# Ryan21wy/HSIMAE

Hardware: AMD Instinct MI355X
Metric: HSI patches/sec (9x9x96, mask 75%) pretrain fwd+bwd (higher is better)
Workload: dtype bf16; 1 GPU; HSIMAE-Base pretrain fwd+bwd, 9x9x96 cubes, per-GPU batch 4096, mask 0.75, bf16 MFMA operands / fp32 accumulate + residual; per_gpu_batch=4096, global_batch=4096, parallelism=dp1

## Files before the change

hsimae_amd/_lib.py:

```python
from __future__ import annotations

import ctypes as C
import os

HERE = os.path.dirname(os.path.abspath(__file__))
LIB_PATH = os.environ.get("HSIMAE_LIB") or os.path.join(HERE, "libhsimae_hip.so")

i32, i64, f32, vp = C.c_int32, C.c_int64, C.c_float, C.c_void_p


class Config(C.Structure):
    _fields_ = [("bands", i32), ("embed_dim", i32), ("depth", i32), ("s_depth", i32), ("num_heads", i32),
                ("dec_dim", i32), ("dec_depth", i32), ("dec_heads", i32), ("hidden", i32), ("dec_hidden", i32),
                ("norm_pix_loss", i32), ("precision", i32)]


class IO(C.Structure):
    _fields_ = [("x", vp), ("sn", i64), ("sb", i64), ("sh", i64), ("sw", i64),
                ("N", i32), ("len_t", i32), ("len_l", i32),
                ("noise1", vp), ("noise2", vp), ("params", vp), ("wpk", vp),
                ("workspace", vp), ("workspace_bytes", i64),
                ("grad_scale", f32), ("want_recons", i32),
                ("loss", vp), ("pred_img", vp), ("mask_img", vp), ("mask", vp),
                ("ids_keep", vp), ("ids_restore", vp), ("latent", vp), ("pred", vp), ("drop_scale", vp),
                ("bucket_stream", vp), ("det_acc", vp)]


class MaskParams(C.Structure):
    _fields_ = [("noise1", vp), ("noise2", vp), ("N", i32), ("T", i32), ("L", i32), ("len_t", i32), ("len_l", i32),
                ("ids_keep", vp), ("ids_restore", vp), ("mask", vp)]


class PatchParams(C.Structure):
    _fields_ = [("x", vp), ("sn", i64), ("sb", i64), ("sh", i64), ("sw", i64), ("N", i32), ("T", i32), ("K", i32),
                ("ids_keep", vp), ("out", vp), ("pos_ids", vp)]


class GemmParams(C.Structure):
    _fields_ = [("A", vp), ("lda", i32), ("M", i32), ("N", i32), ("K", i32), ("n_valid", i32),
                ("W", vp), ("W2", vp), ("bias", vp), ("bias2", vp), ("gamma", vp), ("beta", vp),
                ("stats", vp), ("u_out", vp), ("ldu", i32), ("out", vp), ("ldo", i32),
                ("res", vp), ("res2", vp), ("ldr", i32), ("pos", vp), ("ids", vp), ("ldpos", i32),
                ("h13", vp), ("ldh", i32), ("hoff", i32),
                ("lnx", vp), ("dgamma", vp), ("dbeta", vp), ("accumulate", i32),
                ("a_rowscale", vp), ("out_rowscale", vp),
                ("prec", i32), ("W8", vp), ("S8", vp), ("W8b", vp), ("S8b", vp), ("ln_width", i32),
                ("det_base", vp), ("det_acc", vp)]


class PackDesc(C.Structure):
    _fields_ = [("src", vp), ("rows", i32), ("cols", i32), ("transpose", i32), ("n_off", i32), ("k_off", i32),
                ("KS", i32), ("dst", vp), ("fp8", i32), ("scales", vp)]


class AttnParams(C.Structure):
    _fields_ = [("qkv", vp), ("ld", i32), ("d", i32), ("heads", i32), ("hd", i32), ("Ts", i32), ("nsamples", i32),
                ("mode", i32), ("len_l", i32), ("o", vp), ("ldo", i32), ("lse", vp), ("dout", vp), ("lddo", i32),
                ("dqkv", vp), ("kv_off", i32)]


class AttnBlockWeights(C.Structure):
    _fields_ = [(n, vp) for n in ("n1w", "n1b", "bqkv", "pb", "qkv", "p", "qkvT", "pT")]


class MlpWeights(C.Structure):
    _fields_ = [("n2w", vp), ("n2b", vp), ("w1b", vp), ("w3b", vp), ("w2b", vp),
                ("w1", vp), ("w3", vp), ("w2", vp), ("w2T", vp), ("w13T", vp), ("hidden", i32)]


class DecBlockWeights(C.Structure):
    _fields_ = [(n, vp) for n in ("n1w", "n1b", "bqkv", "pb", "n2w", "n2b", "w1b", "w3b", "w2b", "qkv", "p", "w1", "w3", "w2", "w2T",
                                  "qf", "kf", "vf", "pf", "w1f", "w3f")] + [("hidden", i32)]


class DecBlockGrads(C.Structure):
    _fields_ = [(n, vp) for n in ("n1w", "n1b", "qw", "qb", "kw", "kb", "vw", "vb", "pw", "pb", "n2w", "n2b", "w1w", "w1b", "w2w",
                                  "w2b", "w3w", "w3b")]


class WgradTask(C.Structure):
    _fields_ = [("dO", vp), ("dO_f32", i32), ("ldo", i32), ("A", vp), ("lda", i32), ("N", i32), ("K", i32),
                ("dW", vp), ("ldw", i32), ("db", vp), ("dO_rowscale", vp), ("dO_plane_rows", i32), ("A_plane_rows", i32)]


class WgradParams(C.Structure):
    _fields_ = [("t", WgradTask * 16), ("ntasks", i32), ("M", i32), ("msplit", i32), ("det_base", vp), ("det_acc", vp), ("slab", vp)]


class LnBwdParams(C.Structure):
    _fields_ = [("du", vp), ("x", vp), ("stats", vp), ("gamma", vp), ("dres", vp), ("dx", vp), ("accumulate", i32),
                ("dgamma", vp), ("dbeta", vp), ("M", i32), ("d", i32), ("ld", i32),
                ("det_base", vp), ("det_acc", vp)]


class AssembleParams(C.Structure):
    _fields_ = [("y", vp), ("N", i32), ("K", i32), ("TL", i32), ("Dd", i32), ("ids_restore", vp), ("pos", vp),
                ("yfull", vp), ("dyfull", vp), ("dy", vp), ("ld", i32)]


class LossParams(C.Structure):
    _fields_ = [("x", vp), ("sn", i64), ("sb", i64), ("sh", i64), ("sw", i64), ("N", i32), ("T", i32),
                ("pred", vp), ("mask", vp), ("norm_pix", i32), ("inv_scale", f32), ("partial", vp), ("loss", vp),
                ("sum_mask", f32), ("dpred", vp), ("pred_img", vp), ("mask_img", vp)]


class CubeParams(C.Structure):
    _fields_ = [("scenes", vp), ("scene_f64", i32), ("scene_off", vp), ("scene_w", vp), ("bands", i32),
                ("cut", vp), ("index", vp), ("flips", vp), ("N", i32),
                ("out", vp), ("sn", i64), ("sb", i64), ("sh", i64), ("sw", i64)]


class SceneParams(C.Structure):
    _fields_ = [("scene", vp), ("scene_f64", i32), ("H", i32), ("W", i32), ("C", i32),
                ("p0", i64), ("pixels", vp), ("N", i32),
                ("out", vp), ("sn", i64), ("sb", i64), ("sh", i64), ("sw", i64)]


class GwpcaParams(C.Structure):
    _fields_ = [("scene", vp), ("scene_f64", i32), ("H", i32), ("W", i32), ("C", i32), ("nc", i32), ("group", i32), ("whiten", i32),
                ("minmax", vp), ("mean", vp), ("lambda_", vp), ("proj", vp), ("group_off", vp)]


class BuildInfo(C.Structure):
    _fields_ = [("abi_version", i32), ("variant_bits", C.c_uint32), ("kernel_source_hash", C.c_uint64), ("flags_hash", C.c_uint64),
                ("default_flags", i32), ("reserved", i32)]


BUCKET_CB = C.CFUNCTYPE(None, i32, i64, i64, vp)

SYMBOLS = {
    "hsimae_version": (C.c_int, []),
    "hsimae_build_info": (C.c_int, [C.POINTER(BuildInfo)]),
    "hsimae_variant_name": (C.c_char_p, [C.c_int]),
    "hsimae_strerror": (C.c_char_p, [C.c_int]),
    "hsimae_two_streams_active": (C.c_int, []),
    "hsimae_effective_precision": (C.c_int, [C.POINTER(Config)]),
    "hsimae_dec_block_slab_floats": (i64, []),
    "hsimae_wgrad_slab_bytes": (i64, [C.POINTER(Config), i32]),
    "hsimae_param_layout": (C.c_int, [C.POINTER(Config), C.POINTER(i64), C.POINTER(i64), C.c_int]),
    "hsimae_wpk_elems": (i64, [C.POINTER(Config)]),
    "hsimae_pack_table_bytes": (i64, [C.POINTER(Config)]),
    "hsimae_build_pack_table": (C.c_int, [C.POINTER(Config), vp, vp, vp]),
    "hsimae_pack_params": (C.c_int, [C.POINTER(Config), vp, vp]),
    "hsimae_workspace_bytes": (i64, [C.POINTER(Config), i32, i32, i32]),
    "hsimae_forward": (C.c_int, [C.POINTER(Config), C.POINTER(IO), vp]),
    "hsimae_backward": (C.c_int, [C.POINTER(Config), C.POINTER(IO), vp, BUCKET_CB, vp, vp]),
    "hsimae_mask_from_noise": (C.c_int, [C.POINTER(MaskParams), vp]),
    "hsimae_patch_gather": (C.c_int, [C.POINTER(PatchParams), vp]),
    "hsimae_gemm": (C.c_int, [C.POINTER(GemmParams), i32, i32, vp]),
    "hsimae_gemm_tiled": (C.c_int, [C.POINTER(GemmParams), i32, i32, i32, i32, vp]),
    "hsimae_pack_matrix": (C.c_int, [vp, i32, i32, vp]),
    "hsimae_enc_mlp_fwd": (C.c_int, [vp, vp, vp, i32, i32, C.POINTER(MlpWeights), vp, vp]),
    "hsimae_enc_mlp_bwd": (C.c_int, [vp, vp, vp, vp, vp, vp, vp, vp, i32, i32, C.POINTER(MlpWeights), vp, vp, vp, vp, i32, vp]),
    "hsimae_dec_block_fwd": (C.c_int, [C.POINTER(DecBlockWeights), vp, vp, vp, vp, vp, i32, i32, i32, vp]),
    "hsimae_dec_block_bwd": (C.c_int, [C.POINTER(DecBlockWeights), C.POINTER(DecBlockGrads), vp, vp, vp, vp, vp, vp, vp, i32, i32, vp, vp]),
    "hsimae_attn_fwd": (C.c_int, [C.POINTER(AttnParams), vp]),
    "hsimae_attn_bwd": (C.c_int, [C.POINTER(AttnParams), vp]),
    "hsimae_attn_block_fwd": (C.c_int, [C.POINTER(AttnBlockWeights), vp, vp, vp, vp, vp, vp, vp, i32, i32, i32, i32, i32, i32, vp]),
    "hsimae_attn_block_bwd": (C.c_int, [C.POINTER(AttnBlockWeights), vp, vp, vp, vp, vp, vp, vp, vp, vp, vp, vp, vp, i32, i32, i32,
                                        i32, i32, i32, i32, vp]),
    "hsimae_wgrad": (C.c_int, [C.POINTER(WgradParams), vp]),
    "hsimae_wgrad_msplit": (i32, [i32, i64]),
    "hsimae_ln_bwd": (C.c_int, [C.POINTER(LnBwdParams), vp]),
    "hsimae_ln_fwd": (C.c_int, [vp, vp, vp, vp, i32, i32, vp]),
    "hsimae_assemble_fwd": (C.c_int, [C.POINTER(AssembleParams), vp]),
    "hsimae_assemble_bwd": (C.c_int, [C.POINTER(AssembleParams), vp]),
    "hsimae_loss_partials": (C.c_int, [i32, i32]),
    "hsimae_loss": (C.c_int, [C.POINTER(LossParams), vp]),
    "hsimae_adamw_step": (C.c_int, [vp, vp, vp, vp, vp, i64, f32, f32, f32, f32, f32, i32, vp]),
    "hsimae_cube_gather": (C.c_int, [C.POINTER(CubeParams), vp]),
    "hsimae_scene_windows": (C.c_int, [C.POINTER(SceneParams), vp]),
    "hsimae_class_argmax": (C.c_int, [C.POINTER(SceneParams), vp, i32, i32, i32, vp, vp]),
    "hsimae_gwpca_workspace_bytes": (i64, [C.POINTER(GwpcaParams)]),
    "hsimae_gwpca_fit": (C.c_int, [C.POINTER(GwpcaParams), vp, vp]),
    "hsimae_gwpca_apply": (C.c_int, [C.POINTER(GwpcaParams), vp, i32, vp]),
    "hsimae_encode": (C.c_int, [C.POINTER(Config), C.POINTER(IO), vp]),
    "hsimae_encode_backward": (C.c_int, [C.POINTER(Config), C.POINTER(IO), vp, vp, BUCKET_CB, vp, vp]),
    "hsimae_agg_pool": (C.c_int, [vp, vp, i32, i32, i32, i32, vp]),
    "hsimae_head_bwd": (C.c_int, [vp, vp, vp, vp, vp, vp, i32, i32, i32, i32, i32, vp]),
    "hsimae_decode": (C.c_int, [C.POINTER(Config), C.POINTER(IO), vp, vp, vp]),
    "hsimae_decode_backward": (C.c_int, [C.POINTER(Config), C.POINTER(IO), vp, vp, vp, BUCKET_CB, vp, vp]),
}

ABI_VERSION = 108
PREC_BF16, PREC_FP8 = 0, 1
A_BF16, A_F32, A_F32_LN = 0, 1, 2
E_BF16, E_F32, E_RES_F32, E_POS_F32, E_SWIGLU, E_SWIGLU_BWD, E_LN_BWD = 0, 1, 2, 3, 4, 5, 6

_lib = None


def load() -> C.CDLL:
    global _lib
    if _lib is None:
        if not os.path.exists(LIB_PATH):
            raise RuntimeError(
                f"{LIB_PATH} not found: build it with `python -m hsimae_amd.build` (hipcc --offload-arch=gfx950). "
                "hsimae_amd has no CPU fallback.")
        lib = C.CDLL(LIB_PATH)
        for name, (res, args) in SYMBOLS.items():
            fn = getattr(lib, name)
            fn.restype, fn.argtypes = res, args
        got = lib.hsimae_version()
        if got != ABI_VERSION:
            raise RuntimeError(f"{LIB_PATH} answers ABI version {got}, these bindings were written for {ABI_VERSION}: "
                               "rebuild it with `python -m hsimae_amd.build --force`")
        info = _query_build_info(lib)
        if info["variant"] and os.environ.get("HSIMAE_ALLOW_VARIANT") != "1":
            raise RuntimeError(f"{LIB_PATH} is a variant build ({', '.join(info['variant'])}): its kernels are instrumented or compute "
                               "wrong results on purpose (timing ablations).  Set HSIMAE_ALLOW_VARIANT=1 to load it for an experiment.")
        _lib = lib
    return _lib


def _query_build_info(lib) -> dict:
    bi = BuildInfo()
    rc = lib.hsimae_build_info(C.byref(bi))
    if rc != 0:
        raise RuntimeError(f"hsimae_build_info failed with code {rc}")
    names = []
    for b in range(32):
        if bi.variant_bits >> b & 1:
            n = lib.hsimae_variant_name(b)
            names.append(n.decode() if n else f"bit{b}")
    return {"path": LIB_PATH, "abi_version": bi.abi_version, "variant_bits": bi.variant_bits, "variant": names,
            "kernel_source_hash": f"{bi.kernel_source_hash:016x}", "flags_hash": f"{bi.flags_hash:016x}",
            "default_flags": bool(bi.default_flags)}


def build_info() -> dict:
    return _query_build_info(load())


def check(code: int, what: str = "hsimae") -> None:
    if code != 0:
        msg = load().hsimae_strerror(code)
        raise RuntimeError(f"{what} failed with code {code}: {msg.decode() if msg else '?'}")


def ptr(t) -> int | None:
    return None if t is None else t.data_ptr()
```

hsimae_amd/csrc/api.hip:

```cpp
#include "common.h"
#include "kernels.h"
#include "plan.h"
#include <vector>
#include <algorithm>
#include <cstring>
#include <cstdlib>
#include <mutex>
#include <unordered_map>
#include <initializer_list>

using namespace hsplan;

namespace {

#define CK(expr) do { int _e = (expr); if (_e) return _e; } while (0)
#define CK0(expr) do { int _e0 = (expr); if (_e0) return _e0; } while (0)

inline hipStream_t S(void* s) { return reinterpret_cast<hipStream_t>(s); }
struct BlkP {
    const float *n1w, *n1b, *bqkv, *pb, *n2w, *n2b, *w1b, *w3b, *w2b;
    const hs_bf16 *qkv, *p, *w1, *w3, *w2, *qkvT, *pT, *w13T, *w2T;
    const float *qf, *kf, *vf, *pf, *w1f, *w3f;
    int prec;
    struct I8 { const uint8_t* w; const uint8_t* s; } qkv8, p8, w1_8, w3_8, w2_8, qkvT8, pT8, w13T8, w2T8;
};

BlkP resolve(const BlkOff& o, const BlkW& w, const float* P, const hs_bf16* wpk, const WLayout& WL) {
    const float* fbase = reinterpret_cast<const float*>(wpk + WL.bf16_elems);
    BlkP b;
    b.n1w = P + o.n1w; b.n1b = P + o.n1b; b.bqkv = fbase + w.bqkv; b.pb = P + o.pb; b.n2w = P + o.n2w; b.n2b = P + o.n2b;
    b.w1b = P + o.w1b; b.w3b = P + o.w3b; b.w2b = P + o.w2b;
    b.qkv = wpk + w.qkv; b.p = wpk + w.p; b.w1 = wpk + w.w1; b.w3 = wpk + w.w3; b.w2 = wpk + w.w2;
    b.qkvT = wpk + w.qkvT; b.pT = wpk + w.pT; b.w13T = wpk + w.w13T; b.w2T = wpk + w.w2T;
    b.qf = P + o.qw; b.kf = P + o.kw; b.vf = P + o.vw; b.pf = P + o.pw; b.w1f = P + o.w1w; b.w3f = P + o.w3w;
    const uint8_t* base8 = reinterpret_cast<const uint8_t*>(fbase + WL.f32_elems);
    auto i8 = [&](const Img8& im) { BlkP::I8 r; r.w = base8 + im.w; r.s = base8 + im.s; return r; };
    b.prec = HSIMAE_PREC_BF16;
    b.qkv8 = i8(w.qkv8); b.p8 = i8(w.p8); b.w1_8 = i8(w.w1_8); b.w3_8 = i8(w.w3_8); b.w2_8 = i8(w.w2_8);
    b.qkvT8 = i8(w.qkvT8); b.pT8 = i8(w.pT8); b.w13T8 = i8(w.w13T8); b.w2T8 = i8(w.w2T8);
    return b;
}
enum : uint32_t {
    SC_FUSED_DEC = 1u << 0,
    SC_DEC_SPLIT = 1u << 1,
    SC_FP8_UNFUSED = 1u << 2,
    SC_FUSED_MLP = 1u << 3,
    SC_ATTN_BLOCK = 1u << 4,
    SC_ATTN_BLOCK256 = 1u << 5,
    SC_ATTN_BLOCK_BWD = 1u << 6,
    SC_PROJ_BWD = 1u << 7,
    SC_LNBWD = 1u << 8,
    SC_LNBWD_512 = 1u << 9,
    SC_RECOMPUTE = 1u << 10,
    SC_WGRAD_SLAB = 1u << 11,
    SC_DEC_SLAB = 1u << 12,
    SC_PLANAR = 1u << 13,
    SC_ATTN_BLOCK256_BWD = 1u << 14,
};
uint32_t sched_from_env() {
    auto off = [](const char* name) { const char* e = getenv(name); return e && e[0] == '0'; };
    auto one = [](const char* name) { const char* e = getenv(name); return e && e[0] == '1'; };
    uint32_t b = 0;
    if (!off("HSIMAE_FUSED_DEC")) b |= SC_FUSED_DEC;
    if (!off("HSIMAE_DEC_SPLIT")) b |= SC_DEC_SPLIT;
    if (one("HSIMAE_FP8_UNFUSED")) b |= SC_FP8_UNFUSED;
    if (!off("HSIMAE_FUSED_MLP")) b |= SC_FUSED_MLP;
    if (!off("HSIMAE_FUSED_ATTN_BLOCK")) b |= SC_ATTN_BLOCK;
    if (!off("HSIMAE_FUSED_ATTN_BLOCK256")) b |= SC_ATTN_BLOCK256;
    if (!off("HSIMAE_FUSED_ATTN_BLOCK_BWD")) b |= SC_ATTN_BLOCK_BWD;
    if (!off("HSIMAE_FUSED_PROJ_BWD")) b |= SC_PROJ_BWD;
    if (!off("HSIMAE_FUSED_LNBWD")) b |= SC_LNBWD;
    if (!off("HSIMAE_FUSED_LNBWD_512")) b |= SC_LNBWD_512;
    if (!off("HSIMAE_ATTN_BWD_RECOMPUTE")) b |= SC_RECOMPUTE;
    if (!off("HSIMAE_WGRAD_SLAB")) b |= SC_WGRAD_SLAB;
    if (!off("HSIMAE_DEC_SLAB")) b |= SC_DEC_SLAB;
    if (!off("HSIMAE_WGRAD_PLANAR")) b |= SC_PLANAR;
    if (!off("HSIMAE_FUSED_ATTN_BLOCK256_BWD")) b |= SC_ATTN_BLOCK256_BWD;
    return b;
}
struct SchedRec { uint32_t enc = 0, dec = 0; bool has_enc = false, has_dec = false; uint64_t gen = 0; };
std::mutex g_sched_mu;
std::unordered_map<const void*, SchedRec> g_sched;
uint64_t g_sched_gen = 0;
void record_sched(const void* ws, bool enc, bool dec, uint32_t bits) {
    std::lock_guard<std::mutex> lk(g_sched_mu);
    if (g_sched.size() > 4096 && g_sched.find(ws) == g_sched.end()) {
        std::vector<uint64_t> gens;
        gens.reserve(g_sched.size());
        for (auto& kv : g_sched) gens.push_back(kv.second.gen);
        std::nth_element(gens.begin(), gens.begin() + gens.size() / 2, gens.end());
        const uint64_t cut = gens[gens.size() / 2];
        for (auto it = g_sched.begin(); it != g_sched.end();) it = it->second.gen < cut ? g_sched.erase(it) : std::next(it);
    }
    SchedRec& r = g_sched[ws];
    r.gen = ++g_sched_gen;
    if (enc) {
        r.enc = bits; r.has_enc = true;
        if (!dec) r.has_dec = false;
    }
    if (dec) { r.dec = bits; r.has_dec = true; }
}
int lookup_sched(const void* ws, bool need_enc, bool need_dec, uint32_t& enc, uint32_t& dec) {
    std::lock_guard<std::mutex> lk(g_sched_mu);
    auto it = g_sched.find(ws);
    if (it == g_sched.end() || (need_enc && !it->second.has_enc) || (need_dec && !it->second.has_dec)) return HSIMAE_ENOFORWARD;
    enc = it->second.enc; dec = it->second.dec;
    return HSIMAE_OK;
}

BlkP resolve_enc(const Geo& g, uint32_t sc, const BlkOff& o, const BlkW& w, const float* P, const hs_bf16* wpk, const WLayout& WL) {
    BlkP b = resolve(o, w, P, wpk, WL);
    b.prec = (g.prec == HSIMAE_PREC_FP8 && (g.D >= 512 || (sc & SC_FP8_UNFUSED))) ? HSIMAE_PREC_FP8 : HSIMAE_PREC_BF16;
    return b;
}


struct Side {
    hipStream_t s = nullptr; hipEvent_t fork = nullptr, join = nullptr; bool ok = false, init = false;
    std::vector<hipEvent_t> pool; size_t next = 0;
};
Side& side() {
    static Side sides[32];
    static Side none;
    static std::mutex mu;
    int dev = -1;
    if (hipGetDevice(&dev) != hipSuccess || dev < 0 || dev >= 32) return none;
    std::lock_guard<std::mutex> lk(mu);
    Side& x = sides[dev];
    if (!x.init) {
        x.init = true;
        const char* e = getenv("HSIMAE_TWO_STREAMS");
        if (!(e && e[0] == '0'))
            x.ok = hipStreamCreateWithFlags(&x.s, hipStreamNonBlocking) == hipSuccess &&
                   hipEventCreateWithFlags(&x.fork, hipEventDisableTiming) == hipSuccess &&
                   hipEventCreateWithFlags(&x.join, hipEventDisableTiming) == hipSuccess;
    }
    return x;
}
hipEvent_t pool_event(Side& sd) {
    if (sd.pool.size() < 96) {
        hipEvent_t e = nullptr;
        if (hipEventCreateWithFlags(&e, hipEventDisableTiming) == hipSuccess) { sd.pool.push_back(e); return e; }
    }
    if (sd.pool.empty()) return nullptr;
    return sd.pool[sd.next++ % sd.pool.size()];
}

struct Emitter {
    hsimae_bucket_cb cb; void* user; hipStream_t bucket; int stage;
    float* grads; const int64_t* det_acc;
    int operator()(int64_t off, int64_t end, hipStream_t done_on) {
        if (det_acc) CK0(hs_det_convert(det_acc + off, grads + off, end - off, done_on));
        if (cb) {
            if (bucket) {
                hipEvent_t e = pool_event(side());
                if (!e) return (int)hipErrorOutOfMemory;
                CK0((int)hipEventRecord(e, done_on));
                CK0((int)hipStreamWaitEvent(bucket, e, 0));
            }
            cb(stage, off, end - off, user);
        }
        ++stage;
        return HSIMAE_OK;
    }
};

bool fused_dec_enabled(const Geo& g, uint32_t sc) {
    return (sc & SC_FUSED_DEC) && hs_dec_fused_supported(g.Dd, g.Hd, g.hdec, g.TL);
}



bool fused_mlp_enabled(int d, int h, uint32_t sc) {
    return (sc & SC_FUSED_MLP) && hs_enc_mlp_fused_supported(d, h);
}

EncMlpPtrs mlp_ptrs(const BlkP& b, int h) {
    EncMlpPtrs m;
    m.n2w = b.n2w; m.n2b = b.n2b; m.w1b = b.w1b; m.w3b = b.w3b; m.w2b = b.w2b;
    m.w1 = b.w1; m.w3 = b.w3; m.w2 = b.w2; m.w2T = b.w2T; m.w13T = b.w13T; m.h = h;
    return m;
}

DecBlockPtrs dec_ptrs(const BlkP& b, int h) {
    DecBlockPtrs d;
    d.n1w = b.n1w; d.n1b = b.n1b; d.bqkv = b.bqkv; d.pb = b.pb; d.n2w = b.n2w; d.n2b = b.n2b;
    d.w1b = b.w1b; d.w3b = b.w3b; d.w2b = b.w2b;
    d.qkv = b.qkv; d.p = b.p; d.w1 = b.w1; d.w3 = b.w3; d.w2 = b.w2;
    d.qkvT = b.qkvT; d.pT = b.pT; d.w13T = b.w13T; d.w2T = b.w2T; d.h = h;
    d.qf = b.qf; d.kf = b.kf; d.vf = b.vf; d.pf = b.pf; d.w1f = b.w1f; d.w3f = b.w3f;
    return d;
}

GemmParams gp() { GemmParams p; std::memset(&p, 0, sizeof(p)); return p; }

int dec_block_fwd_fused(const BlkP& bp, const float* z, const BlkBuf& b, int N, int64_t Md, int TL, int Dd, int hdec, uint32_t sc, hipStream_t s) {
    if ((sc & SC_DEC_SPLIT) && hs_enc_mlp_fused_supported(Dd, hdec)) {
        CK(hs_dec_attn_fwd(z, b.x1, b.o, b.lse, N, TL, dec_ptrs(bp, hdec), s));
        return hs_enc_mlp_fwd(b.x1, nullptr, b.x2, (int)Md, Dd, mlp_ptrs(bp, hdec), s);
    }
    return hs_dec_block_fwd(z, b.x1, b.x2, b.o, b.lse, N, TL, dec_ptrs(bp, hdec), s);
}

static bool attn_bwd_recompute(int d, int dp, int heads, int h, int Ts, bool f8u, uint32_t sc) {
    if (!(sc & SC_PROJ_BWD) || !(sc & SC_LNBWD) || !(sc & SC_RECOMPUTE)) return false;
    return !f8u && d == 128 && dp == d && fused_mlp_enabled(d, h, sc) && (sc & SC_ATTN_BLOCK) && (sc & SC_ATTN_BLOCK_BWD) &&
           hs_attn_block_bwd_fusable(d, heads, Ts);
}

int block_fwd(const BlkP& P, uint32_t sc, const float* x_in, const BlkBuf& b, int64_t M, int d, int heads, int h, int hp, int Ts,
              int nsamples, int mode, int len_l, const float* res2, hipStream_t s, const float* rs_a = nullptr,
              const float* rs_m = nullptr) {
    GemmParams p = gp();
    const int dp = rup(d, 32);
    const bool f8 = P.prec == HSIMAE_PREC_FP8;
    const bool f8u = f8 && (sc & SC_FP8_UNFUSED);
    auto w8 = [&](GemmParams& q, const BlkP::I8& a) { if (f8) { q.prec = HSIMAE_PREC_FP8; q.W8 = a.w; q.S8 = a.s; } };
    if (!f8u && (sc & SC_ATTN_BLOCK) && hs_attn_block_fusable(d, heads, Ts)) {
        CK(hs_attn_block_fwd(x_in, P.n1w, P.n1b, P.qkv, P.bqkv, P.p, P.pb, b.u, attn_bwd_recompute(d, dp, heads, h, Ts, f8u, sc) ? nullptr : b.qkv,
                             b.o, b.lse, b.x1, rs_a, Ts, nsamples, mode, len_l, s));
        if (fused_mlp_enabled(d, h, sc)) return hs_enc_mlp_fwd(b.x1, res2, b.x2, (int)M, d, mlp_ptrs(P, h), s, rs_m);
    } else if (!f8 && dp == d && (sc & SC_ATTN_BLOCK256) && hs_attn_block256_fusable(d, heads, Ts, nsamples)) {
        CK(hs_attn_block256_fwd(x_in, P.n1w, P.n1b, P.qkv, P.bqkv, P.p, P.pb, b.u, b.qkv, b.o, b.lse, b.x1, rs_a, Ts, nsamples, mode,
                                len_l, s));
    } else {
    p.A = x_in; p.lda = dp; p.M = (int)M; p.N = 3 * dp; p.K = dp; p.n_valid = 3 * dp; p.W = P.qkv; p.bias = P.bqkv;
    p.gamma = P.n1w; p.beta = P.n1b; p.u_out = b.u; p.ldu = dp; p.out = b.qkv; p.ldo = 3 * dp; p.ln_width = d;
    w8(p, P.qkv8);
    CK(hs_gemm(p, A_F32_LN, E_BF16, s));
    AttnParams a; std::memset(&a, 0, sizeof(a));
    a.qkv = b.qkv; a.ld = 3 * dp; a.d = d; a.heads = heads; a.hd = d / heads; a.Ts = Ts; a.nsamples = nsamples;
    a.mode = mode; a.len_l = len_l; a.o = b.o; a.ldo = dp; a.lse = b.lse; a.kv_off = dp;
    CK(hs_attn_fwd(a, s));
    p = gp();
    p.A = b.o; p.lda = dp; p.M = (int)M; p.N = dp; p.K = dp; p.n_valid = d; p.W = P.p; p.bias = P.pb;
    p.res = x_in; p.ldr = dp; p.out = b.x1; p.ldo = dp; p.out_rowscale = rs_a;
    w8(p, P.p8);
    CK(hs_gemm(p, A_BF16, E_RES_F32, s));
    }
    if (!f8u && fused_mlp_enabled(d, h, sc)) return hs_enc_mlp_fwd(b.x1, res2, b.x2, (int)M, d, mlp_ptrs(P, h), s, rs_m);
    p = gp();
    p.A = b.x1; p.lda = dp; p.M = (int)M; p.N = hp; p.K = dp; p.n_valid = h; p.W = P.w1; p.W2 = P.w3; p.bias = P.w1b;
    p.bias2 = P.w3b; p.gamma = P.n2w; p.beta = P.n2b; p.u_out = b.u2; p.ldu = dp; p.out = b.g; p.ldo = hp;
    p.h13 = b.h13; p.ldh = 2 * hp; p.hoff = hp; p.ln_width = d;
    if (f8) { w8(p, P.w1_8); p.W8b = P.w3_8.w; p.S8b = P.w3_8.s; }
    CK(hs_gemm(p, A_F32_LN, E_SWIGLU, s));
    p = gp();
    p.A = b.g; p.lda = hp; p.M = (int)M; p.N = dp; p.K = hp; p.n_valid = d; p.W = P.w2; p.bias = P.w2b;
    p.res = b.x1; p.res2 = res2; p.ldr = dp; p.out = b.x2; p.ldo = dp; p.out_rowscale = rs_m;
    w8(p, P.w2_8);
    CK(hs_gemm(p, A_BF16, E_RES_F32, s));
    return HSIMAE_OK;
}


static bool wide_ln_fused(int d, int dp, bool f8, uint32_t sc) {
    return (sc & SC_LNBWD) && dp == d && (d == 256 || (d == 512 && f8 && (sc & SC_LNBWD_512)));
}

int block_bwd(const BlkP& P, uint32_t sc, const BlkOff& o, float* grads, const float* x_in, const BlkBuf& b, int64_t M, int d,
              int heads, int h, int hp, int Ts, int nsamples, int mode, int len_l, float* G0, const Scr& w,
              float* dx_out, int accumulate, hipStream_t s, int concurrent = 1, const float* rs_a = nullptr,
              const float* rs_m = nullptr, int64_t* det_acc = nullptr) {
    float* G1 = w.G1;
    GemmParams p = gp();
    const int dp = rup(d, 32);
    LnBwdParams l; std::memset(&l, 0, sizeof(l));
    l.M = (int)M; l.d = d; l.ld = dp; l.det_base = grads; l.det_acc = det_acc;
    const bool f8 = P.prec == HSIMAE_PREC_FP8;
    const bool f8u = f8 && (sc & SC_FP8_UNFUSED);
    auto w8 = [&](GemmParams& q, const BlkP::I8& a) { if (f8) { q.prec = HSIMAE_PREC_FP8; q.W8 = a.w; q.S8 = a.s; } };
    const bool fmlp = !f8u && fused_mlp_enabled(d, h, sc);
    bool g1b_done = false;
    const int hp64 = rup(hp, 64);
    const bool planar = fmlp && (sc & SC_PLANAR) && M % 32 == 0 && (M + kPlanePadRows) * 2 * (int64_t)(hp64 + 256) * 2 < (1ll << 32);
    const int prow = planar ? (int)M + HS_PLANE_PAD_ROWS : 0;
    if (fmlp) {
        CK(hs_enc_mlp_bwd(b.x1, G0, G1, b.u2, w.dh13, b.g, w.g0b, w.g1b, (int)M, d, mlp_ptrs(P, h), grads + o.n2w,
                          grads + o.n2b, s, rs_m, rs_a, HsDet{grads, reinterpret_cast<long long*>(det_acc)}, prow));
    } else {
        p.A = G0; p.lda = dp; p.M = (int)M; p.N = hp; p.K = dp; p.n_valid = hp; p.W = P.w2T; p.out = w.dh13; p.ldo = 2 * hp;
        p.h13 = b.h13; p.ldh = 2 * hp; p.hoff = hp; p.a_rowscale = rs_m;
        w8(p, P.w2T8);
        CK(hs_gemm(p, A_F32, E_SWIGLU_BWD, s));
        p = gp();
        p.A = w.dh13; p.lda = 2 * hp; p.M = (int)M; p.N = dp; p.K = 2 * hp; p.n_valid = d; p.W = P.w13T;
        w8(p, P.w13T8);
        if (wide_ln_fused(d, dp, f8, sc)) {
            p.out = G1; p.ldo = dp; p.res = G0; p.ldr = dp; p.lnx = b.x1; p.gamma = P.n2w; p.accumulate = 0;
            p.dgamma = grads + o.n2w; p.dbeta = grads + o.n2b; p.det_base = grads; p.det_acc = det_acc;
            if (!rs_a) { p.u_out = w.g1b; p.ldu = dp; g1b_done = true; }
            CK(hs_gemm(p, A_BF16, E_LN_BWD, s));
        } else {
            p.out = w.du; p.ldo = dp;
            CK(hs_gemm(p, A_BF16, E_F32, s));
            l.du = w.du; l.x = b.x1; l.gamma = P.n2w; l.dres = G0; l.dx = G1; l.accumulate = 0;
            l.dgamma = grads + o.n2w; l.dbeta = grads + o.n2b;
            CK(hs_ln_bwd(l, s));
        }
        CK(hs_rows_to_bf16(G0, w.g0b, M, dp, rs_m, s));
        if (!g1b_done) CK(hs_rows_to_bf16(G1, w.g1b, M, dp, rs_a, s));
    }
    auto run_wgrad = [&]() -> int {
        WgradParams g; std::memset(&g, 0, sizeof(g));
        auto task = [&](int, const void* dO, int ldo, const hs_bf16* A, int lda, int N, int K, int64_t dW, int64_t db) {
            WgradTask& t = g.t[g.ntasks++];
            t.dO = dO; t.dO_f32 = 0; t.ldo = ldo; t.A = A; t.lda = lda; t.N = N; t.K = K; t.dW = grads + dW; t.ldw = K;
            t.db = grads + db; t.dO_rowscale = nullptr;
        };
        task(0, w.dqkv, 3 * dp, b.u, dp, d, d, o.qw, o.qb);
        task(1, w.dqkv + dp, 3 * dp, b.u, dp, d, d, o.kw, o.kb);
        task(2, w.dqkv + 2 * dp, 3 * dp, b.u, dp, d, d, o.vw, o.vb);
        task(3, w.g1b, dp, b.o, dp, d, d, o.pw, o.pb);
        if (planar) {
            task(4, w.dh13, hp64, b.u2, dp, h, d, o.w1w, o.w1b); g.t[g.ntasks - 1].dO_plane_rows = prow;
            task(5, w.dh13 + (int64_t)hp64 * prow, hp64, b.u2, dp, h, d, o.w3w, o.w3b); g.t[g.ntasks - 1].dO_plane_rows = prow;
        } else {
            task(4, w.dh13, 2 * hp, b.u2, dp, h, d, o.w1w, o.w1b);
            task(5, w.dh13 + hp, 2 * hp, b.u2, dp, h, d, o.w3w, o.w3b);
        }
#ifdef HS_ABL_DW2
        if (!fmlp)
#endif
        { task(6, w.g0b, dp, b.g, planar ? hp64 : hp, d, h, o.w2w, o.w2b); g.t[g.ntasks - 1].A_plane_rows = prow; }
        g.M = (int)M; g.det_base = grads; g.det_acc = det_acc;
        g.slab = (sc & SC_WGRAD_SLAB) ? w.slab : nullptr;
        int tiles = 0;
        for (int i = 0; i < g.ntasks; ++i) tiles += ((g.t[i].N + 127) / 128) * ((g.t[i].K + 127) / 128);
        g.msplit = wgrad_msplit(tiles, M, concurrent);
        return hs_wgrad(g, s);
    };
    AttnParams a; std::memset(&a, 0, sizeof(a));
    a.qkv = b.qkv; a.ld = 3 * dp; a.d = d; a.heads = heads; a.hd = d / heads; a.Ts = Ts; a.nsamples = nsamples;
    a.mode = mode; a.len_l = len_l; a.o = b.o; a.ldo = dp; a.lse = b.lse; a.dout = w.dob; a.lddo = dp; a.dqkv = w.dqkv; a.kv_off = dp;
    const bool fuse_pb = (sc & SC_PROJ_BWD) != 0;
    const bool fuse_ln = (sc & SC_LNBWD) != 0;
    const bool rc = attn_bwd_recompute(d, dp, heads, h, Ts, f8u, sc);
    const bool blk_bwd = rc || (fuse_pb && fuse_ln && fmlp && !f8u && d == 128 && dp == d && hs_attn_proj_fusable(a) &&
                                (sc & SC_ATTN_BLOCK_BWD) && hs_attn_block_bwd_fusable(d, heads, Ts));
    const bool blk256_bwd = !blk_bwd && !f8 && dp == d && (sc & SC_ATTN_BLOCK256_BWD) && (sc & SC_LNBWD) && (sc & SC_PROJ_BWD) &&
                            hs_attn_block256_bwd_fusable(d, heads, Ts, nsamples);
    if (blk256_bwd) {
        CK(hs_attn_block256_bwd(b.qkv, b.lse, w.g1b, G1, x_in, P.n1w, P.pT, P.qkvT, w.dqkv, dx_out, grads + o.n1w, grads + o.n1b, grads,
                                reinterpret_cast<long long*>(det_acc), Ts, nsamples, mode, len_l, accumulate, s));
        CK(run_wgrad());
        return HSIMAE_OK;
    }
    if (blk_bwd) {
        CK(hs_attn_block_bwd(rc ? nullptr : b.qkv, b.u, P.qkv, P.bqkv, b.o, b.lse, w.g1b, G1, x_in, P.n1w, P.pT, P.qkvT, w.dqkv, dx_out,
                             grads + o.n1w, grads + o.n1b, grads, reinterpret_cast<long long*>(det_acc), Ts, nsamples, mode, len_l,
                             accumulate, s));
    } else {
        p = gp();
        p.A = w.g1b; p.lda = dp; p.M = (int)M; p.N = dp; p.K = dp; p.n_valid = dp;
        p.W = P.pT; p.out = w.dob; p.ldo = dp;
        w8(p, P.pT8);
        CK(hs_gemm(p, A_BF16, E_BF16, s));
    }
    if (!blk_bwd) CK(hs_attn_bwd(a, s));
    CK(run_wgrad());

    if (blk_bwd) return HSIMAE_OK;
    const bool ln_fused = fuse_ln && ((d == 128 && !f8u) || wide_ln_fused(d, dp, f8, sc));
    p = gp();
    p.A = w.dqkv; p.lda = 3 * dp; p.M = (int)M; p.N = dp; p.K = 3 * dp; p.n_valid = d; p.W = P.qkvT;
    if (ln_fused) {
        p.out = dx_out; p.ldo = d; p.res = G1; p.ldr = d; p.lnx = x_in; p.gamma = P.n1w; p.accumulate = accumulate;
        p.dgamma = grads + o.n1w; p.dbeta = grads + o.n1b; p.det_base = grads; p.det_acc = det_acc;
        if (d != 128) w8(p, P.qkvT8);
        CK(hs_gemm(p, A_BF16, E_LN_BWD, s));
    } else {
        p.out = w.du; p.ldo = dp;
        w8(p, P.qkvT8);
        CK(hs_gemm(p, A_BF16, E_F32, s));
    }

    if (!ln_fused) {
        l.du = w.du; l.x = x_in; l.gamma = P.n1w; l.dres = G1; l.dx = dx_out; l.accumulate = accumulate;
        l.dgamma = grads + o.n1w; l.dbeta = grads + o.n1b;
        CK(hs_ln_bwd(l, s));
    }
    return HSIMAE_OK;
}

struct Ctx {
    Geo g; PLayout L; WLayout W; Ws w;
    int N, K, len_t, len_l;
    int64_t Me, Md;
};

int make_ctx(const hsimae_config* cfg, const hsimae_io* io, Ctx& c, bool need_ws) {
    CK(make_geo(cfg, c.g));
    if (!io) return HSIMAE_ENULL;
    c.N = io->N; c.len_t = io->len_t; c.len_l = io->len_l;
    if (c.N <= 0 || c.len_t < 1 || c.len_t > c.g.T || c.len_l < 1 || c.len_l > 9) return HSIMAE_EDIMS;
    c.K = c.len_t * c.len_l;
    c.Me = (int64_t)c.N * c.K; c.Md = (int64_t)c.N * c.g.TL;
    if (c.Md * 96 >= (1ll << 31) || c.Me * 3 * c.g.Dp >= (1ll << 31)) return HSIMAE_EUNSUPPORTED;
    make_playout(c.g, c.L);
    make_wlayout(c.g, c.W);
    if (need_ws) {
        if (!io->workspace || !io->params || !io->wpk) return HSIMAE_ENULL;
        if (reinterpret_cast<uintptr_t>(io->workspace) % 256) return HSIMAE_EALIGN;
        carve(c.g, c.N, c.K, reinterpret_cast<char*>(io->workspace), c.w);
        if (c.w.bytes > io->workspace_bytes) return HSIMAE_EDIMS;
    }
    return HSIMAE_OK;
}

}

extern "C" unsigned hs_variant_bits_gemm();
extern "C" unsigned hs_variant_bits_attn();
extern "C" unsigned hs_variant_bits_attn_wide();
extern "C" unsigned hs_variant_bits_wgrad();
extern "C" unsigned hs_variant_bits_elem();
extern "C" unsigned hs_variant_bits_pack();
extern "C" unsigned hs_variant_bits_fused_dec();
extern "C" unsigned hs_variant_bits_fused_enc();
extern "C" unsigned hs_variant_bits_loader();
extern "C" unsigned hs_variant_bits_scene();
extern "C" unsigned hs_variant_bits_gwpca();
#ifndef HS_KERNEL_SOURCE_HASH
#define HS_KERNEL_SOURCE_HASH 0ULL
#endif
#ifndef HS_BUILD_FLAGS_HASH
#define HS_BUILD_FLAGS_HASH 0ULL
#endif
#ifndef HS_BUILD_DEFAULT_FLAGS
#define HS_BUILD_DEFAULT_FLAGS 0
#endif

extern "C" {

int hsimae_version(void) { return HSIMAE_VERSION; }

int hsimae_build_info(hsimae_build_info_t* out) {
    if (!out) return HSIMAE_ENULL;
    out->abi_version = HSIMAE_VERSION;
    out->variant_bits = hs_variant_bits() | hs_variant_bits_gemm() | hs_variant_bits_attn() | hs_variant_bits_attn_wide() | hs_variant_bits_wgrad() | hs_variant_bits_elem() | hs_variant_bits_pack() | hs_variant_bits_fused_dec() | hs_variant_bits_fused_enc() | hs_variant_bits_loader() | hs_variant_bits_scene() | hs_variant_bits_gwpca();
    out->kernel_source_hash = HS_KERNEL_SOURCE_HASH;
    out->flags_hash = HS_BUILD_FLAGS_HASH;
    out->default_flags = HS_BUILD_DEFAULT_FLAGS;
    out->reserved = 0;
    return HSIMAE_OK;
}
const char* hsimae_variant_name(int bit) {
    switch (bit) {
#define HS_X(b, name) case b: return #name;
        HS_VARIANT_TABLE(HS_X)
#undef HS_X
        default: return nullptr;
    }
}

int hsimae_two_streams_active(void) { return side().ok ? 1 : 0; }
int hsimae_effective_precision(const hsimae_config* cfg) {
    if (!cfg) return HSIMAE_ENULL;
    Geo g; CK(make_geo(cfg, g));
    return (g.prec == HSIMAE_PREC_FP8 && (g.D >= 512 || (sched_from_env() & SC_FP8_UNFUSED))) ? HSIMAE_PREC_FP8 : HSIMAE_PREC_BF16;
}

const char* hsimae_strerror(int code) {
    switch (code) {
        case HSIMAE_OK: return "ok";
        case HSIMAE_EDIMS: return "bad dimensions or strides";
        case HSIMAE_EUNSUPPORTED: return "configuration not supported by the gfx950 kernels";
        case HSIMAE_EALIGN: return "misaligned pointer";
        case HSIMAE_ENULL: return "required pointer is NULL";
        case HSIMAE_ENOFORWARD: return "no forward pass of this process has filled this workspace (the backward follows the forward's recorded schedule)";
        default: return code > 0 ? hipGetErrorString((hipError_t)code) : "unknown error";
    }
}

int hsimae_param_layout(const hsimae_config* cfg, int64_t* offsets, int64_t* sizes, int max_entries) {
    return param_layout(cfg, offsets, sizes, max_entries);
}

int64_t hsimae_wpk_elems(const hsimae_config* cfg) { return wpk_elems(cfg); }

int64_t hsimae_pack_table_bytes(const hsimae_config* cfg) { return pack_table_bytes(cfg); }

int hsimae_build_pack_table(const hsimae_config* cfg, const float* params_dev, hs_bf16* wpk_dev, void* table_host) {
    return build_pack_table(cfg, params_dev, wpk_dev, table_host);
}

int hsimae_pack_params(const hsimae_config* cfg, const void* table_dev, void* stream) {
    Geo g; CK(make_geo(cfg, g));
    if (!table_dev) return HSIMAE_ENULL;
    const int n = (int)(hsimae_pack_table_bytes(cfg) / (int64_t)sizeof(PackDesc));
    const int maxe = std::max({g.D * g.D, g.h * g.D, g.Dd * g.Dd, g.hdec * g.Dd, g.D * g.Dd, g.D * 72});
    return hs_pack(reinterpret_cast<const PackDesc*>(table_dev), n, maxe, S(stream));
}

int64_t hsimae_workspace_bytes(const hsimae_config* cfg, int32_t N, int32_t len_t, int32_t len_l) {
    return workspace_bytes(cfg, N, len_t, len_l);
}

struct DropRs { const float* a; const float* m; };
static DropRs drop_rs(const hsimae_io* io, int e, int64_t Me) {
    if (!io->drop_scale) return DropRs{nullptr, nullptr};
    const float* base = io->drop_scale + (int64_t)e * 2 * Me;
    return DropRs{base, base + Me};
}

static int forward_impl(const hsimae_config* cfg, const hsimae_io* io, void* stream, bool encoder_only) {
    Ctx c; CK(make_ctx(cfg, io, c, true));
    if (!io->x || !io->noise1 || !io->noise2 || !io->mask || !io->ids_keep || !io->ids_restore) return HSIMAE_ENULL;
    if (encoder_only ? !io->latent : !io->loss) return HSIMAE_ENULL;
    if (!encoder_only && io->want_recons && (!io->pred_img || !io->mask_img)) return HSIMAE_ENULL;
    hipStream_t s = S(stream);
    const Geo& g = c.g; const float* P = io->params; const Ws& w = c.w;
    const uint32_t sc = sched_from_env();
    record_sched(io->workspace, true, !encoder_only, sc);

    MaskParams m; m.noise1 = io->noise1; m.noise2 = io->noise2; m.N = c.N; m.T = g.T; m.L = 9; m.len_t = c.len_t;
    m.len_l = c.len_l; m.ids_keep = io->ids_keep; m.ids_restore = io->ids_restore; m.mask = io->mask;
    CK(hs_mask(m, s));
    PatchParams pp; pp.x = io->x; pp.sn = io->sn; pp.sb = io->sb; pp.sh = io->sh; pp.sw = io->sw; pp.N = c.N; pp.T = g.T;
    pp.K = c.K; pp.ids_keep = io->ids_keep; pp.out = w.a_pe; pp.pos_ids = nullptr;
    CK(hs_patch_gather(pp, s));
    GemmParams p = gp();
    p.A = w.a_pe; p.lda = 96; p.M = (int)c.Me; p.N = g.Dp; p.K = 96; p.n_valid = g.D; p.W = io->wpk + c.W.pe; p.bias = P + c.L.peb;
    p.pos = P + c.L.pos; p.ids = io->ids_keep; p.ldpos = g.D; p.out = w.x0; p.ldo = g.Dp;
    CK(hs_gemm(p, A_BF16, E_POS_F32, s));

    const float* x = w.x0;
    if (g.has_axis) {
        Side& sd = side();
        const bool forked = sd.ok && g.sdepth > 1;
        if (forked) {
            CK((int)hipEventRecord(sd.fork, s));
            CK((int)hipStreamWaitEvent(sd.s, sd.fork, 0));
        }
        const float* xa = w.x0;
        const float* xb = w.x0;
        for (int i = 0; i < g.sdepth; ++i) {
            BlkP b1 = resolve_enc(g, sc, c.L.b1[i], c.W.b1[i], P, io->wpk, c.W);
            const DropRs r1 = drop_rs(io, i, c.Me), r2d = drop_rs(io, g.sdepth + i, c.Me);
            CK(block_fwd(b1, sc, xa, w.b1[i], c.Me, g.D, g.H, g.h, g.hp, c.K, c.N, 1, c.len_l, nullptr, s, r1.a, r1.m));
            xa = w.b1[i].x2;
            BlkP b2 = resolve_enc(g, sc, c.L.b2[i], c.W.b2[i], P, io->wpk, c.W);
            const bool last = (i == g.sdepth - 1);
            const float* r2 = last ? xa : nullptr;
            if (last && forked) {
                CK((int)hipEventRecord(sd.join, sd.s));
                CK((int)hipStreamWaitEvent(s, sd.join, 0));
            }
            CK(block_fwd(b2, sc, xb, w.b2[i], c.Me, g.D, g.H, g.h, g.hp, c.K, c.N, 2, c.len_l, r2, (forked && !last) ? sd.s : s,
                         r2d.a, r2d.m));
            xb = w.b2[i].x2;
        }
        x = xb;
    }
    for (int i = 0; i < g.nfus; ++i) {
        BlkP bp = resolve_enc(g, sc, c.L.bf[i], c.W.bf[i], P, io->wpk, c.W);
        const DropRs rf = drop_rs(io, (g.has_axis ? 2 * g.sdepth : 0) + i, c.Me);
        CK(block_fwd(bp, sc, x, w.bf[i], c.Me, g.D, g.H, g.h, g.hp, c.K, c.N, 0, c.len_l, nullptr, s, rf.a, rf.m));
        x = w.bf[i].x2;
    }
    if (encoder_only) {
        CK(hs_ln_fwd(x, P + c.L.nw, P + c.L.nb, io->latent, (int)c.Me, g.D, s, g.Dp, g.D));
        return HSIMAE_OK;
    }
    p = gp();
    p.A = x; p.lda = g.Dp; p.M = (int)c.Me; p.N = g.Ddp; p.K = g.Dp; p.n_valid = g.Dd; p.W = io->wpk + c.W.de; p.bias = P + c.L.deb;
    p.gamma = P + c.L.nw; p.beta = P + c.L.nb; p.u_out = w.lat; p.ldu = g.Dp; p.out = w.y; p.ldo = g.Ddp; p.ln_width = g.D;
    CK(hs_gemm(p, A_F32_LN, E_F32, s));
    AssembleParams as; std::memset(&as, 0, sizeof(as));
    as.y = w.y; as.N = c.N; as.K = c.K; as.TL = g.TL; as.Dd = g.Dd; as.ld = g.Ddp; as.ids_restore = io->ids_restore; as.pos = P + c.L.dpos;
    as.yfull = w.yfull;
    CK(hs_assemble_fwd(as, s));
    const float* z = w.yfull;
    const bool fdec = fused_dec_enabled(g, sc);
    for (int i = 0; i < g.ddepth; ++i) {
        BlkP bp = resolve(c.L.bd[i], c.W.bd[i], P, io->wpk, c.W);
        if (fdec) CK(dec_block_fwd_fused(bp, z, w.bd[i], c.N, c.Md, g.TL, g.Dd, g.hdec, sc, s));
        else CK(block_fwd(bp, sc, z, w.bd[i], c.Md, g.Dd, g.Hd, g.hdec, g.hpd, g.TL, c.N, 0, 9, nullptr, s));
        z = w.bd[i].x2;
    }
    p = gp();
    p.A = z; p.lda = g.Ddp; p.M = (int)c.Md; p.N = 80; p.K = g.Ddp; p.n_valid = 72; p.W = io->wpk + c.W.dp; p.bias = P + c.L.dpb;
    p.gamma = P + c.L.dnw; p.beta = P + c.L.dnb; p.u_out = w.zn; p.ldu = g.Ddp; p.out = w.pred; p.ldo = 72; p.ln_width = g.Dd;
    CK(hs_gemm(p, A_F32_LN, E_F32, s));
    LossParams lp; std::memset(&lp, 0, sizeof(lp));
    const float sum_mask = (float)((int64_t)c.N * (g.TL - c.K));
    lp.x = io->x; lp.sn = io->sn; lp.sb = io->sb; lp.sh = io->sh; lp.sw = io->sw; lp.N = c.N; lp.T = g.T; lp.pred = w.pred;
    lp.mask = io->mask; lp.norm_pix = g.norm_pix; lp.inv_scale = io->grad_scale / (72.f * sum_mask); lp.partial = w.partial;
    lp.loss = io->loss; lp.sum_mask = sum_mask; lp.dpred = w.dpred;
    lp.pred_img = io->want_recons ? io->pred_img : nullptr; lp.mask_img = io->want_recons ? io->mask_img : nullptr;
    CK(hs_loss(lp, s));
    if (io->pred) CK((int)hipMemcpyAsync(io->pred, w.pred, c.Md * 72 * 4, hipMemcpyDeviceToDevice, s));
    if (io->latent) CK(hs_ln_fwd(x, P + c.L.nw, P + c.L.nb, io->latent, (int)c.Me, g.D, s, g.Dp, g.D));
    return HSIMAE_OK;
}

int hsimae_forward(const hsimae_config* cfg, const hsimae_io* io, void* stream) { return forward_impl(cfg, io, stream, false); }
int hsimae_encode(const hsimae_config* cfg, const hsimae_io* io, void* stream) { return forward_impl(cfg, io, stream, true); }

int hsimae_decode(const hsimae_config* cfg, const hsimae_io* io, const float* latent, float* pred, void* stream) {
    Ctx c; CK(make_ctx(cfg, io, c, true));
    if (!latent || !pred || !io->ids_restore) return HSIMAE_ENULL;
    hipStream_t s = S(stream);
    const Geo& g = c.g; const float* P = io->params; const Ws& w = c.w;
    const uint32_t sc = sched_from_env();
    record_sched(io->workspace, false, true, sc);
    GemmParams p = gp();
    const float* lat_in = latent;
    if (g.Dp != g.D) {
        CK((int)hipMemcpy2DAsync(w.G2, (size_t)g.Dp * 4, latent, (size_t)g.D * 4, (size_t)g.D * 4, (size_t)c.Me, hipMemcpyDeviceToDevice, s));
        lat_in = w.G2;
    }
    p.A = lat_in; p.lda = g.Dp; p.M = (int)c.Me; p.N = g.Ddp; p.K = g.Dp; p.n_valid = g.Dd; p.W = io->wpk + c.W.de; p.bias = P + c.L.deb;
    p.out = w.y; p.ldo = g.Ddp;
    CK(hs_gemm(p, A_F32, E_F32, s));
    CK(hs_rows_to_bf16(lat_in, w.lat, c.Me, g.Dp, nullptr, s));
    AssembleParams as; std::memset(&as, 0, sizeof(as));
    as.y = w.y; as.N = c.N; as.K = c.K; as.TL = g.TL; as.Dd = g.Dd; as.ld = g.Ddp; as.ids_restore = io->ids_restore; as.pos = P + c.L.dpos;
    as.yfull = w.yfull;
    CK(hs_assemble_fwd(as, s));
    const float* z = w.yfull;
    const bool fdec = fused_dec_enabled(g, sc);
    for (int i = 0; i < g.ddepth; ++i) {
        BlkP bp = resolve(c.L.bd[i], c.W.bd[i], P, io->wpk, c.W);
        if (fdec) CK(dec_block_fwd_fused(bp, z, w.bd[i], c.N, c.Md, g.TL, g.Dd, g.hdec, sc, s));
        else CK(block_fwd(bp, sc, z, w.bd[i], c.Md, g.Dd, g.Hd, g.hdec, g.hpd, g.TL, c.N, 0, 9, nullptr, s));
        z = w.bd[i].x2;
    }
    p = gp();
    p.A = z; p.lda = g.Ddp; p.M = (int)c.Md; p.N = 80; p.K = g.Ddp; p.n_valid = 72; p.W = io->wpk + c.W.dp; p.bias = P + c.L.dpb;
    p.gamma = P + c.L.dnw; p.beta = P + c.L.dnb; p.u_out = w.zn; p.ldu = g.Ddp; p.out = pred; p.ldo = 72; p.ln_width = g.Dd;
    return hs_gemm(p, A_F32_LN, E_F32, s);
}

static int encoder_backward(const Ctx& c, const hsimae_io* io, float* grads, hipStream_t s, Emitter& emit, uint32_t sc) {
    const Geo& g = c.g; const float* P = io->params; const Ws& w = c.w; const PLayout& L = c.L;
    for (int i = g.nfus - 1; i >= 0; --i) {
        BlkP bp = resolve_enc(g, sc, L.bf[i], c.W.bf[i], P, io->wpk, c.W);
        const float* xin = (i > 0) ? w.bf[i - 1].x2 : (g.has_axis ? w.b2[g.sdepth - 1].x2 : w.x0);
        const DropRs rf = drop_rs(io, (g.has_axis ? 2 * g.sdepth : 0) + i, c.Me);
        CK(block_bwd(bp, sc, L.bf[i], grads, xin, w.bf[i], c.Me, g.D, g.H, g.h, g.hp, c.K, c.N, 0, c.len_l, w.G0, w.sc, w.G0, 0, s, 1,
                     rf.a, rf.m, io->det_acc));
        CK(emit(L.bf[i].n1w, L.bf[i].end, s));
    }
    if (g.has_axis) {
        Side& sd = side();
        const bool forked = sd.ok && g.sdepth > 1;
        CK((int)hipMemcpyAsync(w.G2, w.G0, c.Me * g.Dp * 4, hipMemcpyDeviceToDevice, s));
        if (forked) {
            CK((int)hipEventRecord(sd.fork, s));
            CK((int)hipStreamWaitEvent(sd.s, sd.fork, 0));
        }
        hipStream_t s2 = forked ? sd.s : s;
        const Scr& scr2 = forked ? w.sc2 : w.sc;
        const bool per_block = emit.bucket != nullptr || !forked;
        for (int i = g.sdepth - 1; i >= 0; --i) {
            BlkP b2 = resolve_enc(g, sc, L.b2[i], c.W.b2[i], P, io->wpk, c.W);
            const DropRs r1 = drop_rs(io, i, c.Me), r2d = drop_rs(io, g.sdepth + i, c.Me);
            const float* xin2 = (i > 0) ? w.b2[i - 1].x2 : w.x0;
            CK(block_bwd(b2, sc, L.b2[i], grads, xin2, w.b2[i], c.Me, g.D, g.H, g.h, g.hp, c.K, c.N, 2, c.len_l, w.G0, scr2, w.G0, 0, s2, forked ? 2 : 1,
                         r2d.a, r2d.m, io->det_acc));
            if (per_block) CK(emit(L.b2[i].n1w, L.b2[i].end, s2));
            if (i == 0 && forked) {
                CK((int)hipEventRecord(sd.join, sd.s));
                CK((int)hipStreamWaitEvent(s, sd.join, 0));
            }
            BlkP b1 = resolve_enc(g, sc, L.b1[i], c.W.b1[i], P, io->wpk, c.W);
            const float* xin1 = (i > 0) ? w.b1[i - 1].x2 : w.x0;
            float* out = (i == 0) ? w.G0 : w.G2;
            CK(block_bwd(b1, sc, L.b1[i], grads, xin1, w.b1[i], c.Me, g.D, g.H, g.h, g.hp, c.K, c.N, 1, c.len_l, w.G2, w.sc, out, i == 0, s, forked ? 2 : 1,
                         r1.a, r1.m, io->det_acc));
            if (per_block) CK(emit(L.b1[i].n1w, L.b1[i].end, s));
        }
        if (!per_block) {
            for (int i = g.sdepth - 1; i >= 0; --i) CK(emit(L.b2[i].n1w, L.b2[i].end, s));
            for (int i = g.sdepth - 1; i >= 0; --i) CK(emit(L.b1[i].n1w, L.b1[i].end, s));
        }
    }
    {
        WgradParams wg; std::memset(&wg, 0, sizeof(wg));
        WgradTask& t = wg.t[0]; t.dO = w.G0; t.dO_f32 = 1; t.ldo = g.Dp; t.A = w.a_pe; t.lda = 96; t.N = g.D; t.K = 72;
        t.dW = grads + L.pew; t.ldw = 72; t.db = grads + L.peb;
        wg.det_base = grads; wg.det_acc = io->det_acc;
        wg.ntasks = 1; wg.M = (int)c.Me; wg.msplit = wgrad_msplit((g.D + 127) / 128, c.Me);
        CK(hs_wgrad(wg, s));
    }
    CK(emit(0, L.peb + g.D, s));
    return HSIMAE_OK;
}

static int decoder_backward(const Ctx& c, const hsimae_io* io, float* grads, hipStream_t s, Emitter& emit, uint32_t sc) {
    const Geo& g = c.g; const float* P = io->params; const Ws& w = c.w; const PLayout& L = c.L;
    const float* zlast = w.bd[g.ddepth - 1].x2;
    GemmParams p = gp();
    p.A = w.dpred; p.lda = 96; p.M = (int)c.Md; p.N = g.Ddp; p.K = 96; p.n_valid = g.Dd; p.W = io->wpk + c.W.dpT; p.out = w.du; p.ldo = g.Ddp;
    CK(hs_gemm(p, A_BF16, E_F32, s));
    {
        WgradParams wg; std::memset(&wg, 0, sizeof(wg));
        WgradTask& t = wg.t[0]; t.dO = w.dpred; t.dO_f32 = 0; t.ldo = 96; t.A = w.zn; t.lda = g.Ddp; t.N = 72; t.K = g.Dd;
        t.dW = grads + L.dpw; t.ldw = g.Dd; t.db = grads + L.dpb;
        wg.det_base = grads; wg.det_acc = io->det_acc;
        wg.ntasks = 1; wg.M = (int)c.Md; wg.msplit = wgrad_msplit(1, c.Md);
        CK(hs_wgrad(wg, s));
    }
    LnBwdParams l; std::memset(&l, 0, sizeof(l));
    l.du = w.du; l.x = zlast; l.gamma = P + L.dnw; l.dres = nullptr; l.dx = w.G0; l.dgamma = grads + L.dnw; l.dbeta = grads + L.dnb;
    l.M = (int)c.Md; l.d = g.Dd; l.ld = g.Ddp; l.det_base = grads; l.det_acc = io->det_acc;
    CK(hs_ln_bwd(l, s));
    CK(emit(L.dnw, L.total, s));

    const bool fdec = fused_dec_enabled(g, sc);
    for (int i = g.ddepth - 1; i >= 0; --i) {
        BlkP bp = resolve(L.bd[i], c.W.bd[i], P, io->wpk, c.W);
        const float* xin = (i == 0) ? w.yfull : w.bd[i - 1].x2;
        if (fdec) {
            const BlkOff& o = L.bd[i];
            DecBlockGrads dg;
            dg.n1w = grads + o.n1w; dg.n1b = grads + o.n1b; dg.qw = grads + o.qw; dg.qb = grads + o.qb;
            dg.kw = grads + o.kw; dg.kb = grads + o.kb; dg.vw = grads + o.vw; dg.vb = grads + o.vb;
            dg.pw = grads + o.pw; dg.pb = grads + o.pb; dg.n2w = grads + o.n2w; dg.n2b = grads + o.n2b;
            dg.w1w = grads + o.w1w; dg.w1b = grads + o.w1b; dg.w2w = grads + o.w2w; dg.w2b = grads + o.w2b;
            dg.w3w = grads + o.w3w; dg.w3b = grads + o.w3b;
            dg.det = HsDet{grads, reinterpret_cast<long long*>(io->det_acc)};
            CK(hs_dec_block_bwd(xin, w.bd[i].x1, w.G0, w.G1, w.G0, w.bd[i].o, w.bd[i].lse, c.N, g.TL, dec_ptrs(bp, g.hdec), dg, s,
                                (sc & SC_DEC_SLAB) ? w.slab : nullptr));
        } else {
            CK(block_bwd(bp, sc, L.bd[i], grads, xin, w.bd[i], c.Md, g.Dd, g.Hd, g.hdec, g.hpd, g.TL, c.N, 0, 9, w.G0, w.sc, w.G0, 0, s, 1, nullptr, nullptr,
                         io->det_acc));
        }
        CK(emit(L.bd[i].n1w, L.bd[i].end, s));
    }
    AssembleParams as; std::memset(&as, 0, sizeof(as));
    as.N = c.N; as.K = c.K; as.TL = g.TL; as.Dd = g.Dd; as.ld = g.Ddp; as.ids_restore = io->ids_restore; as.dyfull = w.G0; as.dy = w.dyb;
    CK(hs_assemble_bwd(as, s));
    p = gp();
    p.A = w.dyb; p.lda = g.Ddp; p.M = (int)c.Me; p.N = g.Dp; p.K = g.Ddp; p.n_valid = g.D; p.W = io->wpk + c.W.deT; p.out = w.du; p.ldo = g.Dp;
    CK(hs_gemm(p, A_BF16, E_F32, s));
    {
        WgradParams wg; std::memset(&wg, 0, sizeof(wg));
        WgradTask& t = wg.t[0]; t.dO = w.dyb; t.dO_f32 = 0; t.ldo = g.Ddp; t.A = w.lat; t.lda = g.Dp; t.N = g.Dd; t.K = g.D;
        t.dW = grads + L.dew; t.ldw = g.D; t.db = grads + L.deb;
        wg.det_base = grads; wg.det_acc = io->det_acc;
        wg.ntasks = 1; wg.M = (int)c.Me; wg.msplit = wgrad_msplit(((g.Dd + 127) / 128) * ((g.D + 127) / 128), c.Me);
        CK(hs_wgrad(wg, s));
    }
    return HSIMAE_OK;
}

int hsimae_backward(const hsimae_config* cfg, const hsimae_io* io, float* grads, hsimae_bucket_cb cb, void* user,
                    void* stream) {
    Ctx c; CK(make_ctx(cfg, io, c, true));
    if (!grads || !io->ids_restore) return HSIMAE_ENULL;
    uint32_t sc_enc = 0, sc_dec = 0;
    CK(lookup_sched(io->workspace, true, true, sc_enc, sc_dec));
    hipStream_t s = S(stream);
    if (io->det_acc) CK((int)hipMemsetAsync(io->det_acc, 0, (size_t)c.L.total * 8, s));
    const Geo& g = c.g; const float* P = io->params; const Ws& w = c.w; const PLayout& L = c.L;
    Emitter emit{cb, user, cb ? S(io->bucket_stream) : nullptr, 0, grads, io->det_acc};
    CK(decoder_backward(c, io, grads, s, emit, sc_dec));
    const float* xf = g.nfus ? w.bf[g.nfus - 1].x2 : (g.has_axis ? w.b2[g.sdepth - 1].x2 : w.x0);
    LnBwdParams l; std::memset(&l, 0, sizeof(l));
    l.du = w.du; l.x = xf; l.gamma = P + L.nw; l.dres = nullptr; l.dx = w.G0; l.dgamma = grads + L.nw; l.dbeta = grads + L.nb;
    l.M = (int)c.Me; l.d = g.D; l.ld = g.Dp; l.det_base = grads; l.det_acc = io->det_acc;
    CK(hs_ln_bwd(l, s));
    CK(emit(L.nw, L.deb + g.Dd, s));
    return encoder_backward(c, io, grads, s, emit, sc_enc);
}

int hsimae_decode_backward(const hsimae_config* cfg, const hsimae_io* io, const float* dpred, float* dlatent, float* grads,
                           hsimae_bucket_cb cb, void* user, void* stream) {
    Ctx c; CK(make_ctx(cfg, io, c, true));
    if (!grads || !dpred || !dlatent || !io->ids_restore) return HSIMAE_ENULL;
    uint32_t sc_enc = 0, sc_dec = 0;
    CK(lookup_sched(io->workspace, false, true, sc_enc, sc_dec));
    hipStream_t s = S(stream);
    if (io->det_acc) CK((int)hipMemsetAsync(io->det_acc, 0, (size_t)c.L.total * 8, s));
    const Geo& g = c.g; const Ws& w = c.w; const PLayout& L = c.L;
    CK(hs_rows_pad_bf16(dpred, w.dpred, c.Md, 72, 96, s));
    Emitter emit{cb, user, cb ? S(io->bucket_stream) : nullptr, 0, grads, io->det_acc};
    CK(decoder_backward(c, io, grads, s, emit, sc_dec));
    CK(emit(L.dew, L.deb + g.Dd, s));
    return (int)hipMemcpy2DAsync(dlatent, (size_t)g.D * 4, w.du, (size_t)g.Dp * 4, (size_t)g.D * 4, (size_t)c.Me, hipMemcpyDeviceToDevice, s);
}

int hsimae_encode_backward(const hsimae_config* cfg, const hsimae_io* io, const float* dlatent, float* grads,
                           hsimae_bucket_cb cb, void* user, void* stream) {
    Ctx c; CK(make_ctx(cfg, io, c, true));
    if (!grads || !dlatent) return HSIMAE_ENULL;
    uint32_t sc_enc = 0, sc_dec = 0;
    CK(lookup_sched(io->workspace, true, false, sc_enc, sc_dec));
    hipStream_t s = S(stream);
    if (io->det_acc) CK((int)hipMemsetAsync(io->det_acc, 0, (size_t)c.L.total * 8, s));
    const Geo& g = c.g; const float* P = io->params; const Ws& w = c.w; const PLayout& L = c.L;
    const float* xf = g.nfus ? w.bf[g.nfus - 1].x2 : (g.has_axis ? w.b2[g.sdepth - 1].x2 : w.x0);
    LnBwdParams l; std::memset(&l, 0, sizeof(l));
    const float* dlat = dlatent;
    if (g.Dp != g.D) {
        CK((int)hipMemcpy2DAsync(w.du, (size_t)g.Dp * 4, dlatent, (size_t)g.D * 4, (size_t)g.D * 4, (size_t)c.Me, hipMemcpyDeviceToDevice, s));
        dlat = w.du;
    }
    l.du = dlat; l.x = xf; l.gamma = P + L.nw; l.dres = nullptr; l.dx = w.G0; l.dgamma = grads + L.nw; l.dbeta = grads + L.nb;
    l.M = (int)c.Me; l.d = g.D; l.ld = g.Dp; l.det_base = grads; l.det_acc = io->det_acc;
    CK(hs_ln_bwd(l, s));
    Emitter emit{cb, user, cb ? S(io->bucket_stream) : nullptr, 0, grads, io->det_acc};
    CK(emit(L.nw, L.nb + g.D, s));
    return encoder_backward(c, io, grads, s, emit, sc_enc);
}

int hsimae_mask_from_noise(const hsimae_mask_params* p, void* stream) { return p ? hs_mask(*p, S(stream)) : HSIMAE_ENULL; }
int hsimae_patch_gather(const hsimae_patch_params* p, void* stream) { return p ? hs_patch_gather(*p, S(stream)) : HSIMAE_ENULL; }
int hsimae_gemm(const hsimae_gemm_params* p, int32_t a_kind, int32_t epilogue, void* stream) {
    return p ? hs_gemm(*p, a_kind, epilogue, S(stream)) : HSIMAE_ENULL;
}
int hsimae_gemm_tiled(const hsimae_gemm_params* p, int32_t a_kind, int32_t epilogue, int32_t bm, int32_t kc, void* stream) {
    return p ? hs_gemm_tiled(*p, a_kind, epilogue, bm, kc, S(stream)) : HSIMAE_ENULL;
}
int hsimae_pack_matrix(const hsimae_pack_desc* d, int32_t n, int32_t max_elems, void* stream) {
    return d ? hs_pack(d, n, max_elems, S(stream)) : HSIMAE_ENULL;
}
static EncMlpPtrs mlp_from_abi(const hsimae_mlp_weights* w) {
    EncMlpPtrs m;
    m.n2w = w->n2w; m.n2b = w->n2b; m.w1b = w->w1b; m.w3b = w->w3b; m.w2b = w->w2b;
    m.w1 = w->w1; m.w3 = w->w3; m.w2 = w->w2; m.w2T = w->w2T; m.w13T = w->w13T; m.h = w->hidden;
    return m;
}
int hsimae_enc_mlp_fwd(const float* x1, const float* res2, float* x2, int32_t M, int32_t d, const hsimae_mlp_weights* w,
                       const float* rowscale, void* stream) {
    if (M <= 0) return HSIMAE_OK;
    if (!x1 || !x2 || !w) return HSIMAE_ENULL;
    if (!hs_enc_mlp_fused_supported(d, w->hidden)) return HSIMAE_EUNSUPPORTED;
    return hs_enc_mlp_fwd(x1, res2, x2, M, d, mlp_from_abi(w), S(stream), rowscale);
}
int hsimae_enc_mlp_bwd(const float* x1, const float* dy, float* dx1, hs_bf16* u2, hs_bf16* dh13, hs_bf16* g, hs_bf16* dyb,
                       hs_bf16* dx1b, int32_t M, int32_t d, const hsimae_mlp_weights* w, float* g_n2w, float* g_n2b,
                       const float* rs_mlp, const float* rs_attn, int32_t plane_rows, void* stream) {
    if (plane_rows && plane_rows < M) return HSIMAE_EDIMS;
    if (M <= 0) return HSIMAE_OK;
    if (!x1 || !dy || !dx1 || !w || !g_n2w || !g_n2b) return HSIMAE_ENULL;
    if ((!u2) != (!dyb) || (!dh13) != (!g)) return HSIMAE_ENULL;
    if (!hs_enc_mlp_fused_supported(d, w->hidden)) return HSIMAE_EUNSUPPORTED;
    return hs_enc_mlp_bwd(x1, dy, dx1, u2, dh13, g, dyb, dx1b, M, d, mlp_from_abi(w), g_n2w, g_n2b, S(stream), rs_mlp, rs_attn,
                          HsDet{nullptr, nullptr}, plane_rows);
}
static DecBlockPtrs dec_from_abi(const hsimae_dec_block_weights* w) {
    DecBlockPtrs d; std::memset(&d, 0, sizeof(d));
    d.n1w = w->n1w; d.n1b = w->n1b; d.bqkv = w->bqkv; d.pb = w->pb; d.n2w = w->n2w; d.n2b = w->n2b;
    d.w1b = w->w1b; d.w3b = w->w3b; d.w2b = w->w2b;
    d.qkv = w->qkv; d.p = w->p; d.w1 = w->w1; d.w3 = w->w3; d.w2 = w->w2; d.w2T = w->w2T;
    d.qf = w->qf; d.kf = w->kf; d.vf = w->vf; d.pf = w->pf; d.w1f = w->w1f; d.w3f = w->w3f; d.h = w->hidden;
    return d;
}
int hsimae_dec_block_fwd(const hsimae_dec_block_weights* w, const float* x, float* x1, float* x2, hs_bf16* o, float* lse,
                         int32_t nsamples, int32_t Ts, int32_t split, void* stream) {
    if (nsamples <= 0) return HSIMAE_OK;
    if (!w || !x || !x1 || !x2 || !o || !lse) return HSIMAE_ENULL;
    if (!hs_dec_fused_supported(64, 8, w->hidden, Ts)) return HSIMAE_EUNSUPPORTED;
    const DecBlockPtrs d = dec_from_abi(w);
    if (split) {
        CK(hs_dec_attn_fwd(x, x1, o, lse, nsamples, Ts, d, S(stream)));
        EncMlpPtrs m;
        m.n2w = d.n2w; m.n2b = d.n2b; m.w1b = d.w1b; m.w3b = d.w3b; m.w2b = d.w2b;
        m.w1 = d.w1; m.w3 = d.w3; m.w2 = d.w2; m.w2T = d.w2T; m.w13T = nullptr; m.h = d.h;
        return hs_enc_mlp_fwd(x1, nullptr, x2, nsamples * Ts, 64, m, S(stream));
    }
    return hs_dec_block_fwd(x, x1, x2, o, lse, nsamples, Ts, d, S(stream));
}
int64_t hsimae_dec_block_slab_floats(void) { return kDecSlabFloats; }
int64_t hsimae_wgrad_slab_bytes(const hsimae_config* cfg, int32_t side_stream) { return wgrad_slab_bytes(cfg, side_stream); }
int hsimae_dec_block_bwd(const hsimae_dec_block_weights* w, const hsimae_dec_block_grads* g, const float* x, const float* x1,
                         const float* dy, float* dx1_tmp, float* dx, const hs_bf16* o, const float* lse, int32_t nsamples,
                         int32_t Ts, float* slab, void* stream) {
    if (nsamples <= 0) return HSIMAE_OK;
    if (!w || !g || !x || !x1 || !dy || !dx1_tmp || !dx || !o || !lse) return HSIMAE_ENULL;
    if (!hs_dec_fused_supported(64, 8, w->hidden, Ts)) return HSIMAE_EUNSUPPORTED;
    DecBlockGrads dg;
    dg.n1w = g->n1w; dg.n1b = g->n1b; dg.qw = g->qw; dg.qb = g->qb; dg.kw = g->kw; dg.kb = g->kb; dg.vw = g->vw; dg.vb = g->vb;
    dg.pw = g->pw; dg.pb = g->pb; dg.n2w = g->n2w; dg.n2b = g->n2b; dg.w1w = g->w1w; dg.w1b = g->w1b; dg.w2w = g->w2w;
    dg.w2b = g->w2b; dg.w3w = g->w3w; dg.w3b = g->w3b; dg.det = HsDet{nullptr, nullptr};
    return hs_dec_block_bwd(x, x1, dy, dx1_tmp, dx, o, lse, nsamples, Ts, dec_from_abi(w), dg, S(stream), slab);
}
int hsimae_attn_fwd(const hsimae_attn_params* p, void* stream) { return p ? hs_attn_fwd(*p, S(stream)) : HSIMAE_ENULL; }
int hsimae_attn_bwd(const hsimae_attn_params* p, void* stream) { return p ? hs_attn_bwd(*p, S(stream)) : HSIMAE_ENULL; }
static int attn_block_check(const hsimae_attn_block_weights* w, int d, int heads, int Ts, int nsamples, int mode, int len_l,
                            std::initializer_list<const void*> rows) {
    if (!w || !w->n1w || !w->n1b || !w->bqkv || !w->pb || !w->qkv || !w->p || !w->qkvT || !w->pT) return HSIMAE_ENULL;
    if (!((d == 128 && heads == 8) || (d == 256 && heads == 16))) return HSIMAE_EUNSUPPORTED;
    if (mode < 0 || mode > 2) return HSIMAE_EUNSUPPORTED;
    if (Ts < 1 || (mode != 0 && len_l < 1)) return HSIMAE_EDIMS;
    if (Ts > 32) return HSIMAE_EUNSUPPORTED;
    if (d == 256 && !hs_attn_block256_fusable(d, heads, Ts, nsamples)) return HSIMAE_EUNSUPPORTED;
    for (const void* r : rows) {
        if (!r) return HSIMAE_ENULL;
        if (reinterpret_cast<uintptr_t>(r) & 15) return HSIMAE_EALIGN;
    }
    return HSIMAE_OK;
}
int hsimae_attn_block_fwd(const hsimae_attn_block_weights* w, const float* x, hs_bf16* u, hs_bf16* qkv, hs_bf16* o, float* lse,
                          float* x1, const float* rowscale, int32_t d, int32_t heads, int32_t Ts, int32_t nsamples, int32_t mode,
                          int32_t len_l, void* stream) {
    if (nsamples < 0) return HSIMAE_EDIMS;
    if (nsamples == 0) return HSIMAE_OK;
    CK(attn_block_check(w, d, heads, Ts, nsamples, mode, len_l, {x, u, o, lse, x1}));
    if (qkv && (reinterpret_cast<uintptr_t>(qkv) & 15)) return HSIMAE_EALIGN;
    if (d == 128)
        return hs_attn_block_fwd(x, w->n1w, w->n1b, w->qkv, w->bqkv, w->p, w->pb, u, qkv, o, lse, x1, rowscale, Ts, nsamples, mode, len_l,
                                 S(stream));
    if (!qkv) return HSIMAE_EUNSUPPORTED;
    return hs_attn_block256_fwd(x, w->n1w, w->n1b, w->qkv, w->bqkv, w->p, w->pb, u, qkv, o, lse, x1, rowscale, Ts, nsamples, mode, len_l,
                                S(stream));
}
int hsimae_attn_block_bwd(const hsimae_attn_block_weights* w, const hs_bf16* qkv, const hs_bf16* u, const hs_bf16* o, const float* lse,
                          const hs_bf16* dx1b, const float* dx1, const float* x, hs_bf16* dqkv, float* dx, float* dgamma, float* dbeta,
                          int64_t* det_acc, int32_t accumulate, int32_t d, int32_t heads, int32_t Ts, int32_t nsamples, int32_t mode,
                          int32_t len_l, void* stream) {
    if (nsamples < 0) return HSIMAE_EDIMS;
    if (nsamples == 0) return HSIMAE_OK;
    CK(attn_block_check(w, d, heads, Ts, nsamples, mode, len_l, {u, o, lse, dx1b, dx1, x, dqkv, dx}));
    if (!dgamma || !dbeta) return HSIMAE_ENULL;
    if (qkv && (reinterpret_cast<uintptr_t>(qkv) & 15)) return HSIMAE_EALIGN;
    if (!qkv && d != 128) return HSIMAE_EUNSUPPORTED;
    if (det_acc && dbeta != dgamma + d) return HSIMAE_EDIMS;
    hipStream_t s = S(stream);
    if (det_acc) CK((int)hipMemsetAsync(det_acc, 0, sizeof(int64_t) * 2 * d, s));
    long long* acc = reinterpret_cast<long long*>(det_acc);
    if (d == 128)
        CK(hs_attn_block_bwd(qkv, u, w->qkv, w->bqkv, o, lse, dx1b, dx1, x, w->n1w, w->pT, w->qkvT, dqkv, dx, dgamma, dbeta, dgamma, acc,
                             Ts, nsamples, mode, len_l, accumulate, s));
    else
        CK(hs_attn_block256_bwd(qkv, lse, dx1b, dx1, x, w->n1w, w->pT, w->qkvT, dqkv, dx, dgamma, dbeta, dgamma, acc, Ts, nsamples, mode,
                                len_l, accumulate, s));
    return det_acc ? hs_det_convert(det_acc, dgamma, 2 * d, s) : HSIMAE_OK;
}
int hsimae_wgrad(const hsimae_wgrad_params* p, void* stream) { return p ? hs_wgrad(*p, S(stream)) : HSIMAE_ENULL; }
int32_t hsimae_wgrad_msplit(int32_t tiles, int64_t M) { return wgrad_msplit(tiles, M); }
int hsimae_agg_pool(const float* latent, float* pooled, int32_t N, int32_t T, int32_t L, int32_t D, void* stream) {
    if (N <= 0) return HSIMAE_OK;
    if (!latent || !pooled) return HSIMAE_ENULL;
    return hs_agg_pool(latent, pooled, N, T, L, D, S(stream));
}
int hsimae_head_bwd(const float* g, const float* pooled, const float* w, float* gw, float* gb, float* dlatent, int32_t N, int32_t C,
                    int32_t T, int32_t L, int32_t D, void* stream) {
    if (N <= 0) return HSIMAE_OK;
    if (!g || !pooled || !w || !gw || !gb || !dlatent) return HSIMAE_ENULL;
    return hs_head_bwd(g, pooled, w, gw, gb, dlatent, N, C, T, L, D, S(stream));
}
int hsimae_cube_gather(const hsimae_cube_params* p, void* stream) {
    if (!p) return HSIMAE_ENULL;
    if (p->N <= 0) return HSIMAE_OK;
    if (!p->scenes || !p->scene_off || !p->scene_w || !p->cut || !p->index || !p->out) return HSIMAE_ENULL;
    return hs_cube_gather(*p, S(stream));
}
int hsimae_scene_windows(const hsimae_scene_params* p, void* stream) {
    if (!p) return HSIMAE_ENULL;
    if (p->N < 0 || p->H <= 0 || p->W <= 0 || p->C <= 0) return HSIMAE_EDIMS;
    if (p->N == 0) return HSIMAE_OK;
    if (!p->scene || !p->out) return HSIMAE_ENULL;
    if (!p->pixels && (p->p0 < 0 || p->p0 + p->N > (int64_t)p->H * p->W)) return HSIMAE_EDIMS;
    return hs_scene_windows(*p, S(stream));
}
int hsimae_class_argmax(const hsimae_scene_params* p, const float* logits, int32_t ld, int32_t num_class, int32_t first, int64_t* map,
                        void* stream) {
    if (!p) return HSIMAE_ENULL;
    if (p->N < 0 || p->H <= 0 || p->W <= 0 || first < 0 || first >= num_class || num_class > 256 || ld < num_class) return HSIMAE_EDIMS;
    if (p->N == 0) return HSIMAE_OK;
    if (!logits || !map) return HSIMAE_ENULL;
    if (!p->pixels && (p->p0 < 0 || p->p0 + p->N > (int64_t)p->H * p->W)) return HSIMAE_EDIMS;
    return hs_class_argmax(*p, logits, ld, num_class, first, map, S(stream));
}
int64_t hsimae_gwpca_workspace_bytes(const hsimae_gwpca_params* p) { return p ? hs_gwpca_workspace_bytes(*p) : (int64_t)HSIMAE_ENULL; }
int hsimae_gwpca_fit(const hsimae_gwpca_params* p, void* workspace, void* stream) {
    return p ? hs_gwpca_fit(*p, workspace, S(stream)) : HSIMAE_ENULL;
}
int hsimae_gwpca_apply(const hsimae_gwpca_params* p, void* out, int32_t out_f64, void* stream) {
    return p ? hs_gwpca_apply(*p, out, out_f64, S(stream)) : HSIMAE_ENULL;
}
int hsimae_ln_bwd(const hsimae_lnbwd_params* p, void* stream) { return p ? hs_ln_bwd(*p, S(stream)) : HSIMAE_ENULL; }
int hsimae_ln_fwd(const float* x, const float* gamma, const float* beta, float* out, int32_t M, int32_t d, void* stream) {
    return (x && gamma && beta && out) ? hs_ln_fwd(x, gamma, beta, out, M, d, S(stream)) : HSIMAE_ENULL;
}
int hsimae_assemble_fwd(const hsimae_assemble_params* p, void* stream) { return p ? hs_assemble_fwd(*p, S(stream)) : HSIMAE_ENULL; }
int hsimae_assemble_bwd(const hsimae_assemble_params* p, void* stream) { return p ? hs_assemble_bwd(*p, S(stream)) : HSIMAE_ENULL; }
int hsimae_adamw_step(float* params, const float* grads, float* exp_avg, float* exp_avg_sq, const uint8_t* group, int64_t n,
                      float lr, float beta1, float beta2, float eps, float weight_decay, int32_t step, void* stream) {
    if (!params || !grads || !exp_avg || !exp_avg_sq || !group) return HSIMAE_ENULL;
    return hs_adamw(params, grads, exp_avg, exp_avg_sq, group, n, lr, beta1, beta2, eps, weight_decay, step, S(stream));
}
int hsimae_loss_partials(int32_t N, int32_t T) { return hs_loss_partials(N, T); }
int hsimae_loss(const hsimae_loss_params* p, void* stream) { return p ? hs_loss(*p, S(stream)) : HSIMAE_ENULL; }

}
```

hsimae_amd/csrc/gemm.hip:

```cpp
#include "common.h"
#include "kernels.h"
#include <algorithm>
#include <cstdlib>
#include <type_traits>

#ifdef HS_PHASE_TIMING
__device__ unsigned long long hs_phase_cycles_gemm[64];
extern "C" __attribute__((visibility("default"))) int hsimae_debug_phases_gemm(unsigned long long* out, int reset) {
    int rc = (int)hipMemcpyFromSymbol(out, HIP_SYMBOL(hs_phase_cycles_gemm), sizeof(unsigned long long) * 64);
    if (reset) { unsigned long long z[64] = {0}; rc |= (int)hipMemcpyToSymbol(HIP_SYMBOL(hs_phase_cycles_gemm), z, sizeof(z)); }
    return rc;
}
#define PH_DECL unsigned long long ph_t0 = __builtin_readcyclecounter(), ph_acc[4] = {0, 0, 0, 0};
#define PH(i) { const unsigned long long ph_t = __builtin_readcyclecounter(); ph_acc[i] += ph_t - ph_t0; ph_t0 = ph_t; }
#define PH_FLUSH(base) if (threadIdx.x == 0) { for (int i = 0; i < 4; ++i) atomicAdd(&hs_phase_cycles_gemm[(base) + i], ph_acc[i]); }
#else
#define PH_DECL
#define PH(i)
#define PH_FLUSH(base)
#endif

namespace {

typedef __attribute__((ext_vector_type(8))) int i32x8;

#ifndef HS_EPI_ROWS_F8
#define HS_EPI_ROWS_F8 16
#endif
template <int KC, int F8 = 0, int BM = 128> struct EpiRows {
    static constexpr int f8rows = HS_EPI_ROWS_F8 > BM ? BM : HS_EPI_ROWS_F8;
    static constexpr int v = F8 ? f8rows : (KC >= 512 ? 16 : 32);
};
constexpr int TS = 132;

template <int AK, int EPI, int KC, int BM, int F8, int NCH>
__global__ __launch_bounds__(256, (EPI == E_LN_BWD || BM <= 64) ? 2 : 1) void gemm_kernel(GemmParams p) {
    extern __shared__ __attribute__((aligned(16))) char smem[];
    static_assert(!F8 || KC == 512, "the fp8 path stages 512-deep chunks (one scale dword per row and lane group)");
    static_assert(NCH == 1 || (AK != A_F32_LN && EPI != E_SWIGLU), "k-outer: no LayerNorm prologue, no gate pair");
    constexpr int MT = BM / 16;
    constexpr int LDA = F8 ? KC + 16 : KC + 8;
    constexpr int ABYTES = F8 ? BM * LDA : BM * LDA * 2;
    constexpr int SCBYTES = F8 ? BM * 16 : 0;
    constexpr bool DUAL = (EPI == E_SWIGLU);
    constexpr int PR = EpiRows<KC, F8, BM>::v;
    bf16_t* As = reinterpret_cast<bf16_t*>(smem);
    unsigned char* As8 = reinterpret_cast<unsigned char*>(smem);
    unsigned char* Sc = reinterpret_cast<unsigned char*>(smem + ABYTES);
    float* rstat = reinterpret_cast<float*>(smem + ABYTES + SCBYTES);
    float* T1 = rstat + 2 * BM;
    float* T2 = T1 + PR * TS;

    const int tid = threadIdx.x, lane = tid & 63, wave = __builtin_amdgcn_readfirstlane(tid >> 6);
    const int row0 = blockIdx.x * BM;
    const int KS_total = F8 ? (p.K + 127) / 128 : p.K / 32;
    const int NT_total = p.N / 16;
    const int n_chunks = (NT_total + 7) / 8;
    const int k_chunks = (p.K + KC - 1) / KC;

    auto put_a8 = [&](int r, int c8, const float (&f)[8]) {
        float am = 0.f;
#pragma unroll
        for (int e = 0; e < 8; ++e) am = fmaxf(am, fabsf(f[e]));
        am = lanes_max<4>(am);
        int eb = (int)((__float_as_uint(am) >> 23) & 0xffu) - 8;
        eb = min(max(eb, 1), 254);
        const float inv = __uint_as_float((unsigned)(254 - eb) << 23);
        float q[8];
#pragma unroll
        for (int e = 0; e < 8; ++e) q[e] = fminf(fmaxf(f[e] * inv, -448.f), 448.f);
        int lo = __builtin_amdgcn_cvt_pk_fp8_f32(q[0], q[1], 0, false);
        lo = __builtin_amdgcn_cvt_pk_fp8_f32(q[2], q[3], lo, true);
        int hi = __builtin_amdgcn_cvt_pk_fp8_f32(q[4], q[5], 0, false);
        hi = __builtin_amdgcn_cvt_pk_fp8_f32(q[6], q[7], hi, true);
        *reinterpret_cast<int2*>(As8 + r * LDA + c8) = make_int2(lo, hi);
        if ((c8 & 31) == 0) Sc[(r * 4 + ((c8 & 127) >> 5)) * 4 + (c8 >> 7)] = (unsigned char)eb;
    };

    auto stage_ln = [&]() {
#ifndef HS_LN_NB
#define HS_LN_NB 4
#endif
        constexpr int TPR = KC / 8, RPP = 256 / TPR, NPASS = BM / RPP, NB = NPASS < HS_LN_NB ? NPASS : HS_LN_NB;
        const float* A = reinterpret_cast<const float*>(p.A);
        const int c8 = (tid % TPR) * 8;
        const int lnw = p.ln_width ? p.ln_width : p.K;
        const bool cok = c8 < p.K, cv = c8 < lnw;
        float g[8], bt[8];
#pragma unroll
        for (int e = 0; e < 8; ++e) { g[e] = cv ? p.gamma[c8 + e] : 0.f; bt[e] = cv ? p.beta[c8 + e] : 0.f; }
        const float invk = 1.f / (float)lnw;
        for (int pb = 0; pb < NPASS; pb += NB) {
            float f[NB][8];
#pragma unroll
            for (int i = 0; i < NB; ++i) {
                const int r = tid / TPR + (pb + i) * RPP;
                const int row = min(row0 + r, p.M - 1);
                float4 x0 = make_float4(0.f, 0.f, 0.f, 0.f), x1 = x0;
                if (cv) {
                    x0 = *reinterpret_cast<const float4*>(A + (size_t)row * p.lda + c8);
                    x1 = *reinterpret_cast<const float4*>(A + (size_t)row * p.lda + c8 + 4);
                }
                f[i][0] = x0.x; f[i][1] = x0.y; f[i][2] = x0.z; f[i][3] = x0.w;
                f[i][4] = x1.x; f[i][5] = x1.y; f[i][6] = x1.z; f[i][7] = x1.w;
            }
#pragma unroll
            for (int i = 0; i < NB; ++i) {
                const int r = tid / TPR + (pb + i) * RPP;
                float sm = 0.f;
#pragma unroll
                for (int e = 0; e < 8; ++e) sm += f[i][e];
                sm = lanes_sum<TPR>(sm);
                const float mean = sm * invk;
                float q = 0.f;
#pragma unroll
                for (int e = 0; e < 8; ++e) { const float dl = cv ? f[i][e] - mean : 0.f; q += dl * dl; }
                q = lanes_sum<TPR>(q);
                const float rstd = rsqrtf(q * invk + 1e-5f);
#pragma unroll
                for (int e = 0; e < 8; ++e) f[i][e] = (f[i][e] - mean) * rstd * g[e] + bt[e];
                const bf16x8 val = cv ? cvt8(f[i]) : zero8();
                if (cok && p.u_out && row0 + r < p.M)
                    HS_NT(true, reinterpret_cast<bf16x8*>(p.u_out + (size_t)(row0 + r) * p.ldu + c8), val);
                if constexpr (F8) {
                    if (!cv) {
#pragma unroll
                        for (int e = 0; e < 8; ++e) f[i][e] = 0.f;
                    }
                    put_a8(r, c8, f[i]);
                } else {
                    *reinterpret_cast<bf16x8*>(As + r * LDA + c8) = val;
                }
            }
        }
    };

    auto stage = [&](int kc) {
        constexpr int TPR = KC / 8;
        constexpr int RPP = 256 / TPR;
        const int c8 = (tid % TPR) * 8;
        const int kcol = kc * KC + c8;
#pragma unroll 4
        for (int r = tid / TPR; r < BM; r += RPP) {
            const int row = min(row0 + r, p.M - 1);
            bf16x8 val = zero8();
            float f[8] = {0.f, 0.f, 0.f, 0.f, 0.f, 0.f, 0.f, 0.f};
            if (kcol < p.K) {
                if constexpr (AK == A_BF16) {
                    const bf16_t* A = reinterpret_cast<const bf16_t*>(p.A);
                    val = *reinterpret_cast<const bf16x8*>(A + (size_t)row * p.lda + kcol);
                    if constexpr (F8) {
#pragma unroll
                        for (int i = 0; i < 8; ++i) f[i] = bf2f(val[i]);
                    }
                } else {
                    const float* A = reinterpret_cast<const float*>(p.A);
                    const float4 x0 = *reinterpret_cast<const float4*>(A + (size_t)row * p.lda + kcol);
                    const float4 x1 = *reinterpret_cast<const float4*>(A + (size_t)row * p.lda + kcol + 4);
                    f[0] = x0.x; f[1] = x0.y; f[2] = x0.z; f[3] = x0.w; f[4] = x1.x; f[5] = x1.y; f[6] = x1.z; f[7] = x1.w;
                    if constexpr (AK == A_F32) {
                        if (p.a_rowscale) {
                            const float rs = p.a_rowscale[row];
#pragma unroll
                            for (int i = 0; i < 8; ++i) f[i] *= rs;
                        }
                    }
                    if constexpr (AK == A_F32_LN) {
                        const float mean = rstat[2 * r], rstd = rstat[2 * r + 1];
                        const float4 g0 = *reinterpret_cast<const float4*>(p.gamma + kcol);
                        const float4 g1 = *reinterpret_cast<const float4*>(p.gamma + kcol + 4);
                        const float4 b0 = *reinterpret_cast<const float4*>(p.beta + kcol);
                        const float4 b1 = *reinterpret_cast<const float4*>(p.beta + kcol + 4);
                        const float g[8] = {g0.x, g0.y, g0.z, g0.w, g1.x, g1.y, g1.z, g1.w};
                        const float b[8] = {b0.x, b0.y, b0.z, b0.w, b1.x, b1.y, b1.z, b1.w};
#pragma unroll
                        for (int i = 0; i < 8; ++i) f[i] = (f[i] - mean) * rstd * g[i] + b[i];
                    }
                    val = cvt8(f);
                    if constexpr (AK == A_F32_LN) {
                        if (p.u_out && row0 + r < p.M)
                            HS_NT(true, reinterpret_cast<bf16x8*>(p.u_out + (size_t)(row0 + r) * p.ldu + kcol), val);
                    }
                }
            }
            if constexpr (F8) put_a8(r, c8, f);
            else *reinterpret_cast<bf16x8*>(As + r * LDA + c8) = val;
        }
    };

    constexpr int NPF = (NCH > 1 && AK == A_BF16) ? BM * KC / 8 / 256 : 1;
    auto stage_load = [&](int kc, bf16x8 (&pre)[NPF]) {
        constexpr int TPR = KC / 8, RPP = 256 / TPR;
        const int kcol = kc * KC + (tid % TPR) * 8;
        const bf16_t* A = reinterpret_cast<const bf16_t*>(p.A);
#pragma unroll
        for (int i = 0; i < NPF; ++i) {
            const int row = min(row0 + tid / TPR + i * RPP, p.M - 1);
            pre[i] = zero8();
            if (kcol < p.K) pre[i] = *reinterpret_cast<const bf16x8*>(A + (size_t)row * p.lda + kcol);
        }
    };
    auto stage_store = [&](const bf16x8 (&pre)[NPF]) {
        constexpr int TPR = KC / 8, RPP = 256 / TPR;
        const int c8 = (tid % TPR) * 8;
#pragma unroll
        for (int i = 0; i < NPF; ++i) {
            const int r = tid / TPR + i * RPP;
            if constexpr (F8) {
                float f[8];
#pragma unroll
                for (int e = 0; e < 8; ++e) f[e] = bf2f(pre[i][e]);
                put_a8(r, c8, f);
            } else {
                *reinterpret_cast<bf16x8*>(As + r * LDA + c8) = pre[i];
            }
        }
    };

    const int arow = lane & 15, ag = lane >> 4;

#ifndef HS_G_F8_128
#define HS_G_F8_128 2
#endif
#ifndef HS_G_BF_128
#define HS_G_BF_128 4
#endif
#ifndef HS_G_F8_64
#define HS_G_F8_64 2
#endif
    constexpr int G = F8 ? (BM == 128 ? HS_G_F8_128 : HS_G_F8_64)
#ifndef HS_G_BF_LN
#define HS_G_BF_LN 4
#endif
                         : (DUAL ? 2 : (AK == A_F32_LN ? HS_G_BF_LN : (BM == 128 ? HS_G_BF_128 : 4)));
    constexpr int KSTEP = F8 ? 128 : 32;
    using Frag = typename std::conditional<F8 != 0, i32x8, bf16x8>::type;
    struct Grp { Frag b[G][2]; Frag b2[DUAL ? G : 1][2]; unsigned sb[2]; unsigned sb2[2]; };
    auto fetch = [&](int nc_, int kc_, int gb_, Grp& gr) {
        const int ks0_ = kc_ * (KC / KSTEP);
        const int nks_ = min(KC / KSTEP, KS_total - ks0_);
#pragma unroll
        for (int i = 0; i < G; ++i)
#pragma unroll
            for (int j = 0; j < 2; ++j) {
                const int nt = nc_ * 8 + wave * 2 + j, ks = gb_ + i;
                const bool live = nc_ < n_chunks && ks < nks_ && nt < NT_total;
                if constexpr (F8) {
                    i32x8 z = {0, 0, 0, 0, 0, 0, 0, 0};
                    gr.b[i][j] = z;
                    if constexpr (DUAL) gr.b2[i][j] = z;
                    if (live) {
                        const size_t off = (((size_t)nt * KS_total + ks0_ + ks) * 64 + lane) * 32;
                        const int4 lo = *reinterpret_cast<const int4*>(p.W8 + off), hi = *reinterpret_cast<const int4*>(p.W8 + off + 16);
                        gr.b[i][j] = i32x8{lo.x, lo.y, lo.z, lo.w, hi.x, hi.y, hi.z, hi.w};
                        if constexpr (DUAL) {
                            const int4 l2 = *reinterpret_cast<const int4*>(p.W8b + off), h2 = *reinterpret_cast<const int4*>(p.W8b + off + 16);
                            gr.b2[i][j] = i32x8{l2.x, l2.y, l2.z, l2.w, h2.x, h2.y, h2.z, h2.w};
                        }
                    }
                } else {
                    if (live) {
                        const size_t off = (((size_t)nt * KS_total + ks0_ + ks) * 64 + lane) * 8;
                        gr.b[i][j] = *reinterpret_cast<const bf16x8*>(p.W + off);
                        if constexpr (DUAL) gr.b2[i][j] = *reinterpret_cast<const bf16x8*>(p.W2 + off);
                    } else {
                        gr.b[i][j] = zero8();
                        if constexpr (DUAL) gr.b2[i][j] = zero8();
                    }
                }
            }
        if constexpr (F8) {
#pragma unroll
            for (int j = 0; j < 2; ++j) {
                const int nt = nc_ * 8 + wave * 2 + j;
                const bool live = nc_ < n_chunks && kc_ < k_chunks && nt < NT_total;
                const size_t so = (((size_t)nt * k_chunks + kc_) * 64 + lane) * 4;
                gr.sb[j] = live ? *reinterpret_cast<const unsigned*>(p.S8 + so) : 0u;
                gr.sb2[j] = 0u;
                if constexpr (DUAL) gr.sb2[j] = live ? *reinterpret_cast<const unsigned*>(p.S8b + so) : 0u;
            }
        }
    };
    Grp cur;
    fetch(0, 0, 0, cur);
    PH_DECL

    auto mma = [&](f32x4 (&acc)[MT][2], f32x4 (&acc2)[DUAL ? MT : 1][2], const Grp& cur, int gb, int nks, const unsigned (&sa)[F8 ? MT : 1]) {
#pragma unroll
                for (int i = 0; i < G; ++i) {
                    const int ks = gb + i;
                    if (ks < nks) {
                        if constexpr (F8) {
                            const int sh = 8 * ks;
                            const int sb0 = (int)(cur.sb[0] >> sh), sb1 = (int)(cur.sb[1] >> sh);
                            const int tb0 = (int)(cur.sb2[0] >> sh), tb1 = (int)(cur.sb2[1] >> sh);
#pragma unroll
                            for (int mt = 0; mt < MT; ++mt) {
                                const unsigned char* ap = As8 + (mt * 16 + arow) * LDA + ks * 128 + ag * 16;
                                const int4 lo = *reinterpret_cast<const int4*>(ap), hi = *reinterpret_cast<const int4*>(ap + 64);
                                const i32x8 a = {lo.x, lo.y, lo.z, lo.w, hi.x, hi.y, hi.z, hi.w};
                                const int sam = (int)(sa[mt] >> sh);
                                acc[mt][0] = __builtin_amdgcn_mfma_scale_f32_16x16x128_f8f6f4(a, cur.b[i][0], acc[mt][0], 0, 0, 0, sam, 0, sb0);
                                acc[mt][1] = __builtin_amdgcn_mfma_scale_f32_16x16x128_f8f6f4(a, cur.b[i][1], acc[mt][1], 0, 0, 0, sam, 0, sb1);
                                if constexpr (DUAL) {
                                    acc2[mt][0] = __builtin_amdgcn_mfma_scale_f32_16x16x128_f8f6f4(a, cur.b2[i][0], acc2[mt][0], 0, 0, 0, sam, 0, tb0);
                                    acc2[mt][1] = __builtin_amdgcn_mfma_scale_f32_16x16x128_f8f6f4(a, cur.b2[i][1], acc2[mt][1], 0, 0, 0, sam, 0, tb1);
                                }
                            }
                        } else {
#pragma unroll
                            for (int mt = 0; mt < MT; ++mt) {
                                const bf16x8 a = *reinterpret_cast<const bf16x8*>(As + (mt * 16 + arow) * LDA + ks * 32 + ag * 8);
#pragma unroll
                                for (int j = 0; j < 2; ++j) {
                                    acc[mt][j] = mfma16(a, cur.b[i][j], acc[mt][j]);
                                    if constexpr (DUAL) acc2[mt][j] = mfma16(a, cur.b2[i][j], acc2[mt][j]);
                                }
                            }
                        }
                    }
                }
    };

    auto epilogue = [&](int nc, f32x4 (&acc)[MT][2], f32x4 (&acc2)[DUAL ? MT : 1][2]) {
        const int ccols = min(128, p.N - nc * 128);
        if constexpr (EPI == E_LN_BWD) {
            const int c8 = (tid & 15) * 8;
            float gm[8], dgam[8], dbet[8];
#pragma unroll
            for (int e = 0; e < 8; ++e) { gm[e] = p.gamma[c8 + e]; dgam[e] = 0.f; dbet[e] = 0.f; }
#pragma unroll
            for (int ps = 0; ps < BM / PR; ++ps) {
                constexpr int NPC = PR * 16 / 256;
                __builtin_amdgcn_sched_barrier(0);
                float xr[NPC][8], rs[NPC][8];
#pragma unroll
                for (int i = 0; i < NPC; ++i) {
                    const int row = row0 + ps * PR + ((tid + 256 * i) >> 4);
#pragma unroll
                    for (int e = 0; e < 8; ++e) { xr[i][e] = 0.f; rs[i][e] = 0.f; }
                    if (row < p.M) {
                        const float* xp = p.lnx + (size_t)row * p.ldr + c8;
                        const float* rp = p.res + (size_t)row * p.ldr + c8;
                        const float4 a0 = *reinterpret_cast<const float4*>(xp), a1 = *reinterpret_cast<const float4*>(xp + 4);
                        const float4 r0 = *reinterpret_cast<const float4*>(rp), r1 = *reinterpret_cast<const float4*>(rp + 4);
                        xr[i][0] = a0.x; xr[i][1] = a0.y; xr[i][2] = a0.z; xr[i][3] = a0.w;
                        xr[i][4] = a1.x; xr[i][5] = a1.y; xr[i][6] = a1.z; xr[i][7] = a1.w;
                        rs[i][0] = r0.x; rs[i][1] = r0.y; rs[i][2] = r0.z; rs[i][3] = r0.w;
                        rs[i][4] = r1.x; rs[i][5] = r1.y; rs[i][6] = r1.z; rs[i][7] = r1.w;
                        if (p.accumulate) {
                            const float* op = reinterpret_cast<const float*>(p.out) + (size_t)row * p.ldo + c8;
                            const float4 o0 = *reinterpret_cast<const float4*>(op), o1 = *reinterpret_cast<const float4*>(op + 4);
                            rs[i][0] += o0.x; rs[i][1] += o0.y; rs[i][2] += o0.z; rs[i][3] += o0.w;
                            rs[i][4] += o1.x; rs[i][5] += o1.y; rs[i][6] += o1.z; rs[i][7] += o1.w;
                        }
                    }
                }
                lds_barrier();
#pragma unroll
                for (int mi = 0; mi < PR / 16; ++mi)
#pragma unroll
                    for (int j = 0; j < 2; ++j)
#pragma unroll
                        for (int r = 0; r < 4; ++r)
                            T1[(mi * 16 + ag * 4 + r) * TS + wave * 32 + j * 16 + arow] = acc[ps * (PR / 16) + mi][j][r];
                lds_barrier();
#pragma unroll
                for (int i = 0; i < NPC; ++i) {
                    const int rl = (tid + 256 * i) >> 4;
                    const int row = row0 + ps * PR + rl;
                    const float4 t0 = *reinterpret_cast<const float4*>(T1 + rl * TS + c8);
                    const float4 t1 = *reinterpret_cast<const float4*>(T1 + rl * TS + c8 + 4);
                    const float du[8] = {t0.x, t0.y, t0.z, t0.w, t1.x, t1.y, t1.z, t1.w};
                    float sm = 0.f;
#pragma unroll
                    for (int e = 0; e < 8; ++e) sm += xr[i][e];
                    sm = lanes_sum<16>(sm);
                    const float mean = sm * (1.f / 128.f);
                    float q = 0.f;
#pragma unroll
                    for (int e = 0; e < 8; ++e) { xr[i][e] -= mean; q += xr[i][e] * xr[i][e]; }
                    q = lanes_sum<16>(q);
                    const float rstd = rsqrtf(q * (1.f / 128.f) + 1e-5f);
                    float a = 0.f, b = 0.f, t[8];
#pragma unroll
                    for (int e = 0; e < 8; ++e) { xr[i][e] *= rstd; t[e] = du[e] * gm[e]; a += t[e]; b += t[e] * xr[i][e]; }
                    a = lanes_sum<16>(a); b = lanes_sum<16>(b);
                    a *= (1.f / 128.f); b *= (1.f / 128.f);
                    if (row < p.M) {
                        float v[8];
#pragma unroll
                        for (int e = 0; e < 8; ++e) {
                            v[e] = rs[i][e] + rstd * (t[e] - a - xr[i][e] * b);
                            dgam[e] += du[e] * xr[i][e];
                            dbet[e] += du[e];
                        }
                        float* op = reinterpret_cast<float*>(p.out) + (size_t)row * p.ldo + c8;
                        *reinterpret_cast<float4*>(op) = make_float4(v[0], v[1], v[2], v[3]);
                        *reinterpret_cast<float4*>(op + 4) = make_float4(v[4], v[5], v[6], v[7]);
                    }
                }
            }
            lds_barrier();
            float* red = T1;
#pragma unroll
            for (int e = 0; e < 8; ++e) { red[tid * 8 + e] = dgam[e]; red[2048 + tid * 8 + e] = dbet[e]; }
            lds_barrier();
            {
                const int which = tid >> 7, c = tid & 127, o8 = c >> 3, e = c & 7;
                float sacc = 0.f;
                for (int t2 = o8; t2 < 256; t2 += 16) sacc += red[which * 2048 + t2 * 8 + e];
                hs_gadd(HsDet{p.det_base, reinterpret_cast<long long*>(p.det_acc)}, (which ? p.dbeta : p.dgamma) + c, sacc);
            }
            PH(2)
            return;
        }
#pragma unroll
        for (int ps = 0; ps < BM / PR; ++ps) {
            lds_barrier();
#pragma unroll
            for (int mi = 0; mi < PR / 16; ++mi)
#pragma unroll
                for (int j = 0; j < 2; ++j)
#pragma unroll
                    for (int r = 0; r < 4; ++r) {
                        const int o = (mi * 16 + ag * 4 + r) * TS + wave * 32 + j * 16 + arow;
                        T1[o] = acc[ps * (PR / 16) + mi][j][r];
                        if constexpr (DUAL) T2[o] = acc2[ps * (PR / 16) + mi][j][r];
                    }
            lds_barrier();
#pragma unroll
            for (int i = 0; i < PR * 16 / 256; ++i) {
                const int piece = tid + 256 * i;
                const int rl = piece >> 4, c8 = (piece & 15) * 8;
                const int row = row0 + ps * PR + rl;
                const int col = nc * 128 + c8;
                if (row >= p.M || c8 >= ccols) continue;
                const float4 t0 = *reinterpret_cast<const float4*>(T1 + rl * TS + c8);
                const float4 t1 = *reinterpret_cast<const float4*>(T1 + rl * TS + c8 + 4);
                float v[8] = {t0.x, t0.y, t0.z, t0.w, t1.x, t1.y, t1.z, t1.w};
                const int nv = p.n_valid - col;
                const bool cvalid = nv > 0;
                if (p.bias && cvalid) {
                    if (nv >= 8) {
                        const float4 b0 = *reinterpret_cast<const float4*>(p.bias + col);
                        const float4 b1 = *reinterpret_cast<const float4*>(p.bias + col + 4);
                        v[0] += b0.x; v[1] += b0.y; v[2] += b0.z; v[3] += b0.w;
                        v[4] += b1.x; v[5] += b1.y; v[6] += b1.z; v[7] += b1.w;
                    } else {
#pragma unroll
                        for (int e = 0; e < 8; ++e) if (e < nv) v[e] += p.bias[col + e];
                    }
                }
                if constexpr (EPI == E_BF16) {
                    if (nv < 8) {
#pragma unroll
                        for (int e = 0; e < 8; ++e) if (e >= nv) v[e] = 0.f;
                    }
                    *reinterpret_cast<bf16x8*>(reinterpret_cast<bf16_t*>(p.out) + (size_t)row * p.ldo + col) = cvt8(v);
                } else if constexpr (EPI == E_F32 || EPI == E_RES_F32 || EPI == E_POS_F32) {
                    if (!cvalid) continue;
                    if constexpr (EPI == E_RES_F32) {
                        if (p.out_rowscale) {
                            const float rs = p.out_rowscale[row];
#pragma unroll
                            for (int e = 0; e < 8; ++e) v[e] *= rs;
                        }
                        const float* rp = p.res + (size_t)row * p.ldr + col;
                        const float4 r0 = *reinterpret_cast<const float4*>(rp), r1 = *reinterpret_cast<const float4*>(rp + 4);
                        v[0] += r0.x; v[1] += r0.y; v[2] += r0.z; v[3] += r0.w;
                        v[4] += r1.x; v[5] += r1.y; v[6] += r1.z; v[7] += r1.w;
                        if (p.res2) {
                            const float* qp = p.res2 + (size_t)row * p.ldr + col;
                            const float4 q0 = *reinterpret_cast<const float4*>(qp), q1 = *reinterpret_cast<const float4*>(qp + 4);
                            v[0] += q0.x; v[1] += q0.y; v[2] += q0.z; v[3] += q0.w;
                            v[4] += q1.x; v[5] += q1.y; v[6] += q1.z; v[7] += q1.w;
                        }
                    } else if constexpr (EPI == E_POS_F32) {
                        const float* rp = p.pos + (size_t)p.ids[row] * p.ldpos + col;
                        const float4 r0 = *reinterpret_cast<const float4*>(rp), r1 = *reinterpret_cast<const float4*>(rp + 4);
                        v[0] += r0.x; v[1] += r0.y; v[2] += r0.z; v[3] += r0.w;
                        v[4] += r1.x; v[5] += r1.y; v[6] += r1.z; v[7] += r1.w;
                    }
                    float* op = reinterpret_cast<float*>(p.out) + (size_t)row * p.ldo + col;
                    *reinterpret_cast<float4*>(op) = make_float4(v[0], v[1], v[2], v[3]);
                    *reinterpret_cast<float4*>(op + 4) = make_float4(v[4], v[5], v[6], v[7]);
                } else if constexpr (EPI == E_SWIGLU) {
                    const float4 s0 = *reinterpret_cast<const float4*>(T2 + rl * TS + c8);
                    const float4 s1 = *reinterpret_cast<const float4*>(T2 + rl * TS + c8 + 4);
                    float w[8] = {s0.x, s0.y, s0.z, s0.w, s1.x, s1.y, s1.z, s1.w};
                    if (p.bias2 && cvalid) {
                        if (nv >= 8) {
                            const float4 b0 = *reinterpret_cast<const float4*>(p.bias2 + col);
                            const float4 b1 = *reinterpret_cast<const float4*>(p.bias2 + col + 4);
                            w[0] += b0.x; w[1] += b0.y; w[2] += b0.z; w[3] += b0.w;
                            w[4] += b1.x; w[5] += b1.y; w[6] += b1.z; w[7] += b1.w;
                        } else {
#pragma unroll
                            for (int e = 0; e < 8; ++e) if (e < nv) w[e] += p.bias2[col + e];
                        }
                    }
#pragma unroll
                    for (int e = 0; e < 8; ++e) if (e >= nv) { v[e] = 0.f; w[e] = 0.f; }
                    const bf16x8 h1 = cvt8(v), h3 = cvt8(w);
                    HS_NT(true, reinterpret_cast<bf16x8*>(p.h13 + (size_t)row * p.ldh + col), h1);
                    HS_NT(true, reinterpret_cast<bf16x8*>(p.h13 + (size_t)row * p.ldh + p.hoff + col), h3);
                    float g[8];
#pragma unroll
                    for (int e = 0; e < 8; ++e) {
                        const float a1 = bf2f(h1[e]), a3 = bf2f(h3[e]);
                        g[e] = silu_nr(a1) * a3;
                    }
                    *reinterpret_cast<bf16x8*>(reinterpret_cast<bf16_t*>(p.out) + (size_t)row * p.ldo + col) = cvt8(g);
                } else if constexpr (EPI == E_SWIGLU_BWD) {
                    const bf16x8 h1 = *reinterpret_cast<const bf16x8*>(p.h13 + (size_t)row * p.ldh + col);
                    const bf16x8 h3 = *reinterpret_cast<const bf16x8*>(p.h13 + (size_t)row * p.ldh + p.hoff + col);
                    float d1[8], d3[8];
#pragma unroll
                    for (int e = 0; e < 8; ++e) {
                        const float a1 = bf2f(h1[e]), a3 = bf2f(h3[e]);
                        const float s = __builtin_amdgcn_rcpf(1.f + __expf(-a1));
                        d1[e] = v[e] * a3 * s * (1.f + a1 * (1.f - s));
                        d3[e] = v[e] * a1 * s;
                    }
                    bf16_t* o = reinterpret_cast<bf16_t*>(p.out);
                    *reinterpret_cast<bf16x8*>(o + (size_t)row * p.ldo + col) = cvt8(d1);
                    *reinterpret_cast<bf16x8*>(o + (size_t)row * p.ldo + p.hoff + col) = cvt8(d3);
                }
            }
        }
        PH(2)
    };

    auto epilogue_ln_ko = [&](f32x4 (&accs)[NCH][MT][2]) {
        if constexpr (EPI == E_LN_BWD && NCH > 1) {
            constexpr int PRL = 16;
            constexpr int NW = 128 * NCH;
            float* TT = T1;
            float dgam[NCH][8], dbet[NCH][8];
#pragma unroll
            for (int c = 0; c < NCH; ++c)
#pragma unroll
                for (int e = 0; e < 8; ++e) { dgam[c][e] = 0.f; dbet[c][e] = 0.f; }
            const int c8 = (tid & 15) * 8, rl = tid >> 4;
            float gm[NCH][8];
#pragma unroll
            for (int c = 0; c < NCH; ++c)
#pragma unroll
                for (int e = 0; e < 8; ++e) gm[c][e] = p.gamma[c * 128 + c8 + e];
            const float invn = 1.f / (float)NW;
#pragma unroll
            for (int ps = 0; ps < BM / PRL; ++ps) {
                __builtin_amdgcn_sched_barrier(0);
                const int row = row0 + ps * PRL + rl;
                const bool rok = row < p.M;
                float xr[NCH][8];
#pragma unroll
                for (int c = 0; c < NCH; ++c) {
#pragma unroll
                    for (int e = 0; e < 8; ++e) xr[c][e] = 0.f;
                    if (rok) {
                        const float* xp = p.lnx + (size_t)row * p.ldr + c * 128 + c8;
                        const float4 a0 = *reinterpret_cast<const float4*>(xp), a1 = *reinterpret_cast<const float4*>(xp + 4);
                        xr[c][0] = a0.x; xr[c][1] = a0.y; xr[c][2] = a0.z; xr[c][3] = a0.w;
                        xr[c][4] = a1.x; xr[c][5] = a1.y; xr[c][6] = a1.z; xr[c][7] = a1.w;
                    }
                }
                lds_barrier();
#pragma unroll
                for (int c = 0; c < NCH; ++c)
#pragma unroll
                    for (int j = 0; j < 2; ++j)
#pragma unroll
                        for (int r = 0; r < 4; ++r)
                            TT[(c * PRL + ag * 4 + r) * TS + wave * 32 + j * 16 + arow] = accs[c][ps][j][r];
                lds_barrier();
                float sm = 0.f;
#pragma unroll
                for (int c = 0; c < NCH; ++c)
#pragma unroll
                    for (int e = 0; e < 8; ++e) sm += xr[c][e];
                sm = lanes_sum<16>(sm);
                const float mean = sm * invn;
                float q = 0.f;
#pragma unroll
                for (int c = 0; c < NCH; ++c)
#pragma unroll
                    for (int e = 0; e < 8; ++e) { xr[c][e] -= mean; q += xr[c][e] * xr[c][e]; }
                q = lanes_sum<16>(q);
                const float rstd = rsqrtf(q * invn + 1e-5f);
                float a = 0.f, b = 0.f;
#pragma unroll
                for (int c = 0; c < NCH; ++c) {
                    const float4 t0 = *reinterpret_cast<const float4*>(TT + (c * PRL + rl) * TS + c8);
                    const float4 t1 = *reinterpret_cast<const float4*>(TT + (c * PRL + rl) * TS + c8 + 4);
                    const float du[8] = {t0.x, t0.y, t0.z, t0.w, t1.x, t1.y, t1.z, t1.w};
#pragma unroll
                    for (int e = 0; e < 8; ++e) {
                        xr[c][e] *= rstd;
                        const float t = du[e] * gm[c][e];
                        a += t; b += t * xr[c][e];
                        if (rok) { dgam[c][e] += du[e] * xr[c][e]; dbet[c][e] += du[e]; }
                    }
                }
                a = lanes_sum<16>(a); b = lanes_sum<16>(b);
                a *= invn; b *= invn;
                if (rok) {
#pragma unroll
                    for (int c = 0; c < NCH; ++c) {
                        const float4 t0 = *reinterpret_cast<const float4*>(TT + (c * PRL + rl) * TS + c8);
                        const float4 t1 = *reinterpret_cast<const float4*>(TT + (c * PRL + rl) * TS + c8 + 4);
                        const float du[8] = {t0.x, t0.y, t0.z, t0.w, t1.x, t1.y, t1.z, t1.w};
                        const float* rp = p.res + (size_t)row * p.ldr + c * 128 + c8;
                        const float4 r0 = *reinterpret_cast<const float4*>(rp), r1 = *reinterpret_cast<const float4*>(rp + 4);
                        float v[8] = {r0.x, r0.y, r0.z, r0.w, r1.x, r1.y, r1.z, r1.w};
                        float* op = reinterpret_cast<float*>(p.out) + (size_t)row * p.ldo + c * 128 + c8;
                        if (p.accumulate) {
                            const float4 o0 = *reinterpret_cast<const float4*>(op), o1 = *reinterpret_cast<const float4*>(op + 4);
                            v[0] += o0.x; v[1] += o0.y; v[2] += o0.z; v[3] += o0.w; v[4] += o1.x; v[5] += o1.y; v[6] += o1.z; v[7] += o1.w;
                        }
#pragma unroll
                        for (int e = 0; e < 8; ++e) v[e] += rstd * (du[e] * gm[c][e] - a - xr[c][e] * b);
                        *reinterpret_cast<float4*>(op) = make_float4(v[0], v[1], v[2], v[3]);
                        *reinterpret_cast<float4*>(op + 4) = make_float4(v[4], v[5], v[6], v[7]);
                        if (p.u_out) *reinterpret_cast<bf16x8*>(p.u_out + (size_t)row * p.ldu + c * 128 + c8) = cvt8(v);
                    }
                }
            }
            const HsDet det{p.det_base, reinterpret_cast<long long*>(p.det_acc)};
            float* red = T1;
#pragma unroll
            for (int c = 0; c < NCH; ++c) {
                lds_barrier();
#pragma unroll
                for (int e = 0; e < 8; ++e) { red[tid * 8 + e] = dgam[c][e]; red[2048 + tid * 8 + e] = dbet[c][e]; }
                lds_barrier();
                const int which = tid >> 7, col = tid & 127, o8 = col >> 3, e = col & 7;
                float sacc = 0.f;
                for (int t2 = o8; t2 < 256; t2 += 16) sacc += red[which * 2048 + t2 * 8 + e];
                hs_gadd(det, (which ? p.dbeta : p.dgamma) + c * 128 + col, sacc);
            }
        }
    };

    if constexpr (NCH == 1) {
    for (int nc = 0; nc < n_chunks; ++nc) {
        f32x4 acc[MT][2];
        f32x4 acc2[DUAL ? MT : 1][2];
#pragma unroll
        for (int mt = 0; mt < MT; ++mt)
#pragma unroll
            for (int j = 0; j < 2; ++j) {
                acc[mt][j] = f32x4{0.f, 0.f, 0.f, 0.f};
                if constexpr (DUAL) acc2[mt][j] = f32x4{0.f, 0.f, 0.f, 0.f};
            }
        for (int kc = 0; kc < k_chunks; ++kc) {
            if (k_chunks > 1 || nc == 0) {
                if (!(nc == 0 && kc == 0)) lds_barrier();
                if constexpr (AK == A_F32_LN) stage_ln(); else stage(kc);
                lds_barrier();
                PH(0)
            }
            const int ks0 = kc * (KC / KSTEP);
            const int nks = min(KC / KSTEP, KS_total - ks0);
            unsigned sa[F8 ? MT : 1];
            if constexpr (F8) {
#pragma unroll
                for (int mt = 0; mt < MT; ++mt) sa[mt] = *reinterpret_cast<const unsigned*>(Sc + ((mt * 16 + arow) * 4 + ag) * 4);
            }
            for (int gb = 0; gb < nks; gb += G) {
                int nnc = nc, nkc = kc, ngb = gb + G;
                if (ngb >= nks) { ngb = 0; if (++nkc >= k_chunks) { nkc = 0; ++nnc; } }
                Grp nxt;
                fetch(nnc, nkc, ngb, nxt);
                mma(acc, acc2, cur, gb, nks, sa);
                cur = nxt;
            }
        }
        PH(1)
        epilogue(nc, acc, acc2);
    }
    } else {
        static_assert(NCH == 1 || !DUAL, "the gate pair keeps one accumulator set");
        f32x4 accs[NCH][MT][2];
        f32x4 acc2[1][2];
#pragma unroll
        for (int c = 0; c < NCH; ++c)
#pragma unroll
            for (int mt = 0; mt < MT; ++mt)
#pragma unroll
                for (int j = 0; j < 2; ++j) accs[c][mt][j] = f32x4{0.f, 0.f, 0.f, 0.f};
        bf16x8 pre[NPF];
        if constexpr (AK == A_BF16) stage_load(0, pre);
        for (int kc = 0; kc < k_chunks; ++kc) {
            if (kc) lds_barrier();
            if constexpr (AK == A_BF16) stage_store(pre); else stage(kc);
            lds_barrier();
            if constexpr (AK == A_BF16) {
                if (kc + 1 < k_chunks) stage_load(kc + 1, pre);
            }
            PH(0)
            const int ks0 = kc * (KC / KSTEP);
            const int nks = min(KC / KSTEP, KS_total - ks0);
            unsigned sa[F8 ? MT : 1];
            if constexpr (F8) {
#pragma unroll
                for (int mt = 0; mt < MT; ++mt) sa[mt] = *reinterpret_cast<const unsigned*>(Sc + ((mt * 16 + arow) * 4 + ag) * 4);
            }
#pragma unroll
            for (int c = 0; c < NCH; ++c) {
                if (c < n_chunks) {
                    for (int gb = 0; gb < nks; gb += G) {
                        int nnc = c, nkc = kc, ngb = gb + G;
                        if (ngb >= nks) { ngb = 0; if (++nnc >= n_chunks) { nnc = 0; ++nkc; } }
                        Grp nxt;
                        fetch(nnc, nkc, ngb, nxt);
                        mma(accs[c], acc2, cur, gb, nks, sa);
                        cur = nxt;
                    }
                }
            }
        }
        PH(1)
        if constexpr (EPI == E_LN_BWD) {
            epilogue_ln_ko(accs);
        } else {
#pragma unroll
            for (int c = 0; c < NCH; ++c)
                if (c < n_chunks) epilogue(c, accs[c], acc2);
        }
    }
    PH_FLUSH(((AK * 3 + (EPI == E_LN_BWD ? 2 : (EPI == E_BF16 ? 0 : 1))) * 4) % 64)
}

template <int AK, int EPI, int KC, int BM, int F8 = 0, int NCH = 1>
int launch(const GemmParams& p, hipStream_t s) {
    const int grid = (p.M + BM - 1) / BM;
    const size_t abytes = F8 ? (size_t)BM * (KC + 16) + BM * 16 : (size_t)BM * (KC + 8) * 2;
    size_t tiles = (EPI == E_SWIGLU ? 2 : 1) * EpiRows<KC, F8, BM>::v * TS * sizeof(float);
    if (EPI == E_LN_BWD && NCH > 1) tiles = std::max(tiles, (size_t)NCH * 16 * TS * sizeof(float));
    const size_t lds = abytes + BM * 2 * sizeof(float) + tiles;
    static bool attr_set = false;
    if (!attr_set) {
        (void)hipFuncSetAttribute(reinterpret_cast<const void*>(gemm_kernel<AK, EPI, KC, BM, F8, NCH>),
                                  hipFuncAttributeMaxDynamicSharedMemorySize, (int)lds);
        attr_set = true;
    }
    hipLaunchKernelGGL((gemm_kernel<AK, EPI, KC, BM, F8, NCH>), dim3(grid), dim3(256), lds, s, p);
    return (int)hipGetLastError();
}

static int wide_mode() { return 1; }
static thread_local int g_force_bm = 0, g_force_kc = 0;
static int ko_bm() { return 0; }
static bool k_outer() { return true; }
static bool small_weights(const GemmParams& p, bool dual) {
    const int64_t nk = (int64_t)p.N * p.K;
    if (p.K < 256) return false;
    if (dual) return nk <= 400 * 1024;
    return p.K <= 512 ? nk <= 800 * 1024 : nk <= 400 * 1024;
}

template <int AK, int EPI>
int launch_f8(const GemmParams& p, hipStream_t s) {
    if constexpr (EPI == E_LN_BWD || EPI == E_POS_F32) {
        return HS_EUNSUPPORTED;
    } else {
        if (!p.W8 || !p.S8 || (EPI == E_SWIGLU && (!p.W8b || !p.S8b))) return HSIMAE_ENULL;
        if (AK == A_F32_LN && p.K > 512) return HS_EUNSUPPORTED;
        const int64_t nk = (int64_t)p.N * p.K * (EPI == E_SWIGLU ? 2 : 1);
        bool bm64 = true;
        (void)nk;
        if (g_force_bm) bm64 = g_force_bm == 64;
        if constexpr (AK != A_F32_LN && EPI != E_SWIGLU) {
            if (k_outer() && p.K > 512 && p.N > 128 && p.N <= 512 && g_force_bm != 128) {
                if constexpr (AK == A_BF16) {
                    if (ko_bm() != 64) return p.N <= 256 ? launch<AK, EPI, 512, 32, 1, 2>(p, s) : launch<AK, EPI, 512, 32, 1, 4>(p, s);
                }
                return p.N <= 256 ? launch<AK, EPI, 512, 64, 1, 2>(p, s) : launch<AK, EPI, 512, 64, 1, 4>(p, s);
            }
        }
        return bm64 ? launch<AK, EPI, 512, 64, 1>(p, s) : launch<AK, EPI, 512, 128, 1>(p, s);
    }
}

template <int AK, int EPI>
int launch_kc(const GemmParams& p, hipStream_t s) {
    if (p.prec == HSIMAE_PREC_FP8) return launch_f8<AK, EPI>(p, s);
    bool bm64 = wide_mode() && small_weights(p, EPI == E_SWIGLU);
    if (g_force_bm) bm64 = g_force_bm == 64;
    if constexpr (AK == A_F32_LN) {
        if (p.K <= 128) return launch<AK, EPI, 128, 128>(p, s);
        if (p.K <= 256) return bm64 ? launch<AK, EPI, 256, 64>(p, s) : launch<AK, EPI, 256, 128>(p, s);
        if (p.K <= 512) return bm64 ? launch<AK, EPI, 512, 64>(p, s) : launch<AK, EPI, 512, 128>(p, s);
        return HS_EUNSUPPORTED;
    } else if constexpr (EPI == E_LN_BWD) {
        return launch<AK, EPI, 128, 128>(p, s);
    } else {
        const bool kc256 = g_force_kc ? g_force_kc == 256 : (bm64 && p.K >= 256 && p.K <= 1024);
        if constexpr (EPI != E_SWIGLU && EPI != E_SWIGLU_BWD) {
            if (k_outer() && !g_force_bm && p.K > 256 && p.N > 128 && p.N <= 512) {
                if constexpr (AK == A_BF16) {
                    if (ko_bm() == 32) return p.N <= 256 ? launch<AK, EPI, 256, 32, 0, 2>(p, s) : launch<AK, EPI, 256, 32, 0, 4>(p, s);
                }
                return p.N <= 256 ? launch<AK, EPI, 256, 64, 0, 2>(p, s) : launch<AK, EPI, 256, 64, 0, 4>(p, s);
            }
        }
        if (kc256) return bm64 ? launch<AK, EPI, 256, 64>(p, s) : launch<AK, EPI, 256, 128>(p, s);
        return bm64 ? launch<AK, EPI, 128, 64>(p, s) : launch<AK, EPI, 128, 128>(p, s);
    }
}

}

int hs_gemm(const GemmParams& p, int akind, int epi, hipStream_t s);
int hs_gemm_tiled(const GemmParams& p, int akind, int epi, int bm, int kc, hipStream_t s) {
    if ((bm != 0 && bm != 64 && bm != 128) || (kc != 0 && kc != 128 && kc != 256)) return HS_EDIMS;
    g_force_bm = bm; g_force_kc = kc;
    const int rc = hs_gemm(p, akind, epi, s);
    g_force_bm = 0; g_force_kc = 0;
    return rc;
}

int hs_gemm(const GemmParams& p, int akind, int epi, hipStream_t s) {
    if (p.M <= 0) return HS_OK;
    if (p.K % 32 || p.N % 16 || p.lda % 8 || p.ldo % 8) return HS_EDIMS;
    if ((epi == E_F32 || epi == E_RES_F32 || epi == E_POS_F32) && p.n_valid % 8) return HS_EDIMS;
    if (akind == A_F32_LN && (p.ln_width < 0 || p.ln_width % 8 || p.ln_width > p.K)) return HS_EDIMS;
#define CASE(AK, EP) \
    if (akind == AK && epi == EP) return launch_kc<AK, EP>(p, s);
    CASE(A_F32_LN, E_BF16)
    CASE(A_F32_LN, E_SWIGLU)
    CASE(A_F32_LN, E_F32)
    CASE(A_BF16, E_RES_F32)
    CASE(A_BF16, E_POS_F32)
    CASE(A_BF16, E_F32)
    CASE(A_BF16, E_BF16)
    if (akind == A_BF16 && epi == E_LN_BWD && p.N == 512) {
        if (p.n_valid != p.N || !p.lnx || !p.res || !p.gamma || !p.dgamma || !p.dbeta || p.ldr % 4 || p.ldo % 4) return HS_EUNSUPPORTED;
        if (p.prec == HSIMAE_PREC_FP8) {
            if (!p.W8 || !p.S8) return HSIMAE_ENULL;
            return launch<A_BF16, E_LN_BWD, 512, 32, 1, 4>(p, s);
        }
        return launch<A_BF16, E_LN_BWD, 256, 32, 0, 4>(p, s);
    }
    if (akind == A_BF16 && epi == E_LN_BWD && p.N == 256) {
        if (p.n_valid != p.N || !p.lnx || !p.res || !p.gamma || !p.dgamma || !p.dbeta || p.ldr % 4 || p.ldo % 4) return HS_EUNSUPPORTED;
        if (p.prec == HSIMAE_PREC_FP8) {
            if (!p.W8 || !p.S8) return HSIMAE_ENULL;
            return ko_bm() != 64 ? launch<A_BF16, E_LN_BWD, 512, 32, 1, 2>(p, s) : launch<A_BF16, E_LN_BWD, 512, 64, 1, 2>(p, s);
        }
        return ko_bm() == 32 ? launch<A_BF16, E_LN_BWD, 256, 32, 0, 2>(p, s) : launch<A_BF16, E_LN_BWD, 256, 64, 0, 2>(p, s);
    }
    if (akind == A_BF16 && epi == E_LN_BWD) {
        if (p.prec == HSIMAE_PREC_FP8) return HS_EUNSUPPORTED;
        if (p.N != 128 || p.n_valid != 128 || !p.lnx || !p.res || !p.gamma || !p.dgamma || !p.dbeta || p.ldr % 4 || p.ldo % 4)
            return HS_EUNSUPPORTED;
        if (p.u_out) return HS_EUNSUPPORTED;
        return launch_kc<A_BF16, E_LN_BWD>(p, s);
    }
    CASE(A_F32, E_SWIGLU_BWD)
    CASE(A_F32, E_BF16)
    CASE(A_F32, E_F32)
#undef CASE
    return HS_EUNSUPPORTED;
}

HS_UNIT_VARIANT_BITS(gemm)
```

hsimae_amd/csrc/kernels.h:

```cpp
#pragma once
#include "common.h"
#include "../../include/hsimae_hip.h"

enum AKind { A_BF16 = HSIMAE_A_BF16, A_F32 = HSIMAE_A_F32, A_F32_LN = HSIMAE_A_F32_LN };
enum Epi { E_BF16 = HSIMAE_E_BF16, E_F32 = HSIMAE_E_F32, E_RES_F32 = HSIMAE_E_RES_F32,
           E_POS_F32 = HSIMAE_E_POS_F32, E_SWIGLU = HSIMAE_E_SWIGLU, E_SWIGLU_BWD = HSIMAE_E_SWIGLU_BWD,
           E_LN_BWD = HSIMAE_E_LN_BWD };

typedef hsimae_gemm_params GemmParams;
typedef hsimae_pack_desc PackDesc;
typedef hsimae_attn_params AttnParams;
typedef hsimae_wgrad_task WgradTask;
typedef hsimae_wgrad_params WgradParams;
typedef hsimae_lnbwd_params LnBwdParams;
typedef hsimae_mask_params MaskParams;
typedef hsimae_patch_params PatchParams;
typedef hsimae_assemble_params AssembleParams;
typedef hsimae_loss_params LossParams;
typedef hsimae_cube_params CubeParams;
typedef hsimae_scene_params SceneParams;

int hs_gemm(const GemmParams& p, int akind, int epi, hipStream_t s);
int hs_gemm_tiled(const GemmParams& p, int akind, int epi, int bm, int kc, hipStream_t s);
int hs_pack(const PackDesc* descs_dev, int ndesc, int max_elems, hipStream_t s);
int hs_attn_fwd(const AttnParams& p, hipStream_t s);
int hs_attn_bwd(const AttnParams& p, hipStream_t s);
bool hs_attn_proj_fusable(const AttnParams& p);
int hs_wgrad(const WgradParams& p, hipStream_t s);
int hs_ln_bwd(const LnBwdParams& p, hipStream_t s);
int hs_ln_fwd(const float* x, const float* gamma, const float* beta, float* out, int M, int d, hipStream_t s, int ldx = 0, int ldo = 0);
int hs_mask(const MaskParams& p, hipStream_t s);
int hs_patch_gather(const PatchParams& p, hipStream_t s);
int hs_assemble_fwd(const AssembleParams& p, hipStream_t s);
int hs_assemble_bwd(const AssembleParams& p, hipStream_t s);
int hs_loss(const LossParams& p, hipStream_t s);
int hs_loss_partials(int N, int T);
int hs_cube_gather(const CubeParams& p, hipStream_t s);
int hs_scene_windows(const SceneParams& p, hipStream_t s);
int hs_class_argmax(const SceneParams& p, const float* logits, int ld, int num_class, int first, int64_t* map, hipStream_t s);
int64_t hs_gwpca_workspace_bytes(const hsimae_gwpca_params& p);
int hs_gwpca_fit(const hsimae_gwpca_params& p, void* workspace, hipStream_t s);
int hs_gwpca_apply(const hsimae_gwpca_params& p, void* out, int out_f64, hipStream_t s);
int hs_agg_pool(const float* latent, float* pooled, int N, int T, int L, int D, hipStream_t s);
int hs_head_bwd(const float* g, const float* pooled, const float* w, float* gw, float* gb, float* dlat, int N, int C, int T, int L,
                int D, hipStream_t s);
int hs_rows_to_bf16(const float* src, hs_bf16* dst, int64_t rows, int d, const float* rowscale, hipStream_t s);
int hs_rows_pad_bf16(const float* src, hs_bf16* dst, int64_t rows, int cols, int ldd, hipStream_t s);
int hs_det_convert(const int64_t* acc, float* g, int64_t n, hipStream_t s);
int hs_add2(const float* a, const float* b, float* out, int64_t n, hipStream_t s);

struct DecBlockPtrs {
    const float *n1w, *n1b, *bqkv, *pb, *n2w, *n2b, *w1b, *w3b, *w2b;
    const bf16_t *qkv, *p, *w1, *w3, *w2, *qkvT, *pT, *w13T, *w2T;
    const float *qf, *kf, *vf, *pf, *w1f, *w3f;
    int h;
};
struct DecBlockGrads {
    float *n1w, *n1b, *qw, *qb, *kw, *kb, *vw, *vb, *pw, *pb, *n2w, *n2b, *w1w, *w1b, *w2w, *w2b, *w3w, *w3b;
    HsDet det;
};
bool hs_dec_fused_supported(int d, int heads, int hidden, int Ts);
int hs_dec_block_fwd(const float* x, float* x1, float* x2, hs_bf16* o, float* lse, int nsamples, int Ts,
                     const DecBlockPtrs& bp, hipStream_t s);
int hs_dec_attn_fwd(const float* x, float* x1, hs_bf16* o, float* lse, int nsamples, int Ts, const DecBlockPtrs& bp, hipStream_t s);
constexpr long long kDecSlabFloats = HSIMAE_DEC_BLOCK_SLAB_FLOATS;
int hs_dec_block_bwd(const float* x, const float* x1, const float* dy, float* dx1_tmp, float* dx, const hs_bf16* o,
                     const float* lse, int nsamples, int Ts, const DecBlockPtrs& bp, const DecBlockGrads& g, hipStream_t s,
                     float* slab = nullptr);

struct EncMlpPtrs {
    const float *n2w, *n2b, *w1b, *w3b, *w2b;
    const bf16_t *w1, *w3, *w2, *w2T, *w13T;
    int h;
};
bool hs_attn_block_fusable(int d, int heads, int Ts);
bool hs_attn_block_bwd_fusable(int d, int heads, int Ts);
int hs_attn_block_bwd(const hs_bf16* qkv, const hs_bf16* u, const hs_bf16* wqkv, const float* bqkv, const hs_bf16* o, const float* lse,
                      const hs_bf16* dx1b, const float* dx1, const float* x, const float* gamma, const hs_bf16* wpT, const hs_bf16* wqkvT,
                      hs_bf16* dqkv, float* dx, float* dgamma, float* dbeta, const float* det_base, long long* det_acc, int Ts,
                      int nsamples, int mode, int len_l, int accumulate, hipStream_t s);
int hs_attn_block_fwd(const float* x, const float* n1w, const float* n1b, const hs_bf16* wqkv, const float* bqkv, const hs_bf16* wp,
                      const float* pb, hs_bf16* u, hs_bf16* qkv, hs_bf16* o, float* lse, float* x1, const float* rowscale, int Ts,
                      int nsamples, int mode, int len_l, hipStream_t s);
bool hs_attn_block256_fusable(int d, int heads, int Ts, int nsamples);
int hs_attn_block256_fwd(const float* x, const float* n1w, const float* n1b, const hs_bf16* wqkv, const float* bqkv, const hs_bf16* wp,
                         const float* pb, hs_bf16* u, hs_bf16* qkv, hs_bf16* o, float* lse, float* x1, const float* rowscale, int Ts,
                         int nsamples, int mode, int len_l, hipStream_t s);
bool hs_attn_block256_bwd_fusable(int d, int heads, int Ts, int nsamples);
int hs_attn_block256_bwd(const hs_bf16* qkv, const float* lse, const hs_bf16* dx1b, const float* dx1, const float* x, const float* gamma,
                         const hs_bf16* wpT, const hs_bf16* wqkvT, hs_bf16* dqkv, float* dx, float* dgamma, float* dbeta,
                         const float* det_base, long long* det_acc, int Ts, int nsamples, int mode, int len_l, int accumulate,
                         hipStream_t s);
bool hs_enc_mlp_fused_supported(int d, int hidden);
int hs_enc_mlp_fwd(const float* x1, const float* res2, float* x2, int M, int d, const EncMlpPtrs& b, hipStream_t s,
                   const float* rowscale = nullptr);
int hs_enc_mlp_bwd(const float* x1, const float* dy, float* dx1, hs_bf16* u2, hs_bf16* dh13, hs_bf16* g, hs_bf16* dyb,
                   hs_bf16* dx1b, int M, int d, const EncMlpPtrs& b, float* g_n2w, float* g_n2b, hipStream_t s,
                   const float* rs_mlp = nullptr, const float* rs_attn = nullptr, HsDet det = HsDet{nullptr, nullptr}, int plane_rows = 0);

int hs_adamw(float* p, const float* g, float* m, float* v, const unsigned char* group, int64_t n, float lr, float b1, float b2,
             float eps, float wd, int step, hipStream_t s);
```

hsimae_amd/csrc/plan.h:

```cpp
#pragma once
#include "../../include/hsimae_hip.h"
#include <algorithm>
#include <cstdint>
#include <cstdlib>
#include <cstring>
#include <vector>

namespace hsplan {

typedef hsimae_pack_desc PackDesc;
constexpr int LOSS_ROWS_PER_WG = 32;
inline int loss_partials(int N, int T) {
    const int64_t M = (int64_t)N * T * 9;
    return (int)std::max<int64_t>((M + LOSS_ROWS_PER_WG - 1) / LOSS_ROWS_PER_WG, N);
}

inline int rup(int x, int m) { return (x + m - 1) / m * m; }

struct BlkOff { int64_t n1w, n1b, qw, qb, kw, kb, vw, vb, pw, pb, n2w, n2b, w1w, w1b, w2w, w2b, w3w, w3b, end; };

struct Geo {
    int B, T, TL, D, H, hd, h, hp, Dd, Hd, hdd, hdec, hpd, depth, sdepth, nfus, ddepth, norm_pix, prec;
    int Dp, Ddp;
    bool has_axis, has_fus;
};

inline int make_geo(const hsimae_config* c, Geo& g) {
    if (!c) return HSIMAE_ENULL;
    if (c->bands <= 0 || c->bands % 8) return HSIMAE_EDIMS;
    g.B = c->bands; g.T = c->bands / 8; g.TL = g.T * 9;
    g.D = c->embed_dim; g.H = c->num_heads; g.Dd = c->dec_dim; g.Hd = c->dec_heads;
    if (g.D <= 0 || g.Dd <= 0 || g.H <= 0 || g.Hd <= 0 || g.D % g.H || g.Dd % g.Hd) return HSIMAE_EDIMS;
    g.hd = g.D / g.H; g.hdd = g.Dd / g.Hd;
    g.h = c->hidden; g.hdec = c->dec_hidden; g.hp = rup(g.h, 32); g.hpd = rup(g.hdec, 32);
    g.depth = c->depth; g.sdepth = c->s_depth; g.ddepth = c->dec_depth;
    g.has_axis = g.sdepth > 0;
    g.has_fus = g.sdepth < 12;
    g.nfus = g.has_fus ? std::max(0, g.depth - g.sdepth) : 0;
    g.norm_pix = c->norm_pix_loss;
    g.prec = c->precision;
    if (g.prec != HSIMAE_PREC_BF16 && g.prec != HSIMAE_PREC_FP8) return HSIMAE_EUNSUPPORTED;
    if (g.D % 8 || g.Dd % 8 || g.D > 512 || g.Dd > 512) return HSIMAE_EUNSUPPORTED;
    g.Dp = rup(g.D, 32); g.Ddp = rup(g.Dd, 32);
    if ((g.hd != 8 && g.hd != 16) || (g.hdd != 8 && g.hdd != 16)) return HSIMAE_EUNSUPPORTED;
    if (g.h <= 0 || g.hdec <= 0 || g.h % 4 || g.hdec % 4 || g.T > 64 || g.ddepth < 1) return HSIMAE_EUNSUPPORTED;
    return HSIMAE_OK;
}

struct PLayout {
    int64_t pos, mask_token, dpos, pew, peb, nw, nb, dew, deb, dnw, dnb, dpw, dpb, total;
    std::vector<BlkOff> b1, b2, bf, bd;
    std::vector<int64_t> offs, sizes;
};

inline void make_playout(const Geo& g, PLayout& L) {
    int64_t cur = 0;
    auto add = [&](int64_t n) { int64_t o = cur; L.offs.push_back(o); L.sizes.push_back(n); cur += n; return o; };
    auto blk = [&](int d, int h) {
        BlkOff b;
        b.n1w = add(d); b.n1b = add(d);
        b.qw = add((int64_t)d * d); b.qb = add(d);
        b.kw = add((int64_t)d * d); b.kb = add(d);
        b.vw = add((int64_t)d * d); b.vb = add(d);
        b.pw = add((int64_t)d * d); b.pb = add(d);
        b.n2w = add(d); b.n2b = add(d);
        b.w1w = add((int64_t)h * d); b.w1b = add(h);
        b.w2w = add((int64_t)d * h); b.w2b = add(d);
        b.w3w = add((int64_t)h * d); b.w3b = add(h);
        b.end = cur;
        return b;
    };
    L.pos = add((int64_t)g.TL * g.D);
    L.mask_token = add(g.Dd);
    L.dpos = add((int64_t)g.TL * g.Dd);
    L.pew = add((int64_t)g.D * 72);
    L.peb = add(g.D);
    if (g.has_axis) {
        for (int i = 0; i < g.sdepth; ++i) L.b1.push_back(blk(g.D, g.h));
        for (int i = 0; i < g.sdepth; ++i) L.b2.push_back(blk(g.D, g.h));
    }
    for (int i = 0; i < g.nfus; ++i) L.bf.push_back(blk(g.D, g.h));
    L.nw = add(g.D); L.nb = add(g.D);
    L.dew = add((int64_t)g.Dd * g.D); L.deb = add(g.Dd);
    for (int i = 0; i < g.ddepth; ++i) L.bd.push_back(blk(g.Dd, g.hdec));
    L.dnw = add(g.Dd); L.dnb = add(g.Dd);
    L.dpw = add((int64_t)72 * g.Dd); L.dpb = add(72);
    L.total = cur;
}

struct Img8 { int64_t w, s; };
struct BlkW {
    int64_t qkv, p, w1, w3, w2, qkvT, pT, w13T, w2T; int64_t bqkv;
    Img8 qkv8, p8, w1_8, w3_8, w2_8, qkvT8, pT8, w13T8, w2T8;
};
struct WLayout {
    int64_t pe, de, deT, dp, dpT;
    std::vector<BlkW> b1, b2, bf, bd;
    int64_t bf16_elems;
    int64_t f32_elems;
    int64_t fp8_bytes;
    int64_t total_elems;
};

inline void make_wlayout(const Geo& g, WLayout& W) {
    int64_t cur = 0, fcur = 0, cur8 = 0;
    auto img = [&](int N, int K) { int64_t o = cur; cur += (int64_t)N * K; return o; };
    auto img8 = [&](int N, int K) {
        const int64_t nt = (N + 15) / 16, ks = (K + 127) / 128, kch = (ks + 3) / 4;
        Img8 o; o.w = cur8; cur8 += nt * ks * 64 * 32; o.s = cur8; cur8 += nt * kch * 64 * 4;
        return o;
    };
    auto blk = [&](int d, int hp, bool f8) {
        BlkW b; std::memset(&b, 0, sizeof(b));
        b.qkv = img(3 * d, d); b.p = img(d, d); b.w1 = img(hp, d); b.w3 = img(hp, d); b.w2 = img(d, hp);
        b.qkvT = img(d, 3 * d); b.pT = img(d, d); b.w13T = img(d, 2 * hp); b.w2T = img(hp, d);
        b.bqkv = fcur; fcur += 3 * d;
        if (f8) {
            b.qkv8 = img8(3 * d, d); b.p8 = img8(d, d); b.w1_8 = img8(hp, d); b.w3_8 = img8(hp, d); b.w2_8 = img8(d, hp);
            b.qkvT8 = img8(d, 3 * d); b.pT8 = img8(d, d); b.w13T8 = img8(d, 2 * hp); b.w2T8 = img8(hp, d);
        }
        return b;
    };
    const bool f8 = g.prec == HSIMAE_PREC_FP8;
    W.pe = img(g.Dp, 96);
    if (g.has_axis) {
        for (int i = 0; i < g.sdepth; ++i) W.b1.push_back(blk(g.Dp, g.hp, f8));
        for (int i = 0; i < g.sdepth; ++i) W.b2.push_back(blk(g.Dp, g.hp, f8));
    }
    for (int i = 0; i < g.nfus; ++i) W.bf.push_back(blk(g.Dp, g.hp, f8));
    W.de = img(g.Ddp, g.Dp); W.deT = img(g.Dp, g.Ddp);
    for (int i = 0; i < g.ddepth; ++i) W.bd.push_back(blk(g.Ddp, g.hpd, false));
    W.dp = img(80, g.Ddp); W.dpT = img(g.Ddp, 96);
    W.bf16_elems = (cur + 7) & ~7ll;
    W.f32_elems = (fcur + 3) & ~3ll;
    W.fp8_bytes = cur8;
    W.total_elems = W.bf16_elems + 2 * W.f32_elems + (cur8 + 1) / 2;
}

inline void pack_descs(const Geo& g, const PLayout& L, const WLayout& W, const float* P, hs_bf16* wpk,
                std::vector<PackDesc>& out) {
    float* fbase = reinterpret_cast<float*>(wpk + W.bf16_elems);
    unsigned char* base8 = reinterpret_cast<unsigned char*>(fbase + W.f32_elems);
    auto mat = [&](int64_t src, int rows, int cols, int tr, int n_off, int k_off, int K_img, int64_t dst) {
        PackDesc d; std::memset(&d, 0, sizeof(d));
        d.src = P + src; d.rows = rows; d.cols = cols; d.transpose = tr; d.n_off = n_off; d.k_off = k_off;
        d.KS = K_img / 32; d.dst = wpk + dst; out.push_back(d);
    };
    auto mat8 = [&](int64_t src, int rows, int cols, int tr, int n_off, int k_off, int K_img, const Img8& im) {
        PackDesc d; std::memset(&d, 0, sizeof(d));
        d.src = P + src; d.rows = rows; d.cols = cols; d.transpose = tr; d.n_off = n_off; d.k_off = k_off;
        d.KS = (K_img + 127) / 128; d.dst = reinterpret_cast<hs_bf16*>(base8 + im.w); d.fp8 = 1; d.scales = base8 + im.s;
        out.push_back(d);
    };
    auto fcopy = [&](int64_t src, int n, int64_t dst_f, int off) {
        PackDesc d; std::memset(&d, 0, sizeof(d));
        d.src = P + src; d.rows = 1; d.cols = n; d.transpose = 0; d.n_off = off; d.k_off = 0; d.KS = 0;
        d.dst = reinterpret_cast<hs_bf16*>(fbase + dst_f); out.push_back(d);
    };
    auto blk = [&](const BlkOff& b, const BlkW& w, int d, int dp, int h, int hp, bool f8) {
        mat(b.qw, d, d, 0, 0, 0, dp, w.qkv); mat(b.kw, d, d, 0, dp, 0, dp, w.qkv); mat(b.vw, d, d, 0, 2 * dp, 0, dp, w.qkv);
        mat(b.pw, d, d, 0, 0, 0, dp, w.p);
        mat(b.w1w, h, d, 0, 0, 0, dp, w.w1); mat(b.w3w, h, d, 0, 0, 0, dp, w.w3);
        mat(b.w2w, d, h, 0, 0, 0, hp, w.w2);
        mat(b.qw, d, d, 1, 0, 0, 3 * dp, w.qkvT); mat(b.kw, d, d, 1, 0, dp, 3 * dp, w.qkvT); mat(b.vw, d, d, 1, 0, 2 * dp, 3 * dp, w.qkvT);
        mat(b.pw, d, d, 1, 0, 0, dp, w.pT);
        mat(b.w1w, h, d, 1, 0, 0, 2 * hp, w.w13T); mat(b.w3w, h, d, 1, 0, hp, 2 * hp, w.w13T);
        mat(b.w2w, d, h, 1, 0, 0, dp, w.w2T);
        fcopy(b.qb, d, w.bqkv, 0); fcopy(b.kb, d, w.bqkv, dp); fcopy(b.vb, d, w.bqkv, 2 * dp);
        if (f8) {
            mat8(b.qw, d, d, 0, 0, 0, dp, w.qkv8); mat8(b.kw, d, d, 0, dp, 0, dp, w.qkv8); mat8(b.vw, d, d, 0, 2 * dp, 0, dp, w.qkv8);
            mat8(b.pw, d, d, 0, 0, 0, dp, w.p8);
            mat8(b.w1w, h, d, 0, 0, 0, dp, w.w1_8); mat8(b.w3w, h, d, 0, 0, 0, dp, w.w3_8);
            mat8(b.w2w, d, h, 0, 0, 0, hp, w.w2_8);
            mat8(b.qw, d, d, 1, 0, 0, 3 * dp, w.qkvT8); mat8(b.kw, d, d, 1, 0, dp, 3 * dp, w.qkvT8); mat8(b.vw, d, d, 1, 0, 2 * dp, 3 * dp, w.qkvT8);
            mat8(b.pw, d, d, 1, 0, 0, dp, w.pT8);
            mat8(b.w1w, h, d, 1, 0, 0, 2 * hp, w.w13T8); mat8(b.w3w, h, d, 1, 0, hp, 2 * hp, w.w13T8);
            mat8(b.w2w, d, h, 1, 0, 0, dp, w.w2T8);
        }
    };
    mat(L.pew, g.D, 72, 0, 0, 0, 96, W.pe);
    const bool f8 = g.prec == HSIMAE_PREC_FP8;
    for (size_t i = 0; i < L.b1.size(); ++i) blk(L.b1[i], W.b1[i], g.D, g.Dp, g.h, g.hp, f8);
    for (size_t i = 0; i < L.b2.size(); ++i) blk(L.b2[i], W.b2[i], g.D, g.Dp, g.h, g.hp, f8);
    for (size_t i = 0; i < L.bf.size(); ++i) blk(L.bf[i], W.bf[i], g.D, g.Dp, g.h, g.hp, f8);
    mat(L.dew, g.Dd, g.D, 0, 0, 0, g.Dp, W.de); mat(L.dew, g.Dd, g.D, 1, 0, 0, g.Ddp, W.deT);
    for (size_t i = 0; i < L.bd.size(); ++i) blk(L.bd[i], W.bd[i], g.Dd, g.Ddp, g.hdec, g.hpd, false);
    mat(L.dpw, 72, g.Dd, 0, 0, 0, g.Ddp, W.dp); mat(L.dpw, 72, g.Dd, 1, 0, 0, 96, W.dpT);
}

#ifndef HS_PLANE_PAD_ROWS
#define HS_PLANE_PAD_ROWS 48
#endif
constexpr int kPlanePadRows = 64;
static_assert(HS_PLANE_PAD_ROWS <= kPlanePadRows && HS_PLANE_PAD_ROWS % 16 == 0,
              "a -DHS_PLANE_PAD_ROWS variant must stay inside the rows the arena reserves per plane (ADVICE r05)");
struct BlkBuf { hs_bf16* u; hs_bf16* qkv; float* lse; hs_bf16* o; float* x1; hs_bf16* u2; hs_bf16* h13; hs_bf16* g; float* x2; };

struct Scr { float* G1; float* du; hs_bf16* dh13; hs_bf16* dob; hs_bf16* dqkv; hs_bf16* g0b; hs_bf16* g1b; float* slab; };

struct Ws {
    Scr sc, sc2;
    hs_bf16* a_pe; float* x0;
    std::vector<BlkBuf> b1, b2, bf, bd;
    hs_bf16* lat; float* y; float* yfull; hs_bf16* zn; float* pred; hs_bf16* dpred; float* partial;
    float *G0, *G1, *G2, *du; hs_bf16 *dh13, *dob, *dqkv, *dyb;
    float* slab;
    int64_t bytes;
};
constexpr int64_t kSlabBytes = 256ll * 256 * 256 * 4;
inline int64_t slab_bytes(const Geo& g, bool side_stream) {
    if (side_stream) return (g.has_axis && g.Dp >= 256) ? kSlabBytes : 0;
    const int64_t wg = std::max(g.Dp, g.Ddp) >= 256 ? kSlabBytes : 0;
    return std::max<int64_t>(wg, HSIMAE_DEC_BLOCK_SLAB_FLOATS * 4);
}

inline void carve(const Geo& g, int N, int K, char* base, Ws& w) {
    int64_t cur = 0;
    auto take = [&](int64_t bytes) { char* p = base ? base + cur : nullptr; cur += (bytes + 255) & ~255ll; return p; };
    const int64_t Me = (int64_t)N * K, Md = (int64_t)N * g.TL;
    auto blk = [&](int64_t M, int d, int heads, int hp) {
        BlkBuf b;
        b.u = (hs_bf16*)take(M * d * 2); b.qkv = (hs_bf16*)take(M * 3 * d * 2); b.lse = (float*)take(M * heads * 4);
        b.o = (hs_bf16*)take(M * d * 2); b.x1 = (float*)take(M * d * 4); b.u2 = (hs_bf16*)take(M * d * 2);
        b.h13 = (hs_bf16*)take(M * 2 * hp * 2); b.g = (hs_bf16*)take((M + kPlanePadRows) * rup(hp, 64) * 2); b.x2 = (float*)take(M * d * 4);
        return b;
    };
    w.a_pe = (hs_bf16*)take(Me * 96 * 2);
    w.x0 = (float*)take(Me * g.Dp * 4);
    w.b1.clear(); w.b2.clear(); w.bf.clear(); w.bd.clear();
    if (g.has_axis) {
        for (int i = 0; i < g.sdepth; ++i) w.b1.push_back(blk(Me, g.Dp, g.H, g.hp));
        for (int i = 0; i < g.sdepth; ++i) w.b2.push_back(blk(Me, g.Dp, g.H, g.hp));
    }
    for (int i = 0; i < g.nfus; ++i) w.bf.push_back(blk(Me, g.Dp, g.H, g.hp));
    w.lat = (hs_bf16*)take(Me * g.Dp * 2);
    w.y = (float*)take(Me * g.Ddp * 4);
    w.yfull = (float*)take(Md * g.Ddp * 4);
    for (int i = 0; i < g.ddepth; ++i) w.bd.push_back(blk(Md, g.Ddp, g.Hd, g.hpd));
    w.zn = (hs_bf16*)take(Md * g.Ddp * 2);
    w.pred = (float*)take(Md * 72 * 4);
    w.dpred = (hs_bf16*)take(Md * 96 * 2);
    w.partial = (float*)take((int64_t)loss_partials(N, g.T) * 4);
    const int64_t gmax = std::max(Me * g.Dp, Md * g.Ddp);
    w.G0 = (float*)take(gmax * 4); w.G1 = (float*)take(gmax * 4); w.G2 = (float*)take(gmax * 4); w.du = (float*)take(gmax * 4);
    w.dh13 = (hs_bf16*)take(std::max((Me + kPlanePadRows) * 2 * rup(g.hp, 64), (Md + kPlanePadRows) * 2 * rup(g.hpd, 64)) * 2);
    w.dob = (hs_bf16*)take(gmax * 2);
    w.dqkv = (hs_bf16*)take(gmax * 3 * 2);
    w.dyb = (hs_bf16*)take(Me * g.Ddp * 2);
    w.sc.G1 = w.G1; w.sc.du = w.du; w.sc.dh13 = w.dh13; w.sc.dob = w.dob; w.sc.dqkv = w.dqkv;
    w.sc2.G1 = (float*)take(Me * g.Dp * 4); w.sc2.du = (float*)take(Me * g.Dp * 4);
    w.sc2.dh13 = (hs_bf16*)take((Me + kPlanePadRows) * 2 * rup(g.hp, 64) * 2); w.sc2.dob = (hs_bf16*)take(Me * g.Dp * 2);
    w.sc2.dqkv = (hs_bf16*)take(Me * g.Dp * 3 * 2);
    w.sc.g0b = (hs_bf16*)take(gmax * 2); w.sc.g1b = (hs_bf16*)take(gmax * 2);
    w.sc2.g0b = (hs_bf16*)take(Me * g.Dp * 2); w.sc2.g1b = (hs_bf16*)take(Me * g.Dp * 2);
    w.slab = (float*)take(slab_bytes(g, false));
    w.sc.slab = w.slab;
    w.sc2.slab = slab_bytes(g, true) ? (float*)take(slab_bytes(g, true)) : nullptr;
    w.bytes = cur;
}

inline int wgrad_msplit(int tiles, int64_t M, int concurrent = 1) {
    const int chunks = (int)((M + 63) / 64);
    const int budget = 512;
    int ms = std::max(1, budget / std::max(1, concurrent) / std::max(1, tiles));
    if (ms < 8) ms = std::max(1, budget / std::max(1, tiles));
    if (ms >= 8) ms &= ~7;
    return std::max(1, std::min(ms, chunks));
}

inline int param_layout(const hsimae_config* cfg, int64_t* offsets, int64_t* sizes, int max_entries) {
    Geo g; int e = make_geo(cfg, g); if (e) return e;
    PLayout L; make_playout(g, L);
    const int n = (int)L.offs.size();
    for (int i = 0; i < n && i < max_entries; ++i) {
        if (offsets) offsets[i] = L.offs[i];
        if (sizes) sizes[i] = L.sizes[i];
    }
    return n;
}
inline int64_t wpk_elems(const hsimae_config* cfg) {
    Geo g; if (make_geo(cfg, g)) return -1;
    WLayout W; make_wlayout(g, W);
    return W.total_elems;
}
inline int64_t pack_table_bytes(const hsimae_config* cfg) {
    Geo g; if (make_geo(cfg, g)) return -1;
    PLayout L; make_playout(g, L); WLayout W; make_wlayout(g, W);
    std::vector<PackDesc> d; pack_descs(g, L, W, nullptr, nullptr, d);
    return (int64_t)d.size() * sizeof(PackDesc);
}
inline int build_pack_table(const hsimae_config* cfg, const float* params_dev, hs_bf16* wpk_dev, void* table_host) {
    Geo g; int e = make_geo(cfg, g); if (e) return e;
    if (!params_dev || !wpk_dev || !table_host) return HSIMAE_ENULL;
    PLayout L; make_playout(g, L); WLayout W; make_wlayout(g, W);
    std::vector<PackDesc> d; pack_descs(g, L, W, params_dev, wpk_dev, d);
    std::memcpy(table_host, d.data(), d.size() * sizeof(PackDesc));
    return HSIMAE_OK;
}
inline int64_t wgrad_slab_bytes(const hsimae_config* cfg, int32_t side_stream) {
    Geo g; if (make_geo(cfg, g)) return -1;
    return slab_bytes(g, side_stream != 0);
}
inline int64_t workspace_bytes(const hsimae_config* cfg, int32_t N, int32_t len_t, int32_t len_l) {
    Geo g; if (make_geo(cfg, g)) return -1;
    if (N <= 0 || len_t < 1 || len_l < 1) return -1;
    Ws w; carve(g, N, len_t * len_l, nullptr, w);
    return w.bytes;
}

}
```

include/hsimae_hip.h:

```cpp
#ifndef HSIMAE_HIP_H
#define HSIMAE_HIP_H
#include <stdint.h>

#ifdef __HIPCC__
typedef __bf16 hs_bf16;
#else
typedef uint16_t hs_bf16;
#endif

#ifdef __cplusplus
extern "C" {
#endif
#pragma GCC visibility push(default)

#define HSIMAE_OK 0
#define HSIMAE_EDIMS (-1)
#define HSIMAE_EUNSUPPORTED (-2)
#define HSIMAE_EALIGN (-3)
#define HSIMAE_ENULL (-4)
#define HSIMAE_ENOFORWARD (-5)

#define HSIMAE_VERSION 108
int hsimae_version(void);
typedef struct {
    int32_t abi_version; uint32_t variant_bits; uint64_t kernel_source_hash; uint64_t flags_hash; int32_t default_flags; int32_t reserved;
} hsimae_build_info_t;
int hsimae_build_info(hsimae_build_info_t* out);
const char* hsimae_variant_name(int bit);
const char* hsimae_strerror(int code);
int hsimae_two_streams_active(void);

typedef struct {
    int32_t bands;
    int32_t embed_dim;
    int32_t depth;
    int32_t s_depth;
    int32_t num_heads;
    int32_t dec_dim;
    int32_t dec_depth;
    int32_t dec_heads;
    int32_t hidden;
    int32_t dec_hidden;
    int32_t norm_pix_loss;
    int32_t precision;
} hsimae_config;
int hsimae_effective_precision(const hsimae_config* cfg);
enum { HSIMAE_PREC_BF16 = 0, HSIMAE_PREC_FP8 = 1 };

int hsimae_param_layout(const hsimae_config* cfg, int64_t* offsets, int64_t* sizes, int max_entries);

int64_t hsimae_wpk_elems(const hsimae_config* cfg);
int64_t hsimae_pack_table_bytes(const hsimae_config* cfg);
int hsimae_build_pack_table(const hsimae_config* cfg, const float* params_dev, hs_bf16* wpk_dev, void* table_host);
int hsimae_pack_params(const hsimae_config* cfg, const void* table_dev, void* stream);

typedef struct {
    const float* x;
    int64_t sn, sb, sh, sw;
    int32_t N, len_t, len_l;
    const float* noise1;
    const float* noise2;
    const float* params;
    const hs_bf16* wpk;
    void* workspace;
    int64_t workspace_bytes;
    float grad_scale;
    int32_t want_recons;
    float* loss;
    float* pred_img;
    float* mask_img;
    float* mask;
    int32_t* ids_keep;
    int32_t* ids_restore;
    float* latent;
    float* pred;
    const float* drop_scale;
    void* bucket_stream;
    int64_t* det_acc;
} hsimae_io;

int64_t hsimae_workspace_bytes(const hsimae_config* cfg, int32_t N, int32_t len_t, int32_t len_l);
int hsimae_forward(const hsimae_config* cfg, const hsimae_io* io, void* stream);

typedef void (*hsimae_bucket_cb)(int32_t stage, int64_t off, int64_t len, void* user);
int hsimae_backward(const hsimae_config* cfg, const hsimae_io* io, float* grads, hsimae_bucket_cb cb, void* user,
                    void* stream);

typedef struct {
    const float* noise1; const float* noise2; int32_t N, T, L, len_t, len_l;
    int32_t* ids_keep; int32_t* ids_restore; float* mask;
} hsimae_mask_params;
int hsimae_mask_from_noise(const hsimae_mask_params* p, void* stream);

typedef struct {
    const float* x; int64_t sn, sb, sh, sw; int32_t N, T, K; const int32_t* ids_keep;
    hs_bf16* out; int32_t* pos_ids;
} hsimae_patch_params;
int hsimae_patch_gather(const hsimae_patch_params* p, void* stream);

enum { HSIMAE_A_BF16 = 0, HSIMAE_A_F32 = 1, HSIMAE_A_F32_LN = 2 };
enum { HSIMAE_E_BF16 = 0, HSIMAE_E_F32 = 1, HSIMAE_E_RES_F32 = 2, HSIMAE_E_POS_F32 = 3, HSIMAE_E_SWIGLU = 4,
       HSIMAE_E_SWIGLU_BWD = 5,
       HSIMAE_E_LN_BWD = 6 };
typedef struct {
    const void* A; int32_t lda;
    int32_t M, N, K;
    int32_t n_valid;
    const hs_bf16* W; const hs_bf16* W2;
    const float* bias; const float* bias2;
    const float* gamma; const float* beta;
    float* stats;
    hs_bf16* u_out; int32_t ldu;
    void* out; int32_t ldo;
    const float* res; const float* res2; int32_t ldr;
    const float* pos; const int32_t* ids; int32_t ldpos;
    hs_bf16* h13; int32_t ldh; int32_t hoff;
    const float* lnx; float* dgamma; float* dbeta; int32_t accumulate;
    const float* a_rowscale; const float* out_rowscale;
    int32_t prec;
    const uint8_t* W8; const uint8_t* S8; const uint8_t* W8b; const uint8_t* S8b;
    int32_t ln_width;
    const float* det_base; int64_t* det_acc;
} hsimae_gemm_params;
int hsimae_gemm(const hsimae_gemm_params* p, int32_t a_kind, int32_t epilogue, void* stream);
int hsimae_gemm_tiled(const hsimae_gemm_params* p, int32_t a_kind, int32_t epilogue, int32_t bm, int32_t kc, void* stream);

typedef struct {
    const float* src; int32_t rows, cols;
    int32_t transpose;
    int32_t n_off, k_off;
    int32_t KS;
    hs_bf16* dst;
    int32_t fp8;
    uint8_t* scales;
} hsimae_pack_desc;
int hsimae_pack_matrix(const hsimae_pack_desc* desc_dev, int32_t ndesc, int32_t max_elems, void* stream);

typedef struct {
    const float* n2w; const float* n2b; const float* w1b; const float* w3b; const float* w2b;
    const hs_bf16* w1; const hs_bf16* w3; const hs_bf16* w2; const hs_bf16* w2T; const hs_bf16* w13T;
    int32_t hidden;
} hsimae_mlp_weights;
int hsimae_enc_mlp_fwd(const float* x1, const float* res2, float* x2, int32_t M, int32_t d, const hsimae_mlp_weights* w,
                       const float* rowscale, void* stream);
int hsimae_enc_mlp_bwd(const float* x1, const float* dy, float* dx1, hs_bf16* u2, hs_bf16* dh13, hs_bf16* g, hs_bf16* dyb,
                       hs_bf16* dx1b, int32_t M, int32_t d, const hsimae_mlp_weights* w, float* g_n2w, float* g_n2b,
                       const float* rs_mlp, const float* rs_attn, int32_t plane_rows, void* stream);

typedef struct {
    const hs_bf16* qkv; int32_t ld;
    int32_t d, heads, hd;
    int32_t Ts;
    int32_t nsamples;
    int32_t mode, len_l;
    hs_bf16* o; int32_t ldo;
    float* lse;
    const hs_bf16* dout; int32_t lddo;
    hs_bf16* dqkv;
    int32_t kv_off;
} hsimae_attn_params;
int hsimae_attn_fwd(const hsimae_attn_params* p, void* stream);
int hsimae_attn_bwd(const hsimae_attn_params* p, void* stream);

typedef struct {
    const float *n1w, *n1b, *bqkv, *pb;
    const hs_bf16 *qkv, *p, *qkvT, *pT;
} hsimae_attn_block_weights;
int hsimae_attn_block_fwd(const hsimae_attn_block_weights* w, const float* x, hs_bf16* u, hs_bf16* qkv, hs_bf16* o, float* lse,
                          float* x1, const float* rowscale, int32_t d, int32_t heads, int32_t Ts, int32_t nsamples, int32_t mode,
                          int32_t len_l, void* stream);
int hsimae_attn_block_bwd(const hsimae_attn_block_weights* w, const hs_bf16* qkv, const hs_bf16* u, const hs_bf16* o, const float* lse,
                          const hs_bf16* dx1b, const float* dx1, const float* x, hs_bf16* dqkv, float* dx, float* dgamma, float* dbeta,
                          int64_t* det_acc, int32_t accumulate, int32_t d, int32_t heads, int32_t Ts, int32_t nsamples, int32_t mode,
                          int32_t len_l, void* stream);

typedef struct {
    const float *n1w, *n1b, *bqkv, *pb, *n2w, *n2b, *w1b, *w3b, *w2b;
    const hs_bf16 *qkv, *p, *w1, *w3, *w2, *w2T;
    const float *qf, *kf, *vf, *pf, *w1f, *w3f;
    int32_t hidden;
} hsimae_dec_block_weights;
typedef struct {
    float *n1w, *n1b, *qw, *qb, *kw, *kb, *vw, *vb, *pw, *pb, *n2w, *n2b, *w1w, *w1b, *w2w, *w2b, *w3w, *w3b;
} hsimae_dec_block_grads;
int hsimae_dec_block_fwd(const hsimae_dec_block_weights* w, const float* x, float* x1, float* x2, hs_bf16* o, float* lse,
                         int32_t nsamples, int32_t Ts, int32_t split, void* stream);
#define HSIMAE_DEC_BLOCK_SLAB_FLOATS (256ll * (104 * 512 + 2112))
int64_t hsimae_dec_block_slab_floats(void);
int64_t hsimae_wgrad_slab_bytes(const hsimae_config* cfg, int32_t side_stream);
int hsimae_dec_block_bwd(const hsimae_dec_block_weights* w, const hsimae_dec_block_grads* g, const float* x, const float* x1,
                         const float* dy, float* dx1_tmp, float* dx, const hs_bf16* o, const float* lse, int32_t nsamples,
                         int32_t Ts, float* slab, void* stream);

typedef struct {
    const void* dO; int32_t dO_f32; int32_t ldo;
    const hs_bf16* A; int32_t lda;
    int32_t N, K;
    float* dW; int32_t ldw;
    float* db;
    const float* dO_rowscale;
    int32_t dO_plane_rows, A_plane_rows;
} hsimae_wgrad_task;
typedef struct {
    hsimae_wgrad_task t[16]; int32_t ntasks; int32_t M; int32_t msplit;
    const float* det_base; int64_t* det_acc;
    float* slab;
} hsimae_wgrad_params;
int hsimae_wgrad(const hsimae_wgrad_params* p, void* stream);
int32_t hsimae_wgrad_msplit(int32_t tiles, int64_t M);

typedef struct {
    const float* du; const float* x; const float* stats; const float* gamma; const float* dres;
    float* dx; int32_t accumulate; float* dgamma; float* dbeta; int32_t M, d;
    int32_t ld;
    const float* det_base; int64_t* det_acc;
} hsimae_lnbwd_params;
int hsimae_ln_bwd(const hsimae_lnbwd_params* p, void* stream);
int hsimae_ln_fwd(const float* x, const float* gamma, const float* beta, float* out, int32_t M, int32_t d, void* stream);

typedef struct {
    const float* y; int32_t N, K, TL, Dd; const int32_t* ids_restore; const float* pos;
    float* yfull; const float* dyfull; hs_bf16* dy;
    int32_t ld;
} hsimae_assemble_params;
int hsimae_assemble_fwd(const hsimae_assemble_params* p, void* stream);
int hsimae_assemble_bwd(const hsimae_assemble_params* p, void* stream);

typedef struct {
    const float* x; int64_t sn, sb, sh, sw; int32_t N, T; const float* pred; const float* mask;
    int32_t norm_pix; float inv_scale;
    float* partial; float* loss; float sum_mask;
    hs_bf16* dpred; float* pred_img; float* mask_img;
} hsimae_loss_params;
int hsimae_loss_partials(int32_t N, int32_t T);
int hsimae_loss(const hsimae_loss_params* p, void* stream);

int hsimae_adamw_step(float* params, const float* grads, float* exp_avg, float* exp_avg_sq, const uint8_t* group, int64_t n,
                      float lr, float beta1, float beta2, float eps, float weight_decay, int32_t step, void* stream);

int hsimae_encode(const hsimae_config* cfg, const hsimae_io* io, void* stream);
int hsimae_encode_backward(const hsimae_config* cfg, const hsimae_io* io, const float* dlatent, float* grads,
                           hsimae_bucket_cb cb, void* user, void* stream);
int hsimae_agg_pool(const float* latent, float* pooled, int32_t N, int32_t T, int32_t L, int32_t D, void* stream);
int hsimae_head_bwd(const float* g, const float* pooled, const float* w, float* gw, float* gb, float* dlatent, int32_t N, int32_t C,
                    int32_t T, int32_t L, int32_t D, void* stream);
int hsimae_decode(const hsimae_config* cfg, const hsimae_io* io, const float* latent, float* pred, void* stream);
int hsimae_decode_backward(const hsimae_config* cfg, const hsimae_io* io, const float* dpred, float* dlatent, float* grads,
                           hsimae_bucket_cb cb, void* user, void* stream);

typedef struct {
    const void* scenes; int32_t scene_f64; const int64_t* scene_off; const int32_t* scene_w; int32_t bands;
    const int16_t* cut; const int64_t* index; const uint8_t* flips; int32_t N;
    float* out; int64_t sn, sb, sh, sw;
} hsimae_cube_params;
int hsimae_cube_gather(const hsimae_cube_params* p, void* stream);

typedef struct {
    const void* scene; int32_t scene_f64; int32_t H, W, C;
    int64_t p0; const int64_t* pixels; int32_t N;
    float* out; int64_t sn, sb, sh, sw;
} hsimae_scene_params;
int hsimae_scene_windows(const hsimae_scene_params* p, void* stream);
int hsimae_class_argmax(const hsimae_scene_params* p, const float* logits, int32_t ld, int32_t num_class, int32_t first, int64_t* map,
                        void* stream);

typedef struct {
    const void* scene; int32_t scene_f64; int32_t H, W, C;
    int32_t nc, group, whiten;
    double* minmax; double* mean; double* lambda; double* proj; int32_t* group_off;
} hsimae_gwpca_params;
int64_t hsimae_gwpca_workspace_bytes(const hsimae_gwpca_params* p);
int hsimae_gwpca_fit(const hsimae_gwpca_params* p, void* workspace, void* stream);
int hsimae_gwpca_apply(const hsimae_gwpca_params* p, void* out, int32_t out_f64, void* stream);

#pragma GCC visibility pop
#ifdef __cplusplus
}
#endif
#endif
```

Measured before the change: 272,900 patches/s.

## Fuse decoder and encoder final-norm LayerNorm backward into GEMM epilogue, drop stack copy

Adds a no-residual LayerNorm-backward GEMM epilogue, generalized to 64- or 128-wide rows, and uses it to fuse the decoder-pred and decoder-embed backward GEMMs with the following LN backward. This removes two standalone LN-backward kernels and their du round trips through memory. It also replaces the device-to-device copy of the stacked-branch gradient with a separate G3 buffer that the two branches route into. The cost is extra workspace memory and a more complex epilogue with cross-block dgamma/dbeta accumulation.

```diff
diff --git a/hsimae_amd/_lib.py b/hsimae_amd/_lib.py
--- a/hsimae_amd/_lib.py
+++ b/hsimae_amd/_lib.py
@@ -185,7 +185,7 @@
 ABI_VERSION = 108
 PREC_BF16, PREC_FP8 = 0, 1
 A_BF16, A_F32, A_F32_LN = 0, 1, 2
-E_BF16, E_F32, E_RES_F32, E_POS_F32, E_SWIGLU, E_SWIGLU_BWD, E_LN_BWD = 0, 1, 2, 3, 4, 5, 6
+E_BF16, E_F32, E_RES_F32, E_POS_F32, E_SWIGLU, E_SWIGLU_BWD, E_LN_BWD, E_LN_BWD_NORES = 0, 1, 2, 3, 4, 5, 6, 7
 
 _lib = None
 
diff --git a/hsimae_amd/csrc/api.hip b/hsimae_amd/csrc/api.hip
--- a/hsimae_amd/csrc/api.hip
+++ b/hsimae_amd/csrc/api.hip
@@ -56,6 +56,9 @@
     SC_DEC_SLAB = 1u << 12,
     SC_PLANAR = 1u << 13,
     SC_ATTN_BLOCK256_BWD = 1u << 14,
+    SC_DNORM_BWD = 1u << 15,
+    SC_NORM_BWD = 1u << 16,
+    SC_STACK_NOCOPY = 1u << 17,
 };
 uint32_t sched_from_env() {
     auto off = [](const char* name) { const char* e = getenv(name); return e && e[0] == '0'; };
@@ -76,6 +79,9 @@
     if (!off("HSIMAE_DEC_SLAB")) b |= SC_DEC_SLAB;
     if (!off("HSIMAE_WGRAD_PLANAR")) b |= SC_PLANAR;
     if (!off("HSIMAE_FUSED_ATTN_BLOCK256_BWD")) b |= SC_ATTN_BLOCK256_BWD;
+    if (!off("HSIMAE_FUSED_DNORM_BWD")) b |= SC_DNORM_BWD;
+    if (!off("HSIMAE_FUSED_NORM_BWD")) b |= SC_NORM_BWD;
+    if (!off("HSIMAE_STACK_NOCOPY")) b |= SC_STACK_NOCOPY;
     return b;
 }
 struct SchedRec { uint32_t enc = 0, dec = 0; bool has_enc = false, has_dec = false; uint64_t gen = 0; };
@@ -635,6 +641,7 @@
 
 static int encoder_backward(const Ctx& c, const hsimae_io* io, float* grads, hipStream_t s, Emitter& emit, uint32_t sc) {
     const Geo& g = c.g; const float* P = io->params; const Ws& w = c.w; const PLayout& L = c.L;
+    const float* dX = w.G0;
     for (int i = g.nfus - 1; i >= 0; --i) {
         BlkP bp = resolve_enc(g, sc, L.bf[i], c.W.bf[i], P, io->wpk, c.W);
         const float* xin = (i > 0) ? w.bf[i - 1].x2 : (g.has_axis ? w.b2[g.sdepth - 1].x2 : w.x0);
@@ -646,7 +653,10 @@
     if (g.has_axis) {
         Side& sd = side();
         const bool forked = sd.ok && g.sdepth > 1;
-        CK((int)hipMemcpyAsync(w.G2, w.G0, c.Me * g.Dp * 4, hipMemcpyDeviceToDevice, s));
+        const bool nocopy = (sc & SC_STACK_NOCOPY) != 0;
+        float* const X2 = nocopy ? w.G3 : w.G0;
+        if (!nocopy) CK((int)hipMemcpyAsync(w.G2, w.G0, c.Me * g.Dp * 4, hipMemcpyDeviceToDevice, s));
+        dX = X2;
         if (forked) {
             CK((int)hipEventRecord(sd.fork, s));
             CK((int)hipStreamWaitEvent(sd.s, sd.fork, 0));
@@ -658,7 +668,8 @@
             BlkP b2 = resolve_enc(g, sc, L.b2[i], c.W.b2[i], P, io->wpk, c.W);
             const DropRs r1 = drop_rs(io, i, c.Me), r2d = drop_rs(io, g.sdepth + i, c.Me);
             const float* xin2 = (i > 0) ? w.b2[i - 1].x2 : w.x0;
-            CK(block_bwd(b2, sc, L.b2[i], grads, xin2, w.b2[i], c.Me, g.D, g.H, g.h, g.hp, c.K, c.N, 2, c.len_l, w.G0, scr2, w.G0, 0, s2, forked ? 2 : 1,
+            const bool first = nocopy && i == g.sdepth - 1;
+            CK(block_bwd(b2, sc, L.b2[i], grads, xin2, w.b2[i], c.Me, g.D, g.H, g.h, g.hp, c.K, c.N, 2, c.len_l, first ? w.G0 : X2, scr2, X2, 0, s2, forked ? 2 : 1,
                          r2d.a, r2d.m, io->det_acc));
             if (per_block) CK(emit(L.b2[i].n1w, L.b2[i].end, s2));
             if (i == 0 && forked) {
@@ -667,8 +678,8 @@
             }
             BlkP b1 = resolve_enc(g, sc, L.b1[i], c.W.b1[i], P, io->wpk, c.W);
             const float* xin1 = (i > 0) ? w.b1[i - 1].x2 : w.x0;
-            float* out = (i == 0) ? w.G0 : w.G2;
-            CK(block_bwd(b1, sc, L.b1[i], grads, xin1, w.b1[i], c.Me, g.D, g.H, g.h, g.hp, c.K, c.N, 1, c.len_l, w.G2, w.sc, out, i == 0, s, forked ? 2 : 1,
+            float* out = (i == 0) ? X2 : w.G2;
+            CK(block_bwd(b1, sc, L.b1[i], grads, xin1, w.b1[i], c.Me, g.D, g.H, g.h, g.hp, c.K, c.N, 1, c.len_l, first ? w.G0 : w.G2, w.sc, out, i == 0, s, forked ? 2 : 1,
                          r1.a, r1.m, io->det_acc));
             if (per_block) CK(emit(L.b1[i].n1w, L.b1[i].end, s));
         }
@@ -679,7 +690,7 @@
     }
     {
         WgradParams wg; std::memset(&wg, 0, sizeof(wg));
-        WgradTask& t = wg.t[0]; t.dO = w.G0; t.dO_f32 = 1; t.ldo = g.Dp; t.A = w.a_pe; t.lda = 96; t.N = g.D; t.K = 72;
+        WgradTask& t = wg.t[0]; t.dO = dX; t.dO_f32 = 1; t.ldo = g.Dp; t.A = w.a_pe; t.lda = 96; t.N = g.D; t.K = 72;
         t.dW = grads + L.pew; t.ldw = 72; t.db = grads + L.peb;
         wg.det_base = grads; wg.det_acc = io->det_acc;
         wg.ntasks = 1; wg.M = (int)c.Me; wg.msplit = wgrad_msplit((g.D + 127) / 128, c.Me);
@@ -689,12 +700,26 @@
     return HSIMAE_OK;
 }
 
-static int decoder_backward(const Ctx& c, const hsimae_io* io, float* grads, hipStream_t s, Emitter& emit, uint32_t sc) {
+static const float* enc_last_x(const Geo& g, const Ws& w) {
+    return g.nfus ? w.bf[g.nfus - 1].x2 : (g.has_axis ? w.b2[g.sdepth - 1].x2 : w.x0);
+}
+static bool dnorm_bwd_fused(const Geo& g, uint32_t sc) { return (sc & SC_DNORM_BWD) && g.Dd == 64 && g.Ddp == 64; }
+static bool norm_bwd_fused(const Geo& g, uint32_t sc) { return (sc & SC_NORM_BWD) && g.D == 128 && g.Dp == 128; }
+static int decoder_backward(const Ctx& c, const hsimae_io* io, float* grads, hipStream_t s, Emitter& emit, uint32_t sc,
+                            bool through_norm = false) {
     const Geo& g = c.g; const float* P = io->params; const Ws& w = c.w; const PLayout& L = c.L;
     const float* zlast = w.bd[g.ddepth - 1].x2;
+    const bool dn_fused = dnorm_bwd_fused(g, sc);
     GemmParams p = gp();
-    p.A = w.dpred; p.lda = 96; p.M = (int)c.Md; p.N = g.Ddp; p.K = 96; p.n_valid = g.Dd; p.W = io->wpk + c.W.dpT; p.out = w.du; p.ldo = g.Ddp;
-    CK(hs_gemm(p, A_BF16, E_F32, s));
+    p.A = w.dpred; p.lda = 96; p.M = (int)c.Md; p.N = g.Ddp; p.K = 96; p.n_valid = g.Dd; p.W = io->wpk + c.W.dpT;
+    if (dn_fused) {
+        p.out = w.G0; p.ldo = g.Ddp; p.lnx = zlast; p.ldr = g.Ddp; p.gamma = P + L.dnw; p.dgamma = grads + L.dnw; p.dbeta = grads + L.dnb;
+        p.det_base = grads; p.det_acc = io->det_acc;
+        CK(hs_gemm(p, A_BF16, E_LN_BWD_NR, s));
+    } else {
+        p.out = w.du; p.ldo = g.Ddp;
+        CK(hs_gemm(p, A_BF16, E_F32, s));
+    }
     {
         WgradParams wg; std::memset(&wg, 0, sizeof(wg));
         WgradTask& t = wg.t[0]; t.dO = w.dpred; t.dO_f32 = 0; t.ldo = 96; t.A = w.zn; t.lda = g.Ddp; t.N = 72; t.K = g.Dd;
@@ -703,10 +728,12 @@
         wg.ntasks = 1; wg.M = (int)c.Md; wg.msplit = wgrad_msplit(1, c.Md);
         CK(hs_wgrad(wg, s));
     }
-    LnBwdParams l; std::memset(&l, 0, sizeof(l));
-    l.du = w.du; l.x = zlast; l.gamma = P + L.dnw; l.dres = nullptr; l.dx = w.G0; l.dgamma = grads + L.dnw; l.dbeta = grads + L.dnb;
-    l.M = (int)c.Md; l.d = g.Dd; l.ld = g.Ddp; l.det_base = grads; l.det_acc = io->det_acc;
-    CK(hs_ln_bwd(l, s));
+    if (!dn_fused) {
+        LnBwdParams l; std::memset(&l, 0, sizeof(l));
+        l.du = w.du; l.x = zlast; l.gamma = P + L.dnw; l.dres = nullptr; l.dx = w.G0; l.dgamma = grads + L.dnw; l.dbeta = grads + L.dnb;
+        l.M = (int)c.Md; l.d = g.Dd; l.ld = g.Ddp; l.det_base = grads; l.det_acc = io->det_acc;
+        CK(hs_ln_bwd(l, s));
+    }
     CK(emit(L.dnw, L.total, s));
 
     const bool fdec = fused_dec_enabled(g, sc);
@@ -734,8 +761,15 @@
     as.N = c.N; as.K = c.K; as.TL = g.TL; as.Dd = g.Dd; as.ld = g.Ddp; as.ids_restore = io->ids_restore; as.dyfull = w.G0; as.dy = w.dyb;
     CK(hs_assemble_bwd(as, s));
     p = gp();
-    p.A = w.dyb; p.lda = g.Ddp; p.M = (int)c.Me; p.N = g.Dp; p.K = g.Ddp; p.n_valid = g.D; p.W = io->wpk + c.W.deT; p.out = w.du; p.ldo = g.Dp;
-    CK(hs_gemm(p, A_BF16, E_F32, s));
+    p.A = w.dyb; p.lda = g.Ddp; p.M = (int)c.Me; p.N = g.Dp; p.K = g.Ddp; p.n_valid = g.D; p.W = io->wpk + c.W.deT;
+    if (through_norm) {
+        p.out = w.G0; p.ldo = g.Dp; p.lnx = enc_last_x(g, w); p.ldr = g.Dp; p.gamma = P + L.nw; p.dgamma = grads + L.nw; p.dbeta = grads + L.nb;
+        p.det_base = grads; p.det_acc = io->det_acc;
+        CK(hs_gemm(p, A_BF16, E_LN_BWD_NR, s));
+    } else {
+        p.out = w.du; p.ldo = g.Dp;
+        CK(hs_gemm(p, A_BF16, E_F32, s));
+    }
     {
         WgradParams wg; std::memset(&wg, 0, sizeof(wg));
         WgradTask& t = wg.t[0]; t.dO = w.dyb; t.dO_f32 = 0; t.ldo = g.Ddp; t.A = w.lat; t.lda = g.Dp; t.N = g.Dd; t.K = g.D;
@@ -757,12 +791,14 @@
     if (io->det_acc) CK((int)hipMemsetAsync(io->det_acc, 0, (size_t)c.L.total * 8, s));
     const Geo& g = c.g; const float* P = io->params; const Ws& w = c.w; const PLayout& L = c.L;
     Emitter emit{cb, user, cb ? S(io->bucket_stream) : nullptr, 0, grads, io->det_acc};
-    CK(decoder_backward(c, io, grads, s, emit, sc_dec));
-    const float* xf = g.nfus ? w.bf[g.nfus - 1].x2 : (g.has_axis ? w.b2[g.sdepth - 1].x2 : w.x0);
-    LnBwdParams l; std::memset(&l, 0, sizeof(l));
-    l.du = w.du; l.x = xf; l.gamma = P + L.nw; l.dres = nullptr; l.dx = w.G0; l.dgamma = grads + L.nw; l.dbeta = grads + L.nb;
-    l.M = (int)c.Me; l.d = g.D; l.ld = g.Dp; l.det_base = grads; l.det_acc = io->det_acc;
-    CK(hs_ln_bwd(l, s));
+    const bool nfused = norm_bwd_fused(g, sc_dec);
+    CK(decoder_backward(c, io, grads, s, emit, sc_dec, nfused));
+    if (!nfused) {
+        LnBwdParams l; std::memset(&l, 0, sizeof(l));
+        l.du = w.du; l.x = enc_last_x(g, w); l.gamma = P + L.nw; l.dres = nullptr; l.dx = w.G0; l.dgamma = grads + L.nw; l.dbeta = grads + L.nb;
+        l.M = (int)c.Me; l.d = g.D; l.ld = g.Dp; l.det_base = grads; l.det_acc = io->det_acc;
+        CK(hs_ln_bwd(l, s));
+    }
     CK(emit(L.nw, L.deb + g.Dd, s));
     return encoder_backward(c, io, grads, s, emit, sc_enc);
 }
@@ -792,7 +828,7 @@
     hipStream_t s = S(stream);
     if (io->det_acc) CK((int)hipMemsetAsync(io->det_acc, 0, (size_t)c.L.total * 8, s));
     const Geo& g = c.g; const float* P = io->params; const Ws& w = c.w; const PLayout& L = c.L;
-    const float* xf = g.nfus ? w.bf[g.nfus - 1].x2 : (g.has_axis ? w.b2[g.sdepth - 1].x2 : w.x0);
+    const float* xf = enc_last_x(g, w);
     LnBwdParams l; std::memset(&l, 0, sizeof(l));
     const float* dlat = dlatent;
     if (g.Dp != g.D) {
diff --git a/hsimae_amd/csrc/gemm.hip b/hsimae_amd/csrc/gemm.hip
--- a/hsimae_amd/csrc/gemm.hip
+++ b/hsimae_amd/csrc/gemm.hip
@@ -34,7 +34,7 @@
 constexpr int TS = 132;
 
 template <int AK, int EPI, int KC, int BM, int F8, int NCH>
-__global__ __launch_bounds__(256, (EPI == E_LN_BWD || BM <= 64) ? 2 : 1) void gemm_kernel(GemmParams p) {
+__global__ __launch_bounds__(256, (EPI == E_LN_BWD || EPI == E_LN_BWD_NR || BM <= 64) ? 2 : 1) void gemm_kernel(GemmParams p) {
     extern __shared__ __attribute__((aligned(16))) char smem[];
     static_assert(!F8 || KC == 512, "the fp8 path stages 512-deep chunks (one scale dword per row and lane group)");
     static_assert(NCH == 1 || (AK != A_F32_LN && EPI != E_SWIGLU), "k-outer: no LayerNorm prologue, no gate pair");
@@ -324,93 +324,109 @@
 
     auto epilogue = [&](int nc, f32x4 (&acc)[MT][2], f32x4 (&acc2)[DUAL ? MT : 1][2]) {
         const int ccols = min(128, p.N - nc * 128);
-        if constexpr (EPI == E_LN_BWD) {
-            const int c8 = (tid & 15) * 8;
-            float gm[8], dgam[8], dbet[8];
-#pragma unroll
-            for (int e = 0; e < 8; ++e) { gm[e] = p.gamma[c8 + e]; dgam[e] = 0.f; dbet[e] = 0.f; }
-#pragma unroll
-            for (int ps = 0; ps < BM / PR; ++ps) {
-                constexpr int NPC = PR * 16 / 256;
-                __builtin_amdgcn_sched_barrier(0);
-                float xr[NPC][8], rs[NPC][8];
-#pragma unroll
-                for (int i = 0; i < NPC; ++i) {
-                    const int row = row0 + ps * PR + ((tid + 256 * i) >> 4);
-#pragma unroll
-                    for (int e = 0; e < 8; ++e) { xr[i][e] = 0.f; rs[i][e] = 0.f; }
-                    if (row < p.M) {
-                        const float* xp = p.lnx + (size_t)row * p.ldr + c8;
-                        const float* rp = p.res + (size_t)row * p.ldr + c8;
-                        const float4 a0 = *reinterpret_cast<const float4*>(xp), a1 = *reinterpret_cast<const float4*>(xp + 4);
-                        const float4 r0 = *reinterpret_cast<const float4*>(rp), r1 = *reinterpret_cast<const float4*>(rp + 4);
-                        xr[i][0] = a0.x; xr[i][1] = a0.y; xr[i][2] = a0.z; xr[i][3] = a0.w;
-                        xr[i][4] = a1.x; xr[i][5] = a1.y; xr[i][6] = a1.z; xr[i][7] = a1.w;
-                        rs[i][0] = r0.x; rs[i][1] = r0.y; rs[i][2] = r0.z; rs[i][3] = r0.w;
-                        rs[i][4] = r1.x; rs[i][5] = r1.y; rs[i][6] = r1.z; rs[i][7] = r1.w;
-                        if (p.accumulate) {
-                            const float* op = reinterpret_cast<const float*>(p.out) + (size_t)row * p.ldo + c8;
-                            const float4 o0 = *reinterpret_cast<const float4*>(op), o1 = *reinterpret_cast<const float4*>(op + 4);
-                            rs[i][0] += o0.x; rs[i][1] += o0.y; rs[i][2] += o0.z; rs[i][3] += o0.w;
-                            rs[i][4] += o1.x; rs[i][5] += o1.y; rs[i][6] += o1.z; rs[i][7] += o1.w;
+        if constexpr (EPI == E_LN_BWD || EPI == E_LN_BWD_NR) {
+            auto ln_rows = [&](auto lwc) {
+                constexpr int LW = decltype(lwc)::value;
+                constexpr bool RES = EPI == E_LN_BWD;
+                constexpr float INVN = 1.f / (float)(LW * 8);
+                const int c8 = (tid & (LW - 1)) * 8;
+                float gm[8], dgam[8], dbet[8];
+#pragma unroll
+                for (int e = 0; e < 8; ++e) { gm[e] = p.gamma[c8 + e]; dgam[e] = 0.f; dbet[e] = 0.f; }
+#pragma unroll
+                for (int ps = 0; ps < BM / PR; ++ps) {
+                    constexpr int NPC = PR * LW / 256;
+                    static_assert(NPC >= 1, "a pass of PR rows must give every thread a piece");
+                    __builtin_amdgcn_sched_barrier(0);
+                    float xr[NPC][8], rs[NPC][8];
+#pragma unroll
+                    for (int i = 0; i < NPC; ++i) {
+                        const int row = row0 + ps * PR + ((tid + 256 * i) / LW);
+#pragma unroll
+                        for (int e = 0; e < 8; ++e) { xr[i][e] = 0.f; rs[i][e] = 0.f; }
+                        if (row < p.M) {
+                            const float* xp = p.lnx + (size_t)row * p.ldr + c8;
+                            const float4 a0 = *reinterpret_cast<const float4*>(xp), a1 = *reinterpret_cast<const float4*>(xp + 4);
+                            xr[i][0] = a0.x; xr[i][1] = a0.y; xr[i][2] = a0.z; xr[i][3] = a0.w;
+                            xr[i][4] = a1.x; xr[i][5] = a1.y; xr[i][6] = a1.z; xr[i][7] = a1.w;
+                            if constexpr (RES) {
+                                const float* rp = p.res + (size_t)row * p.ldr + c8;
+                                const float4 r0 = *reinterpret_cast<const float4*>(rp), r1 = *reinterpret_cast<const float4*>(rp + 4);
+                                rs[i][0] = r0.x; rs[i][1] = r0.y; rs[i][2] = r0.z; rs[i][3] = r0.w;
+                                rs[i][4] = r1.x; rs[i][5] = r1.y; rs[i][6] = r1.z; rs[i][7] = r1.w;
+                            }
+                            if (p.accumulate) {
+                                const float* op = reinterpret_cast<const float*>(p.out) + (size_t)row * p.ldo + c8;
+                                const float4 o0 = *reinterpret_cast<const float4*>(op), o1 = *reinterpret_cast<const float4*>(op + 4);
+                                rs[i][0] += o0.x; rs[i][1] += o0.y; rs[i][2] += o0.z; rs[i][3] += o0.w;
+                                rs[i][4] += o1.x; rs[i][5] += o1.y; rs[i][6] += o1.z; rs[i][7] += o1.w;
+                            }
                         }
                     }
+                    lds_barrier();
+#pragma unroll
+                    for (int mi = 0; mi < PR / 16; ++mi)
+#pragma unroll
+                        for (int j = 0; j < 2; ++j)
+#pragma unroll
+                            for (int r = 0; r < 4; ++r)
+                                T1[(mi * 16 + ag * 4 + r) * TS + wave * 32 + j * 16 + arow] = acc[ps * (PR / 16) + mi][j][r];
+                    lds_barrier();
+#pragma unroll
+                    for (int i = 0; i < NPC; ++i) {
+                        const int rl = (tid + 256 * i) / LW;
+                        const int row = row0 + ps * PR + rl;
+                        const float4 t0 = *reinterpret_cast<const float4*>(T1 + rl * TS + c8);
+                        const float4 t1 = *reinterpret_cast<const float4*>(T1 + rl * TS + c8 + 4);
+                        const float du[8] = {t0.x, t0.y, t0.z, t0.w, t1.x, t1.y, t1.z, t1.w};
+                        float sm = 0.f;
+#pragma unroll
+                        for (int e = 0; e < 8; ++e) sm += xr[i][e];
+                        sm = lanes_sum<LW>(sm);
+                        const float mean = sm * INVN;
+                        float q = 0.f;
+#pragma unroll
+                        for (int e = 0; e < 8; ++e) { xr[i][e] -= mean; q += xr[i][e] * xr[i][e]; }
+                        q = lanes_sum<LW>(q);
+                        const float rstd = rsqrtf(q * INVN + 1e-5f);
+                        float a = 0.f, b = 0.f, t[8];
+#pragma unroll
+                        for (int e = 0; e < 8; ++e) { xr[i][e] *= rstd; t[e] = du[e] * gm[e]; a += t[e]; b += t[e] * xr[i][e]; }
+                        a = lanes_sum<LW>(a); b = lanes_sum<LW>(b);
+                        a *= INVN; b *= INVN;
+                        if (row < p.M) {
+                            float v[8];
+#pragma unroll
+                            for (int e = 0; e < 8; ++e) {
+                                v[e] = rs[i][e] + rstd * (t[e] - a - xr[i][e] * b);
+                                dgam[e] += du[e] * xr[i][e];
+                                dbet[e] += du[e];
+                            }
+                            float* op = reinterpret_cast<float*>(p.out) + (size_t)row * p.ldo + c8;
+                            *reinterpret_cast<float4*>(op) = make_float4(v[0], v[1], v[2], v[3]);
+                            *reinterpret_cast<float4*>(op + 4) = make_float4(v[4], v[5], v[6], v[7]);
+                        }
+                    }
                 }
                 lds_barrier();
-#pragma unroll
-                for (int mi = 0; mi < PR / 16; ++mi)
-#pragma unroll
-                    for (int j = 0; j < 2; ++j)
-#pragma unroll
-                        for (int r = 0; r < 4; ++r)
-                            T1[(mi * 16 + ag * 4 + r) * TS + wave * 32 + j * 16 + arow] = acc[ps * (PR / 16) + mi][j][r];
+                float* red = T1;
+#pragma unroll
+                for (int e = 0; e < 8; ++e) { red[tid * 8 + e] = dgam[e]; red[2048 + tid * 8 + e] = dbet[e]; }
                 lds_barrier();
-#pragma unroll
-                for (int i = 0; i < NPC; ++i) {
-                    const int rl = (tid + 256 * i) >> 4;
-                    const int row = row0 + ps * PR + rl;
-                    const float4 t0 = *reinterpret_cast<const float4*>(T1 + rl * TS + c8);
-                    const float4 t1 = *reinterpret_cast<const float4*>(T1 + rl * TS + c8 + 4);
-                    const float du[8] = {t0.x, t0.y, t0.z, t0.w, t1.x, t1.y, t1.z, t1.w};
-                    float sm = 0.f;
-#pragma unroll
-                    for (int e = 0; e < 8; ++e) sm += xr[i][e];
-                    sm = lanes_sum<16>(sm);
-                    const float mean = sm * (1.f / 128.f);
-                    float q = 0.f;
-#pragma unroll
-                    for (int e = 0; e < 8; ++e) { xr[i][e] -= mean; q += xr[i][e] * xr[i][e]; }
-                    q = lanes_sum<16>(q);
-                    const float rstd = rsqrtf(q * (1.f / 128.f) + 1e-5f);
-                    float a = 0.f, b = 0.f, t[8];
-#pragma unroll
-                    for (int e = 0; e < 8; ++e) { xr[i][e] *= rstd; t[e] = du[e] * gm[e]; a += t[e]; b += t[e] * xr[i][e]; }
-                    a = lanes_sum<16>(a); b = lanes_sum<16>(b);
-                    a *= (1.f / 128.f); b *= (1.f / 128.f);
-                    if (row < p.M) {
-                        float v[8];
-#pragma unroll
-                        for (int e = 0; e < 8; ++e) {
-                            v[e] = rs[i][e] + rstd * (t[e] - a - xr[i][e] * b);
-                            dgam[e] += du[e] * xr[i][e];
-                            dbet[e] += du[e];
-                        }
-                        float* op = reinterpret_cast<float*>(p.out) + (size_t)row * p.ldo + c8;
-                        *reinterpret_cast<float4*>(op) = make_float4(v[0], v[1], v[2], v[3]);
-                        *reinterpret_cast<float4*>(op + 4) = make_float4(v[4], v[5], v[6], v[7]);
-                    }
-                }
-            }
-            lds_barrier();
-            float* red = T1;
-#pragma unroll
-            for (int e = 0; e < 8; ++e) { red[tid * 8 + e] = dgam[e]; red[2048 + tid * 8 + e] = dbet[e]; }
-            lds_barrier();
-            {
-                const int which = tid >> 7, c = tid & 127, o8 = c >> 3, e = c & 7;
-                float sacc = 0.f;
-                for (int t2 = o8; t2 < 256; t2 += 16) sacc += red[which * 2048 + t2 * 8 + e];
-                hs_gadd(HsDet{p.det_base, reinterpret_cast<long long*>(p.det_acc)}, (which ? p.dbeta : p.dgamma) + c, sacc);
+                {
+                    const int which = tid >> 7, c = tid & 127, o8 = c >> 3, e = c & 7;
+                    if (c < LW * 8) {
+                        float sacc = 0.f;
+                        for (int t2 = o8; t2 < 256; t2 += LW) sacc += red[which * 2048 + t2 * 8 + e];
+                        hs_gadd(HsDet{p.det_base, reinterpret_cast<long long*>(p.det_acc)}, (which ? p.dbeta : p.dgamma) + c, sacc);
+                    }
+                }
+            };
+            if constexpr (EPI == E_LN_BWD) {
+                ln_rows(std::integral_constant<int, 16>{});
+            } else {
+                if (p.N == 64) ln_rows(std::integral_constant<int, 8>{});
+                else ln_rows(std::integral_constant<int, 16>{});
             }
             PH(2)
             return;
@@ -763,7 +779,7 @@
 
 template <int AK, int EPI>
 int launch_f8(const GemmParams& p, hipStream_t s) {
-    if constexpr (EPI == E_LN_BWD || EPI == E_POS_F32) {
+    if constexpr (EPI == E_LN_BWD || EPI == E_LN_BWD_NR || EPI == E_POS_F32) {
         return HS_EUNSUPPORTED;
     } else {
         if (!p.W8 || !p.S8 || (EPI == E_SWIGLU && (!p.W8b || !p.S8b))) return HSIMAE_ENULL;
@@ -794,7 +810,7 @@
         if (p.K <= 256) return bm64 ? launch<AK, EPI, 256, 64>(p, s) : launch<AK, EPI, 256, 128>(p, s);
         if (p.K <= 512) return bm64 ? launch<AK, EPI, 512, 64>(p, s) : launch<AK, EPI, 512, 128>(p, s);
         return HS_EUNSUPPORTED;
-    } else if constexpr (EPI == E_LN_BWD) {
+    } else if constexpr (EPI == E_LN_BWD || EPI == E_LN_BWD_NR) {
         return launch<AK, EPI, 128, 128>(p, s);
     } else {
         const bool kc256 = g_force_kc ? g_force_kc == 256 : (bm64 && p.K >= 256 && p.K <= 1024);
@@ -859,6 +875,12 @@
         if (p.u_out) return HS_EUNSUPPORTED;
         return launch_kc<A_BF16, E_LN_BWD>(p, s);
     }
+    if (akind == A_BF16 && epi == E_LN_BWD_NR) {
+        if (p.prec == HSIMAE_PREC_FP8 || (p.N != 64 && p.N != 128) || p.n_valid != p.N || !p.lnx || !p.gamma || !p.dgamma || !p.dbeta ||
+            p.ldr % 4 || p.ldo % 4 || p.u_out)
+            return HS_EUNSUPPORTED;
+        return launch_kc<A_BF16, E_LN_BWD_NR>(p, s);
+    }
     CASE(A_F32, E_SWIGLU_BWD)
     CASE(A_F32, E_BF16)
     CASE(A_F32, E_F32)
diff --git a/hsimae_amd/csrc/kernels.h b/hsimae_amd/csrc/kernels.h
--- a/hsimae_amd/csrc/kernels.h
+++ b/hsimae_amd/csrc/kernels.h
@@ -5,7 +5,7 @@
 enum AKind { A_BF16 = HSIMAE_A_BF16, A_F32 = HSIMAE_A_F32, A_F32_LN = HSIMAE_A_F32_LN };
 enum Epi { E_BF16 = HSIMAE_E_BF16, E_F32 = HSIMAE_E_F32, E_RES_F32 = HSIMAE_E_RES_F32,
            E_POS_F32 = HSIMAE_E_POS_F32, E_SWIGLU = HSIMAE_E_SWIGLU, E_SWIGLU_BWD = HSIMAE_E_SWIGLU_BWD,
-           E_LN_BWD = HSIMAE_E_LN_BWD };
+           E_LN_BWD = HSIMAE_E_LN_BWD, E_LN_BWD_NR = HSIMAE_E_LN_BWD_NORES };
 
 typedef hsimae_gemm_params GemmParams;
 typedef hsimae_pack_desc PackDesc;
diff --git a/hsimae_amd/csrc/plan.h b/hsimae_amd/csrc/plan.h
--- a/hsimae_amd/csrc/plan.h
+++ b/hsimae_amd/csrc/plan.h
@@ -203,7 +203,7 @@
     hs_bf16* a_pe; float* x0;
     std::vector<BlkBuf> b1, b2, bf, bd;
     hs_bf16* lat; float* y; float* yfull; hs_bf16* zn; float* pred; hs_bf16* dpred; float* partial;
-    float *G0, *G1, *G2, *du; hs_bf16 *dh13, *dob, *dqkv, *dyb;
+    float *G0, *G1, *G2, *G3, *du; hs_bf16 *dh13, *dob, *dqkv, *dyb;
     float* slab;
     int64_t bytes;
 };
@@ -256,6 +256,7 @@
     w.slab = (float*)take(slab_bytes(g, false));
     w.sc.slab = w.slab;
     w.sc2.slab = slab_bytes(g, true) ? (float*)take(slab_bytes(g, true)) : nullptr;
+    w.G3 = g.has_axis ? (float*)take(Me * g.Dp * 4) : nullptr;
     w.bytes = cur;
 }
 
diff --git a/include/hsimae_hip.h b/include/hsimae_hip.h
--- a/include/hsimae_hip.h
+++ b/include/hsimae_hip.h
@@ -101,7 +101,8 @@
 enum { HSIMAE_A_BF16 = 0, HSIMAE_A_F32 = 1, HSIMAE_A_F32_LN = 2 };
 enum { HSIMAE_E_BF16 = 0, HSIMAE_E_F32 = 1, HSIMAE_E_RES_F32 = 2, HSIMAE_E_POS_F32 = 3, HSIMAE_E_SWIGLU = 4,
        HSIMAE_E_SWIGLU_BWD = 5,
-       HSIMAE_E_LN_BWD = 6 };
+       HSIMAE_E_LN_BWD = 6,
+       HSIMAE_E_LN_BWD_NORES = 7 };
 typedef struct {
     const void* A; int32_t lda;
     int32_t M, N, K;
```

New measurement: 274,600 patches/s (median of 5 runs). About the same (+0.6%).
